# uc-vision/splat-trainer

Hardware: AMD Instinct MI355X
Metric: fwd+bwd Gaussians/s (higher is better)
Workload: dtype f32

## Files before the change

include/gsplat_hip.h:

```cpp
#ifndef GSPLAT_HIP_H
#define GSPLAT_HIP_H

#include <stddef.h>
#include <stdint.h>

#ifdef __cplusplus
extern "C" {
#endif

#define GSR_OK 0
#define GSR_ERR_INVALID_ARGUMENT -1
#define GSR_ERR_WORKSPACE_TOO_SMALL -2
#define GSR_ERR_LAUNCH_FAILED -3
#define GSR_ERR_UNSUPPORTED -4

#define GSR_ROW_FLOATS 16
#define GSR_PARTIAL_FLOATS 12
#define GSR_MAX_FEATURES 16
#define GSR_WIDE_MIN_FEATURES 4

#ifndef GSR_HAVE_RASTER_PARAMS
#define GSR_HAVE_RASTER_PARAMS
typedef struct GsrRasterParamsC {
  float alpha_threshold;
  float clamp_max_alpha;
  float T_eps;
  float q_max;
  float blur;
  int32_t antialias;
  int32_t tile_size;
  float margin_px;
} GsrRasterParamsC;
#endif

typedef struct GsrSegmentsC {
  const uint32_t* tile_seg;
  const uint32_t* seg_desc;
  const uint32_t* seg_total;
  int64_t capacity;
  int64_t heavy_capacity;
  float* seg_P;
  float* seg_TC;
  int32_t* seg_last;
  float* seg_median;
  const uint32_t* tile_order;
} GsrSegmentsC;
#define GSR_SEG_TOTAL_WORDS 272
#define GSR_TILE_ORDER_WORDS(num_tiles) (8 * 32 * ((((num_tiles) + 127) / 128) * 16))

int64_t gsr_struct_bytes(int32_t which);
int gsr_abi_version(void);
const char* gsr_error_string(int code);

size_t gsr_scan_workspace_bytes(int64_t n);
int gsr_exclusive_scan_u32(const uint32_t* in, uint32_t* out, int64_t n, uint32_t* total_dev, void* workspace,
                           size_t workspace_bytes, void* stream);
int gsr_exclusive_scan_u32_checked(const uint32_t* in, uint32_t* out, int64_t n, uint32_t* total_dev,
                                   uint32_t* overflow_dev, void* workspace, size_t workspace_bytes, void* stream);
size_t gsr_sort_workspace_bytes(int64_t n);
int gsr_sort_pairs_u32(uint32_t* keys_a, uint32_t* vals_a, uint32_t* keys_b, uint32_t* vals_b, int64_t n,
                       int vals_are_iota, int begin_bit, int end_bit, void* workspace, size_t workspace_bytes,
                       const uint32_t* n_dev, void* stream);
int gsr_sort_pairs2_u32(uint32_t* keys_a, uint32_t* vals_a, uint32_t* vals2_a, uint32_t* keys_b, uint32_t* vals_b,
                        uint32_t* vals2_b, int64_t n, int vals_are_iota, int begin_bit, int end_bit, void* workspace,
                        size_t workspace_bytes, const uint32_t* n_dev, void* stream);

size_t gsr_cull_workspace_bytes(int64_t N);
int gsr_frustum_cull(const float* position, int64_t N, const float* T_camera_world, const float* projection,
                     int32_t W, int32_t H, float near_plane, float far_plane, float margin_px,
                     int64_t* indexes_out, uint32_t* count_dev, void* workspace, size_t workspace_bytes, void* stream);

int gsr_project_forward(const float* position, const float* log_scaling, const float* rotation_xyzw,
                        const float* alpha_logit, const int64_t* indexes, int64_t M, const float* T_camera_world,
                        const float* projection, const GsrRasterParamsC* params_host, float* gaussians2d_out,
                        float* depth_out, const uint32_t* count_dev, uint32_t* depth_keys_out, uint32_t depth_key_bias,
                        uint32_t depth_key_max, void* stream);
int gsr_project_backward(const float* position, const float* log_scaling, const float* rotation_xyzw,
                         const float* alpha_logit, const int64_t* indexes, int64_t M, const float* T_camera_world,
                         const float* projection, const GsrRasterParamsC* params_host, const float* dL_dgaussians2d,
                         const float* dL_ddepth, float* d_position, float* d_log_scaling, float* d_rotation,
                         float* d_alpha_logit, int32_t accumulate, void* stream);

int64_t gsr_camera_grad_partial_rows(int64_t count);
int gsr_project_backward_camera(const float* position, const float* log_scaling, const float* rotation_xyzw,
                                const float* alpha_logit, const int64_t* indexes, int64_t M, const float* T_camera_world,
                                const float* projection, const GsrRasterParamsC* params_host,
                                const float* dL_dgaussians2d, const float* dL_ddepth, float* d_position,
                                float* d_log_scaling, float* d_rotation, float* d_alpha_logit, int32_t accumulate,
                                float* camera_partials, float* d_camera, void* stream);
int gsr_sh_camera_position_grad(const float* dL_dcolors, const float* jacobian, int64_t M, float* camera_partials,
                                float* d_camera_pos, void* stream);
int gsr_camera_grad_finish(const float* camera_partials, int64_t rows, const float* T_camera_world, float* d_camera,
                           void* stream);

int gsr_sh_forward(const float* sh_features, const float* positions, const int64_t* indexes, int64_t M, int32_t K,
                   const float* camera_pos, float* colors_out, float* jacobian_out, const uint32_t* count_dev,
                   void* stream);
int gsr_sh_backward(const float* dL_dcolors, const float* sh_features, const float* positions, const int64_t* indexes,
                    int64_t M, int32_t K, const float* camera_pos, const float* jacobian ,
                    float* d_sh_features, float* d_positions, int32_t accumulate, void* stream);

int gsr_inverse_map(const int64_t* indexes, int64_t M, int64_t N, int32_t* inverse_out, void* stream);
int gsr_sh_backward_dense(const float* dL_dcolors, const float* sh_features, const float* positions,
                          const int32_t* inverse, int64_t M, int64_t N, int32_t K, const float* camera_pos,
                          const float* jacobian , float* d_sh_features, float* d_positions,
                          void* stream);

int gsr_sh_backward_multi(const float* dL_dcolors_dense, int64_t dense_stride, const float* camera_positions,
                          int64_t camera_stride, int32_t num_cameras, const float* sh_features, const float* positions,
                          int64_t N, int32_t K, float* d_sh_features, float* d_positions, int32_t accumulate,
                          void* stream);

int gsr_project_sh_forward(const float* position, const float* log_scaling, const float* rotation_xyzw,
                           const float* alpha_logit, const float* sh_features, int32_t K, const int64_t* indexes, int64_t M,
                           const float* T_camera_world, const float* projection, const float* camera_pos,
                           const GsrRasterParamsC* params_host, float* rows_out, float* screen_scale_out,
                           float* jacobian_out, const uint32_t* count_dev, uint32_t* depth_keys_out,
                           uint32_t depth_key_bias, uint32_t depth_key_max, void* stream);
int gsr_project_backward_rows(const float* position, const float* log_scaling, const float* rotation_xyzw,
                              const float* alpha_logit, const int64_t* indexes, int64_t M, const int32_t* inverse,
                              int64_t N, const float* T_camera_world, const float* projection,
                              const GsrRasterParamsC* params_host, const float* rows ,
                              const float* grad_rows, const float* dL_dgaussians2d_extra, const float* dL_ddepth,
                              const float* jacobian,
                              float* d_position, float* d_log_scaling, float* d_rotation, float* d_alpha_logit,
                              int32_t mode, float* d_colors_out, float* prune_cost_out, float* split_score_out,
                              float* visibility_out, void* stream);
int gsr_project_backward_rows_camera(const float* position, const float* log_scaling, const float* rotation_xyzw,
                                     const float* alpha_logit, const int64_t* indexes, int64_t M, const int32_t* inverse,
                                     int64_t N, const float* T_camera_world, const float* projection,
                                     const GsrRasterParamsC* params_host, const float* rows, const float* grad_rows,
                                     const float* dL_dgaussians2d_extra, const float* dL_ddepth, const float* jacobian,
                                     float* d_position, float* d_log_scaling, float* d_rotation, float* d_alpha_logit,
                                     int32_t mode, float* d_colors_out, float* prune_cost_out, float* split_score_out,
                                     float* visibility_out, float* camera_partials, float* d_camera, void* stream);

int gsr_depth_key_range(float near_plane, float far_plane, uint32_t* bias_out, uint32_t* max_key_out);
int gsr_depth_keys(const float* depth, int64_t M, uint32_t bias, uint32_t max_key, uint32_t* keys_out, void* stream);
int gsr_pack_rows(const float* gaussians2d, const float* depth, const float* features, int64_t M, int32_t C,
                  const GsrRasterParamsC* params_host, float* rows_out, float* screen_scale_out, void* stream);
int gsr_pack_rows_wide(const float* gaussians2d, const float* depth, const float* features, int64_t M, int32_t C,
                       const GsrRasterParamsC* params_host, float* rows_out, float* feat_rows_out, float* screen_scale_out,
                       void* stream);
int gsr_tile_count(const float* rows, const uint32_t* order, int64_t M, int32_t W, int32_t H,
                   const GsrRasterParamsC* params_host, uint32_t* count_out, uint32_t* tile_hits_out,
                   const uint32_t* M_dev , void* stream);
#define GSR_TILE_COUNT_OFFSETS_MAX 4194304
size_t gsr_tile_count_offsets_workspace_bytes(int64_t M);
int gsr_tile_count_offsets(const float* rows, const uint32_t* order, int64_t M, int32_t W, int32_t H,
                           const GsrRasterParamsC* params_host, uint32_t* count_out, uint32_t* tile_hits_out,
                           const uint32_t* M_dev, uint32_t* offsets_out, uint32_t* total_dev, uint32_t* overflow_flag,
                           void* workspace, size_t workspace_bytes, void* stream);
int gsr_tile_emit(const float* rows, const uint32_t* order, const uint32_t* offsets, const uint32_t* tile_hits, int64_t M,
                  int32_t W, int32_t H, const GsrRasterParamsC* params_host, uint32_t* keys_out, uint32_t* inst2splat_out,
                  int64_t capacity, const uint32_t* M_dev , void* stream);
int gsr_tile_ranges(const uint32_t* sorted_keys, int64_t O, int32_t num_tiles, uint32_t* tile_range,
                    const uint32_t* O_dev , void* stream);

int gsr_segment_thresholds(int32_t seg_pairs_cfg, int32_t heavy_min_cfg, int64_t O, int32_t num_tiles, int32_t needs_grad,
                           int32_t* seg_pairs_out, int32_t* heavy_min_out);
int64_t gsr_segment_capacity(int64_t O, int32_t O_is_bound, int32_t seg_pairs_cfg, int32_t heavy_min_cfg, int32_t num_tiles,
                             int32_t needs_grad);
int64_t gsr_segment_heavy_capacity(int64_t O, int32_t O_is_bound, int32_t seg_pairs_cfg, int32_t heavy_min_cfg,
                                   int32_t num_tiles, int32_t needs_grad);
int gsr_segment_plan(const uint32_t* tile_range, int32_t num_tiles, int32_t seg_pairs_cfg, int32_t heavy_min_cfg,
                     int32_t needs_grad, int64_t O, const uint32_t* O_dev, int64_t capacity, int64_t heavy_capacity,
                     uint32_t* tile_seg_out, uint32_t* seg_desc_out, uint32_t* seg_total_out, uint32_t* tile_order_out,
                     void* stream);

int gsr_composite_forward(const float* rows , const uint32_t* sorted_splat, const uint32_t* sorted_inst,
                          const uint32_t* tile_range, int32_t W, int32_t H, int32_t C,
                          const GsrRasterParamsC* params_host, float* image_out, float* final_T_out,
                          int32_t* last_out, float* median_depth_out, float* vis_partial_out, float* pair_vis_out,
                          const GsrSegmentsC* segments_host ,
                          int32_t prefetch_rows ,
                          void* stream);
int gsr_composite_forward_wide(const float* rows , const float* feat_rows ,
                               const uint32_t* sorted_splat, const uint32_t* sorted_inst, const uint32_t* tile_range,
                               int32_t W, int32_t H, int32_t C, const GsrRasterParamsC* params_host, float* image_out,
                               float* final_T_out, int32_t* last_out, float* median_depth_out, float* vis_partial_out,
                               float* pair_vis_out, void* stream);
#ifndef GSR_PREFETCH_MIN_ROWS
#define GSR_PREFETCH_MIN_ROWS 1000000
#endif

int gsr_composite_backward(const float* rows , const uint32_t* sorted_splat, const uint32_t* sorted_inst,
                           const float* pair_vis, const uint32_t* tile_range, int32_t W, int32_t H, int32_t C,
                           const GsrRasterParamsC* params_host, const float* final_T, const int32_t* last,
                           const float* dL_dimage, const float* image ,
                           float* partial_out, const GsrSegmentsC* segments_host ,
                           void* stream);
int gsr_composite_backward_wide(const float* rows , const float* feat_rows ,
                                const uint32_t* sorted_splat, const uint32_t* sorted_inst, const float* pair_vis,
                                const uint32_t* tile_range, int32_t W, int32_t H, int32_t C,
                                const GsrRasterParamsC* params_host, const float* final_T, const int32_t* last,
                                const float* dL_dimage, float* partial_out, void* stream);

int gsr_reduce_visibility(const float* vis_partial, const uint32_t* offsets, const uint32_t* count,
                          const uint32_t* order, int64_t M, float* visibility_out, int64_t capacity,
                          const uint32_t* M_dev , void* stream);
int gsr_reduce_gradients(const float* partial, const float* vis_partial, const uint32_t* offsets,
                         const uint32_t* count, const uint32_t* order, int64_t M, float* grad_rows_out, void* stream);
int gsr_reduce_gradients_wide(const float* partial, const float* vis_partial, const uint32_t* offsets,
                              const uint32_t* count, const uint32_t* order, int64_t M, int32_t C, float* grad_rows_out,
                              float* d_features_out, void* stream);
int gsr_unpack_grad_rows(const float* rows , const float* grad_rows, int64_t M, int32_t C,
                         float* d_gaussians2d, float* d_features, float* prune_cost_out, float* split_score_out,
                         float* visibility_out, void* stream);

typedef struct GsrFrameC {
  const float* position;
  const float* log_scaling;
  const float* rotation_xyzw;
  const float* alpha_logit;
  const float* sh_features;
  int64_t N;
  int32_t K;
  int32_t W, H;
  const float* T_camera_world;
  const float* projection;
  const float* camera_pos;
  float near_plane, far_plane;
  GsrRasterParamsC params;
  int32_t want_jacobian;
  int32_t want_median;
  int32_t compute_visibility;
  int32_t needs_grad;
  int32_t seg_pairs, seg_min_pairs;
  int64_t pair_capacity;
  const float* gaussians2d;
  const float* depth;
  const float* features;
  int32_t C;
  const uint32_t* depth_order;
  int32_t feature_table;
} GsrFrameC;
typedef struct GsrFramePlanC {
  int64_t out_bytes, work_bytes;
  int64_t zero_begin, zero_bytes;
  int64_t prune_cost, split_score, counts, tile_range, vis_partial, indexes, rows, screen_scale, jacobian, visibility,
      image, final_T, last, median, count, offsets, vals_a, vals_b, tvals_a, tvals_b, trank_a, trank_b, pair_vis,
      seg_tables, seg_pix, seg_last;
  int64_t seg_capacity, seg_heavy_capacity;
  int64_t cull_ws, sort_ws, scan_ws, tsort_ws, keys_a, keys_b, tile_hits, tkeys_a, tkeys_b;
  int64_t cull_ws_bytes, sort_ws_bytes, scan_ws_bytes, tsort_ws_bytes;
  int64_t feat_rows;
} GsrFramePlanC;
typedef struct GsrFrameResultC {
  int64_t order;
  int64_t sorted_inst;
  int64_t sorted_splat;
  GsrSegmentsC segments;
  int32_t has_segments;
} GsrFrameResultC;
int gsr_frame_plan(const GsrFrameC* frame_host, GsrFramePlanC* plan_out_host);
int gsr_frame_forward(const GsrFrameC* frame_host, const GsrFramePlanC* plan_host, void* out_arena, void* work_arena,
                      GsrFrameResultC* result_out_host, uint32_t* counts_host, void* event_counts, void* event_k6_begin,
                      void* event_k6_end, void* stream);

typedef struct GsrFrameBackwardC {
  const float* position; const float* log_scaling; const float* rotation_xyzw; const float* alpha_logit;
  const float* sh_features;
  int64_t N; int32_t K; int32_t W, H, C;
  const float* T_camera_world; const float* projection; const float* camera_pos;
  GsrRasterParamsC params;
  int64_t M, O;
  const int64_t* indexes; const float* rows; const uint32_t* order; const uint32_t* count; const uint32_t* offsets;
  const uint32_t* sorted_splat; const uint32_t* sorted_inst; const float* pair_vis; const float* vis_partial;
  const uint32_t* tile_range; const float* final_T; const int32_t* last; const float* image;
  const float* jacobian;
  const GsrSegmentsC* segments;
  const float* d_image; const float* d_gaussians2d; const float* d_depth;
  float* partial;
  float* grad_rows;
  int32_t* inverse;
  float* d_colors;
  float* d_position; float* d_log_scaling; float* d_rotation; float* d_alpha_logit; int32_t mode;
  float* d_sh; int32_t sh_mode;
  float* prune_cost; float* split_score; float* visibility;
  float* camera_partials; float* d_camera;
} GsrFrameBackwardC;
int gsr_frame_backward(const GsrFrameBackwardC* backward_host, void* event_k7_begin, void* event_k7_end, void* stream);
int gsr_frame_backward_stages(const GsrFrameBackwardC* backward_host, int32_t stages, void* event_k7_begin,
                              void* event_k7_end, void* stream);

size_t gsr_ssim_workspace_bytes(int32_t B, int32_t C, int32_t H, int32_t W);
int gsr_ssim_forward(const float* img1, const float* img2, const int64_t* strides1_host, const int64_t* strides2_host,
                     int32_t B, int32_t C, int32_t H, int32_t W, int32_t crop, float* mean_out, float* dm_dmu1,
                     float* dm_dm11, float* dm_dm12, void* workspace, size_t workspace_bytes, void* stream);
int gsr_ssim_backward(const float* img1, const float* img2, const int64_t* strides1_host, const int64_t* strides2_host,
                      const int64_t* strides_out_host, int32_t B, int32_t C, int32_t H, int32_t W, const float* dm_dmu1,
                      const float* dm_dm11, const float* dm_dm12, const float* grad_scale_dev, float* d_img1,
                      void* stream);

size_t gsr_pixel_loss_workspace_bytes(int64_t n);
int gsr_pixel_loss_forward(const float* image, const float* target, int64_t n, int32_t kind, float lo, float hi,
                           float* loss_out, void* workspace, size_t workspace_bytes, void* stream);
int gsr_pixel_loss_backward(const float* image, const float* target, int64_t n, int32_t kind, float lo, float hi,
                            const float* grad_scale_dev, float* d_image, void* stream);

int gsr_opt_point_weights(const int64_t* indexes, const float* visibility, int64_t M, float* step, float* vis_avg,
                          float beta1, float beta2, float vis_beta, float vis_smooth, int32_t bias_correction,
                          float* row_scale_out, void* stream);
int gsr_opt_step(float* param, const float* grad, float* exp_avg, float* exp_avg_sq, const int64_t* indexes,
                 const float* row_scale, const float* basis, int64_t M, int32_t D, int32_t type, int32_t algo, float lr,
                 float beta1, float beta2, float eps, float grad_clip, void* stream);
int gsr_point_basis(const float* log_scaling, const float* rotation_xyzw, const int64_t* indexes, int64_t M, float eps,
                    float* basis_out, void* stream);

size_t gsr_select_workspace_bytes(int64_t N);
int gsr_select_n(const float* values, int64_t N, int64_t n, int32_t descending, uint8_t* mask_out, void* workspace,
                 size_t workspace_bytes, void* stream);

#define GSR_MAX_COLUMNS 32
typedef struct GsrColumnC {
  const void* src;
  void* dst;
  const void* tail;
  int32_t width_dwords;
} GsrColumnC;
size_t gsr_compact_workspace_bytes(int64_t N);
int gsr_compact_offsets(const uint8_t* keep_mask, int64_t N, uint32_t* block_offsets_out, uint32_t* kept_total_dev,
                        void* workspace, size_t workspace_bytes, void* stream);
int gsr_compact_columns(const uint8_t* keep_mask, int64_t N, const uint32_t* block_offsets, int64_t kept_total,
                        int64_t n_tail, const GsrColumnC* columns_host, int32_t n_columns, void* stream);

int gsr_point_state_add(const int64_t* idx, const float* screen_scale, int32_t scale_cols, const float* visibility,
                        const float* split_score, const float* prune_cost, int64_t M, float split_alpha,
                        float prune_alpha, float* state_prune_cost, float* state_split_score, float* state_max_scale_px,
                        int16_t* state_points_in_view, float* state_visibility, float* visible_sum, void* stream);

size_t gsr_msloss_workspace_bytes(int32_t H, int32_t W, int32_t C, int32_t levels);
int gsr_msloss_forward(const float* image, const float* target, int32_t H, int32_t W, int32_t C, int32_t levels,
                       float w_l1, float w_mse, float w_ssim, float lo, float hi, float* metrics_out, void* workspace,
                       size_t workspace_bytes, void* stream);
int gsr_msloss_backward(const float* image, const float* target, int32_t H, int32_t W, int32_t C, int32_t levels,
                        float w_l1, float w_mse, float w_ssim, float lo, float hi, const float* grad_scale_dev,
                        void* workspace, size_t workspace_bytes, float* d_image, void* stream);

#define GSR_BILAGRID_MAX_SIDE 32768
size_t gsr_bilagrid_workspace_bytes(int32_t L, int32_t GH, int32_t GW);
int gsr_bilagrid_slice_forward(const float* grids, int64_t N, int32_t L, int32_t GH, int32_t GW, int64_t k,
                               const float* rgb, int32_t H, int32_t W, float* out, void* stream);
int gsr_bilagrid_slice_backward(const float* grids, int64_t N, int32_t L, int32_t GH, int32_t GW, int64_t k,
                                const float* rgb, int32_t H, int32_t W, const float* d_out, float* d_rgb, float* d_grids,
                                void* workspace, size_t workspace_bytes, void* stream);
int gsr_bilagrid_tv(const float* grids, int64_t N, int32_t L, int32_t GH, int32_t GW, float weight, float* tv_out,
                    float* d_grids, int32_t accumulate, void* workspace, size_t workspace_bytes, void* stream);

#define GSR_KNN_MAX_K 16
#define GSR_NEIGHBOURS_MAX_N 0x7FFFFFFF
size_t gsr_knn_workspace_bytes(int64_t N, int32_t k);
int gsr_knn(const float* points, int64_t N, int32_t k, float* dist2_out, int64_t* idx_out, float* scale_out,
            void* workspace, size_t workspace_bytes, void* stream);
int gsr_assign_clusters(const float* x, int64_t N, const float* centroids, int64_t K, int64_t* labels_out, void* stream);
size_t gsr_kmeans_workspace_bytes(int64_t N, int64_t K);
int gsr_kmeans_iter(const float* x, int64_t N, float* centroids, int64_t K, int32_t iters, int64_t* labels_out,
                    void* workspace, size_t workspace_bytes, void* stream);

typedef struct GsrColorModel {
  int32_t P, G, H, L, S, color_channels;
  const float* weight[7];
  const float* bias[7];
} GsrColorModel;
typedef struct GsrColorGrads {
  float* d_weight[7];
  float* d_bias[7];
  float* d_glo;
  float* d_cam_pos;
} GsrColorGrads;
int64_t gsr_color_struct_bytes(int32_t which);
int gsr_color_supported(const GsrColorModel* model);
size_t gsr_color_forward_workspace_bytes(const GsrColorModel* model);
size_t gsr_color_backward_workspace_bytes(const GsrColorModel* model, int64_t M);
int gsr_color_forward(const GsrColorModel* model, const float* point_features, const float* positions,
                      const float* cam_pos, const float* glo_feature, int64_t M, float* diffuse_out, float* specular_out,
                      void* workspace, size_t workspace_bytes, void* stream);
int gsr_color_backward(const GsrColorModel* model, const float* point_features, const float* positions,
                       const float* cam_pos, const float* glo_feature, int64_t M, const float* d_diffuse,
                       const float* d_specular, float* d_point_features, const GsrColorGrads* grads, void* workspace,
                       size_t workspace_bytes, void* stream);

#define GSR_DP_BLOCK_FLOATS(N) (6 * (int64_t)(N) + 3)
int gsr_dp_pack(const int64_t* idx, const float* dL_dcolors, const float* split_score, const float* prune_cost,
                const float* screen_scale, int32_t scale_cols, const float* camera_pos, int64_t M, int64_t N,
                float* block_out, const float* visibility, float* visibility_sum, float* views_sum, void* stream);
int gsr_dp_replay(const float* blocks, int64_t stride, const int32_t* slots, int32_t num_cameras, int64_t N,
                  float split_alpha, float prune_alpha, float* state_split_score, float* state_prune_cost,
                  float* state_max_scale_px, const float* visibility_sum, const float* views_sum,
                  float* state_visibility, int16_t* state_points_in_view, void* stream);

int gsr_dp_pack_sharded(const int64_t* idx, const float* dL_dcolors, const float* split_score, const float* prune_cost,
                        const float* screen_scale, int32_t scale_cols, const float* camera_pos, int64_t M, int64_t N,
                        int32_t num_ranks, int32_t slots_per_rank, int32_t slot, float* factors_out, float* scores_out,
                        float* scale_max, const float* visibility, float* visibility_sum, float* views_sum, void* stream);
int gsr_dp_pack_factors_rows(const int64_t* idx, const float* grad_rows, const float* camera_pos, int64_t M, int64_t N,
                             float* factors_out, void* stream);
int gsr_dp_replay_slice(const float* recv, int32_t num_ranks, int32_t slots_per_rank, int64_t N, int32_t rank,
                        int32_t num_cameras, float split_alpha, float prune_alpha, const float* state_split_score,
                        const float* state_prune_cost, float* slice_out, void* stream);
int gsr_dp_finish(const float* gathered, int32_t num_ranks, int64_t N, float* state_split_score, float* state_prune_cost,
                  const float* scale_max, float* state_max_scale_px, const float* visibility_sum, const float* views_sum,
                  float* state_visibility, int16_t* state_points_in_view, void* stream);

#ifdef __cplusplus
}
#endif
#endif
```

splat-trainer_amd/_lib.py:

```python
from __future__ import annotations

import ctypes as C
import os
import threading

import torch

PKG_DIR = os.path.dirname(os.path.abspath(__file__))
LIB_PATH = os.path.join(PKG_DIR, "libgsplat_hip.so")

ABI_VERSION = 36
PREFETCH_MIN_ROWS = 1_000_000
MAX_FEATURES = 16
WIDE_MIN_FEATURES = 4
BILAGRID_MAX_SIDE = 32768
KNN_MAX_K = 16
NEIGHBOURS_MAX_N = 0x7FFFFFFF


class GsrRasterParamsC(C.Structure):
  _fields_ = [("alpha_threshold", C.c_float), ("clamp_max_alpha", C.c_float), ("T_eps", C.c_float),
              ("q_max", C.c_float), ("blur", C.c_float), ("antialias", C.c_int32), ("tile_size", C.c_int32),
              ("margin_px", C.c_float)]


class GsrSegmentsC(C.Structure):
  _fields_ = [("tile_seg", C.c_void_p), ("seg_desc", C.c_void_p), ("seg_total", C.c_void_p), ("capacity", C.c_int64),
              ("heavy_capacity", C.c_int64), ("seg_P", C.c_void_p), ("seg_TC", C.c_void_p), ("seg_last", C.c_void_p),
              ("seg_median", C.c_void_p), ("tile_order", C.c_void_p)]


class GsrFrameC(C.Structure):
  _fields_ = [("position", C.c_void_p), ("log_scaling", C.c_void_p), ("rotation_xyzw", C.c_void_p),
              ("alpha_logit", C.c_void_p), ("sh_features", C.c_void_p), ("N", C.c_int64), ("K", C.c_int32),
              ("W", C.c_int32), ("H", C.c_int32), ("T_camera_world", C.c_void_p), ("projection", C.c_void_p),
              ("camera_pos", C.c_void_p), ("near_plane", C.c_float), ("far_plane", C.c_float),
              ("params", GsrRasterParamsC), ("want_jacobian", C.c_int32), ("want_median", C.c_int32),
              ("compute_visibility", C.c_int32), ("needs_grad", C.c_int32), ("seg_pairs", C.c_int32),
              ("seg_min_pairs", C.c_int32), ("pair_capacity", C.c_int64), ("gaussians2d", C.c_void_p),
              ("depth", C.c_void_p), ("features", C.c_void_p), ("C", C.c_int32), ("depth_order", C.c_void_p),
              ("feature_table", C.c_int32)]


FRAME_PLAN_FIELDS = ("out_bytes", "work_bytes", "zero_begin", "zero_bytes", "prune_cost", "split_score", "counts",
                     "tile_range", "vis_partial", "indexes", "rows", "screen_scale", "jacobian", "visibility", "image",
                     "final_T", "last", "median", "count", "offsets", "vals_a", "vals_b", "tvals_a", "tvals_b", "trank_a",
                     "trank_b", "pair_vis", "seg_tables", "seg_pix", "seg_last", "seg_capacity", "seg_heavy_capacity",
                     "cull_ws", "sort_ws", "scan_ws", "tsort_ws", "keys_a", "keys_b", "tile_hits", "tkeys_a", "tkeys_b",
                     "cull_ws_bytes", "sort_ws_bytes", "scan_ws_bytes", "tsort_ws_bytes", "feat_rows")


class GsrFramePlanC(C.Structure):
  _fields_ = [(name, C.c_int64) for name in FRAME_PLAN_FIELDS]


class GsrFrameBackwardC(C.Structure):
  _fields_ = [("position", C.c_void_p), ("log_scaling", C.c_void_p), ("rotation_xyzw", C.c_void_p),
              ("alpha_logit", C.c_void_p), ("sh_features", C.c_void_p), ("N", C.c_int64), ("K", C.c_int32),
              ("W", C.c_int32), ("H", C.c_int32), ("C", C.c_int32), ("T_camera_world", C.c_void_p),
              ("projection", C.c_void_p), ("camera_pos", C.c_void_p), ("params", GsrRasterParamsC), ("M", C.c_int64),
              ("O", C.c_int64), ("indexes", C.c_void_p), ("rows", C.c_void_p), ("order", C.c_void_p),
              ("count", C.c_void_p), ("offsets", C.c_void_p), ("sorted_splat", C.c_void_p), ("sorted_inst", C.c_void_p),
              ("pair_vis", C.c_void_p), ("vis_partial", C.c_void_p), ("tile_range", C.c_void_p), ("final_T", C.c_void_p),
              ("last", C.c_void_p), ("image", C.c_void_p), ("jacobian", C.c_void_p), ("segments", C.c_void_p),
              ("d_image", C.c_void_p), ("d_gaussians2d", C.c_void_p), ("d_depth", C.c_void_p), ("partial", C.c_void_p),
              ("grad_rows", C.c_void_p), ("inverse", C.c_void_p), ("d_colors", C.c_void_p), ("d_position", C.c_void_p),
              ("d_log_scaling", C.c_void_p), ("d_rotation", C.c_void_p), ("d_alpha_logit", C.c_void_p),
              ("mode", C.c_int32), ("d_sh", C.c_void_p), ("sh_mode", C.c_int32), ("prune_cost", C.c_void_p),
              ("split_score", C.c_void_p), ("visibility", C.c_void_p), ("camera_partials", C.c_void_p),
              ("d_camera", C.c_void_p)]


class GsrFrameResultC(C.Structure):
  _fields_ = [("order", C.c_int64), ("sorted_inst", C.c_int64), ("sorted_splat", C.c_int64), ("segments", GsrSegmentsC),
              ("has_segments", C.c_int32)]


class GsrColumnC(C.Structure):
  _fields_ = [("src", C.c_void_p), ("dst", C.c_void_p), ("tail", C.c_void_p), ("width_dwords", C.c_int32)]


MAX_COLUMNS = 32


class GsrColorModelC(C.Structure):
  _fields_ = [("P", C.c_int32), ("G", C.c_int32), ("H", C.c_int32), ("L", C.c_int32), ("S", C.c_int32),
              ("color_channels", C.c_int32), ("weight", C.c_void_p * 7), ("bias", C.c_void_p * 7)]


class GsrColorGradsC(C.Structure):
  _fields_ = [("d_weight", C.c_void_p * 7), ("d_bias", C.c_void_p * 7), ("d_glo", C.c_void_p),
              ("d_cam_pos", C.c_void_p)]


def raster_params(config) -> GsrRasterParamsC:
  blur = float(config.blur_cov) + (float(config.aa_blur) if config.antialias else 0.0)
  return GsrRasterParamsC(float(config.alpha_threshold), float(config.clamp_max_alpha),
                          float(config.transmittance_eps), float(config.gaussian_scale) ** 2, blur,
                          1 if config.antialias else 0, int(config.tile_size),
                          float(config.margin_tiles * config.tile_size))


_p = C.c_void_p
_i64, _i32, _u32, _f, _sz = C.c_int64, C.c_int32, C.c_uint32, C.c_float, C.c_size_t
_pp = C.POINTER(GsrRasterParamsC)
_ps = C.POINTER(GsrSegmentsC)

PROTOTYPES = {
    "gsr_abi_version": (C.c_int, []),
    "gsr_error_string": (C.c_char_p, [C.c_int]),
    "gsr_scan_workspace_bytes": (_sz, [_i64]),
    "gsr_exclusive_scan_u32": (C.c_int, [_p, _p, _i64, _p, _p, _sz, _p]),
    "gsr_exclusive_scan_u32_checked": (C.c_int, [_p, _p, _i64, _p, _p, _p, _sz, _p]),
    "gsr_sort_workspace_bytes": (_sz, [_i64]),
    "gsr_sort_pairs_u32": (C.c_int, [_p, _p, _p, _p, _i64, C.c_int, C.c_int, C.c_int, _p, _sz, _p, _p]),
    "gsr_sort_pairs2_u32": (C.c_int, [_p, _p, _p, _p, _p, _p, _i64, C.c_int, C.c_int, C.c_int, _p, _sz, _p, _p]),
    "gsr_cull_workspace_bytes": (_sz, [_i64]),
    "gsr_frustum_cull": (C.c_int, [_p, _i64, _p, _p, _i32, _i32, _f, _f, _f, _p, _p, _p, _sz, _p]),
    "gsr_project_forward": (C.c_int, [_p, _p, _p, _p, _p, _i64, _p, _p, _pp, _p, _p, _p, _p, _u32, _u32, _p]),
    "gsr_project_backward": (C.c_int, [_p, _p, _p, _p, _p, _i64, _p, _p, _pp, _p, _p, _p, _p, _p, _p, _i32, _p]),
    "gsr_camera_grad_partial_rows": (_i64, [_i64]),
    "gsr_project_backward_camera": (C.c_int, [_p, _p, _p, _p, _p, _i64, _p, _p, _pp, _p, _p, _p, _p, _p, _p, _i32, _p, _p,
                                              _p]),
    "gsr_sh_camera_position_grad": (C.c_int, [_p, _p, _i64, _p, _p, _p]),
    "gsr_camera_grad_finish": (C.c_int, [_p, _i64, _p, _p, _p]),
    "gsr_sh_forward": (C.c_int, [_p, _p, _p, _i64, _i32, _p, _p, _p, _p, _p]),
    "gsr_sh_backward": (C.c_int, [_p, _p, _p, _p, _i64, _i32, _p, _p, _p, _p, _i32, _p]),
    "gsr_sh_backward_multi": (C.c_int, [_p, _i64, _p, _i64, _i32, _p, _p, _i64, _i32, _p, _p, _i32, _p]),
    "gsr_inverse_map": (C.c_int, [_p, _i64, _i64, _p, _p]),
    "gsr_sh_backward_dense": (C.c_int, [_p, _p, _p, _p, _i64, _i64, _i32, _p, _p, _p, _p, _p]),
    "gsr_depth_key_range": (C.c_int, [_f, _f, _p, _p]),
    "gsr_depth_keys": (C.c_int, [_p, _i64, _u32, _u32, _p, _p]),
    "gsr_project_sh_forward": (C.c_int, [_p, _p, _p, _p, _p, _i32, _p, _i64, _p, _p, _p, _pp, _p, _p, _p, _p, _p, _u32,
                                         _u32, _p]),
    "gsr_project_backward_rows": (C.c_int, [_p, _p, _p, _p, _p, _i64, _p, _i64, _p, _p, _pp, _p, _p, _p, _p, _p, _p, _p,
                                            _p, _p, _i32, _p, _p, _p, _p, _p]),
    "gsr_project_backward_rows_camera": (C.c_int, [_p, _p, _p, _p, _p, _i64, _p, _i64, _p, _p, _pp, _p, _p, _p, _p, _p,
                                                   _p, _p, _p, _p, _i32, _p, _p, _p, _p, _p, _p, _p]),
    "gsr_pack_rows": (C.c_int, [_p, _p, _p, _i64, _i32, _pp, _p, _p, _p]),
    "gsr_pack_rows_wide": (C.c_int, [_p, _p, _p, _i64, _i32, _pp, _p, _p, _p, _p]),
    "gsr_tile_count": (C.c_int, [_p, _p, _i64, _i32, _i32, _pp, _p, _p, _p, _p]),
    "gsr_tile_count_offsets_workspace_bytes": (_sz, [_i64]),
    "gsr_tile_count_offsets": (C.c_int, [_p, _p, _i64, _i32, _i32, _pp, _p, _p, _p, _p, _p, _p, _p, _sz, _p]),
    "gsr_tile_emit": (C.c_int, [_p, _p, _p, _p, _i64, _i32, _i32, _pp, _p, _p, _i64, _p, _p]),
    "gsr_tile_ranges": (C.c_int, [_p, _i64, _i32, _p, _p, _p]),
    "gsr_segment_thresholds": (C.c_int, [_i32, _i32, _i64, _i32, _i32, _p, _p]),
    "gsr_segment_capacity": (_i64, [_i64, _i32, _i32, _i32, _i32, _i32]),
    "gsr_segment_heavy_capacity": (_i64, [_i64, _i32, _i32, _i32, _i32, _i32]),
    "gsr_segment_plan": (C.c_int, [_p, _i32, _i32, _i32, _i32, _i64, _p, _i64, _i64, _p, _p, _p, _p, _p]),
    "gsr_composite_forward": (C.c_int, [_p, _p, _p, _p, _i32, _i32, _i32, _pp, _p, _p, _p, _p, _p, _p, _ps, _i32, _p]),
    "gsr_composite_backward": (C.c_int, [_p, _p, _p, _p, _p, _i32, _i32, _i32, _pp, _p, _p, _p, _p, _p, _ps, _p]),
    "gsr_composite_forward_wide": (C.c_int, [_p, _p, _p, _p, _p, _i32, _i32, _i32, _pp, _p, _p, _p, _p, _p, _p, _p]),
    "gsr_composite_backward_wide": (C.c_int, [_p, _p, _p, _p, _p, _p, _i32, _i32, _i32, _pp, _p, _p, _p, _p, _p]),
    "gsr_opt_point_weights": (C.c_int, [_p, _p, _i64, _p, _p, _f, _f, _f, _f, _i32, _p, _p]),
    "gsr_opt_step": (C.c_int, [_p, _p, _p, _p, _p, _p, _p, _i64, _i32, _i32, _i32, _f, _f, _f, _f, _f, _p]),
    "gsr_pixel_loss_workspace_bytes": (_sz, [_i64]),
    "gsr_pixel_loss_forward": (C.c_int, [_p, _p, _i64, _i32, _f, _f, _p, _p, _sz, _p]),
    "gsr_pixel_loss_backward": (C.c_int, [_p, _p, _i64, _i32, _f, _f, _p, _p, _p]),
    "gsr_ssim_workspace_bytes": (_sz, [_i32, _i32, _i32, _i32]),
    "gsr_ssim_forward": (C.c_int, [_p, _p, _p, _p, _i32, _i32, _i32, _i32, _i32, _p, _p, _p, _p, _p, _sz, _p]),
    "gsr_ssim_backward": (C.c_int, [_p, _p, _p, _p, _p, _i32, _i32, _i32, _i32, _p, _p, _p, _p, _p, _p]),
    "gsr_msloss_workspace_bytes": (_sz, [_i32, _i32, _i32, _i32]),
    "gsr_msloss_forward": (C.c_int, [_p, _p, _i32, _i32, _i32, _i32, _f, _f, _f, _f, _f, _p, _p, _sz, _p]),
    "gsr_msloss_backward": (C.c_int, [_p, _p, _i32, _i32, _i32, _i32, _f, _f, _f, _f, _f, _p, _p, _sz, _p, _p]),
    "gsr_select_workspace_bytes": (_sz, [_i64]),
    "gsr_select_n": (C.c_int, [_p, _i64, _i64, _i32, _p, _p, _sz, _p]),
    "gsr_compact_workspace_bytes": (_sz, [_i64]),
    "gsr_compact_offsets": (C.c_int, [_p, _i64, _p, _p, _p, _sz, _p]),
    "gsr_compact_columns": (C.c_int, [_p, _i64, _p, _i64, _i64, C.POINTER(GsrColumnC), _i32, _p]),
    "gsr_point_basis": (C.c_int, [_p, _p, _p, _i64, _f, _p, _p]),
    "gsr_dp_pack": (C.c_int, [_p, _p, _p, _p, _p, _i32, _p, _i64, _i64, _p, _p, _p, _p, _p]),
    "gsr_dp_replay": (C.c_int, [_p, _i64, _p, _i32, _i64, _f, _f, _p, _p, _p, _p, _p, _p, _p, _p]),
    "gsr_dp_pack_sharded": (C.c_int, [_p, _p, _p, _p, _p, _i32, _p, _i64, _i64, _i32, _i32, _i32, _p, _p, _p, _p, _p, _p, _p]),
    "gsr_dp_replay_slice": (C.c_int, [_p, _i32, _i32, _i64, _i32, _i32, _f, _f, _p, _p, _p, _p]),
    "gsr_dp_finish": (C.c_int, [_p, _i32, _i64, _p, _p, _p, _p, _p, _p, _p, _p, _p]),
    "gsr_point_state_add": (C.c_int, [_p, _p, _i32, _p, _p, _p, _i64, _f, _f, _p, _p, _p, _p, _p, _p, _p]),
    "gsr_frame_plan": (C.c_int, [C.POINTER(GsrFrameC), C.POINTER(GsrFramePlanC)]),
    "gsr_struct_bytes": (_i64, [_i32]),
    "gsr_frame_backward": (C.c_int, [C.POINTER(GsrFrameBackwardC), _p, _p, _p]),
    "gsr_frame_backward_stages": (C.c_int, [C.POINTER(GsrFrameBackwardC), _i32, _p, _p, _p]),
    "gsr_dp_pack_factors_rows": (C.c_int, [_p, _p, _p, _i64, _i64, _p, _p]),
    "gsr_frame_forward": (C.c_int, [C.POINTER(GsrFrameC), C.POINTER(GsrFramePlanC), _p, _p, C.POINTER(GsrFrameResultC), _p,
                                    _p, _p, _p, _p]),
    "gsr_reduce_visibility": (C.c_int, [_p, _p, _p, _p, _i64, _p, _i64, _p, _p]),
    "gsr_reduce_gradients": (C.c_int, [_p, _p, _p, _p, _p, _i64, _p, _p]),
    "gsr_reduce_gradients_wide": (C.c_int, [_p, _p, _p, _p, _p, _i64, _i32, _p, _p, _p]),
    "gsr_unpack_grad_rows": (C.c_int, [_p, _p, _i64, _i32, _p, _p, _p, _p, _p, _p]),
    "gsr_bilagrid_workspace_bytes": (_sz, [_i32, _i32, _i32]),
    "gsr_bilagrid_slice_forward": (C.c_int, [_p, _i64, _i32, _i32, _i32, _i64, _p, _i32, _i32, _p, _p]),
    "gsr_bilagrid_slice_backward": (C.c_int, [_p, _i64, _i32, _i32, _i32, _i64, _p, _i32, _i32, _p, _p, _p, _p, _sz, _p]),
    "gsr_bilagrid_tv": (C.c_int, [_p, _i64, _i32, _i32, _i32, _f, _p, _p, _i32, _p, _sz, _p]),
    "gsr_knn_workspace_bytes": (_sz, [_i64, _i32]),
    "gsr_knn": (C.c_int, [_p, _i64, _i32, _p, _p, _p, _p, _sz, _p]),
    "gsr_assign_clusters": (C.c_int, [_p, _i64, _p, _i64, _p, _p]),
    "gsr_kmeans_workspace_bytes": (_sz, [_i64, _i64]),
    "gsr_kmeans_iter": (C.c_int, [_p, _i64, _p, _i64, _i32, _p, _p, _sz, _p]),
    "gsr_color_struct_bytes": (_i64, [_i32]),
    "gsr_color_supported": (C.c_int, [C.POINTER(GsrColorModelC)]),
    "gsr_color_forward_workspace_bytes": (_sz, [C.POINTER(GsrColorModelC)]),
    "gsr_color_backward_workspace_bytes": (_sz, [C.POINTER(GsrColorModelC), _i64]),
    "gsr_color_forward": (C.c_int, [C.POINTER(GsrColorModelC), _p, _p, _p, _p, _i64, _p, _p, _p, _sz, _p]),
    "gsr_color_backward": (C.c_int, [C.POINTER(GsrColorModelC), _p, _p, _p, _p, _i64, _p, _p, _p,
                                     C.POINTER(GsrColorGradsC), _p, _sz, _p]),
}

_lib = None
_lock = threading.Lock()


def current_stream_ptr() -> int:
  return torch._C._cuda_getCurrentRawStream(torch._C._cuda_getDevice())


def current_stream() -> "torch.cuda.Stream":
  return torch.cuda.current_stream(torch._C._cuda_getDevice())


class GsplatHipError(RuntimeError):
  pass


def load() -> C.CDLL:
  global _lib
  if _lib is not None:
    return _lib
  with _lock:
    if _lib is not None:
      return _lib
    if not os.path.exists(LIB_PATH):
      raise GsplatHipError(
          f"{LIB_PATH} not found: build it with `python splat-trainer_amd/build.py` "
          "(hipcc --offload-arch=gfx950). There is no CPU fallback for the rasterizer path.")
    try:
      lib = C.CDLL(LIB_PATH)
    except OSError as e:
      raise GsplatHipError(f"failed to load {LIB_PATH}: {e}") from e
    for name, (restype, argtypes) in PROTOTYPES.items():
      fn = getattr(lib, name)
      fn.restype = restype
      fn.argtypes = argtypes
    if lib.gsr_abi_version() != ABI_VERSION:
      raise GsplatHipError(f"ABI mismatch: library {lib.gsr_abi_version()} != binding {ABI_VERSION}; rebuild")
    for which, mirror in enumerate((GsrRasterParamsC, GsrSegmentsC, GsrFrameC, GsrFramePlanC, GsrFrameResultC,
                                    GsrFrameBackwardC)):
      if lib.gsr_struct_bytes(which) != C.sizeof(mirror):
        raise GsplatHipError(f"struct layout mismatch: {mirror.__name__} is {C.sizeof(mirror)} bytes in the binding, "
                             f"{lib.gsr_struct_bytes(which)} in the library; rebuild")
    for which, mirror in enumerate((GsrColorModelC, GsrColorGradsC)):
      if lib.gsr_color_struct_bytes(which) != C.sizeof(mirror):
        raise GsplatHipError(f"struct layout mismatch: {mirror.__name__} is {C.sizeof(mirror)} bytes in the binding, "
                             f"{lib.gsr_color_struct_bytes(which)} in the library; rebuild")
    _lib = lib
  return _lib


def check(code: int, what: str) -> int:
  if code < 0:
    msg = load().gsr_error_string(code).decode()
    raise GsplatHipError(f"{what} failed: {msg} ({code})")
  return code
```

splat-trainer_amd/csrc/binning.hip:

```cpp
#include "gsr_device.h"
#include "../../include/gsplat_hip.h"

namespace {

inline GsrRasterParams to_params(const GsrRasterParamsC* c) {
  GsrRasterParams rp;
  __builtin_memcpy(&rp, c, sizeof(rp));
  return rp;
}
inline unsigned grid_for(int64_t n, int block) { return (unsigned)((n + block - 1) / block); }

__global__ __launch_bounds__(256) void depth_keys_kernel(const float* __restrict__ depth, int64_t M,
                                                         uint32_t* __restrict__ keys, uint32_t bias, uint32_t max_key) {
  const int64_t m = (int64_t)blockIdx.x * blockDim.x + threadIdx.x;
  if (m >= M) return;
  keys[m] = gsr_depth_key(depth[m], bias, max_key);
}

struct TileHits {
  uint32_t origin;
  uint32_t shape;
  uint32_t lo, hi;
};

__device__ __forceinline__ uint32_t hits_of_large_extent(float u, float v, float A, float B, float C, float qmax, int x0,
                                                         int x1, int y0, int y1, uint32_t* keys, uint32_t* ranks,
                                                         uint32_t o, uint32_t capacity, uint32_t k, int tiles_x,
                                                         int lane) {
  const int nx = x1 - x0, total = nx * (y1 - y0);
  uint32_t n = 0;
  for (int t0 = 0; t0 < total; t0 += 64) {
    const int t = t0 + lane;
    uint32_t hm = 0u;
    int tx = 0, ty = 0;
    if (t < total) {
      ty = y0 + t / nx;
      tx = x0 + t % nx;
      if (gsr_tile_hit(u, v, A, B, C, qmax, tx, ty)) hm = gsr_tile_half_mask(u, v, A, B, C, qmax, tx, ty);
    }
    const uint64_t hit = __ballot(hm != 0u);
    if (keys && hm) {
      const uint32_t at = o + n + (uint32_t)gsr_mbcnt(hit);
      if (at < capacity) {
        keys[at] = (uint32_t)(ty * tiles_x + tx);
        ranks[at] = k | (hm << 30);
      }
    }
    n += (uint32_t)__builtin_popcountll(hit);
  }
  return n;
}

__device__ __forceinline__ float gsr_bcast(float x, int l) {
  return __int_as_float(__builtin_amdgcn_readlane(__float_as_int(x), l));
}

__device__ __forceinline__ uint32_t wave_large_extents(bool large, float u, float v, float A, float B, float C,
                                                       const GsrExtent& e, uint32_t* keys, uint32_t* ranks, uint32_t o,
                                                       uint32_t capacity, uint32_t sid, int tiles_x, int lane) {
  uint32_t mine = 0u;
  uint64_t todo = __ballot(large);
  while (todo) {
    const int l = __builtin_ctzll(todo);
    todo &= todo - 1ull;
    const uint32_t n = hits_of_large_extent(
        gsr_bcast(u, l), gsr_bcast(v, l), gsr_bcast(A, l), gsr_bcast(B, l), gsr_bcast(C, l), gsr_bcast(e.qmax, l),
        __builtin_amdgcn_readlane(e.x0, l), __builtin_amdgcn_readlane(e.x1, l), __builtin_amdgcn_readlane(e.y0, l),
        __builtin_amdgcn_readlane(e.y1, l), keys, ranks, (uint32_t)__builtin_amdgcn_readlane((int)o, l), capacity,
        (uint32_t)__builtin_amdgcn_readlane((int)sid, l), tiles_x, lane);
    if (lane == l) mine = n;
  }
  return mine;
}

__device__ __forceinline__ uint32_t tile_count_one(const float* __restrict__ rows, const uint32_t* __restrict__ order,
                                                   int64_t k, bool live, int tiles_x, int tiles_y,
                                                   const GsrRasterParams& rp, TileHits* __restrict__ hits) {
  float2 uv = make_float2(0.f, 0.f), ab = uv, co = uv;
  GsrExtent e;
  e.x0 = e.x1 = e.y0 = e.y1 = 0; e.qmax = 0.f;
  TileHits h;
  h.origin = 0u; h.shape = 0u; h.lo = 0u; h.hi = 0u;
  uint32_t n = 0;
  bool large = false;
  if (live) {
    const int64_t s = order[k];
    const float4* r = reinterpret_cast<const float4*>(rows + GSR_ROW_FLOATS * s);
    const float4 r0 = r[0];
    const float4 r1 = r[1];
    uv = make_float2(r0.x, r0.y); ab = make_float2(r0.z, r0.w); co = make_float2(r1.x, r1.y);
    e = gsr_splat_extent(uv.x, uv.y, ab.x, ab.y, co.x, co.y, rp, tiles_x, tiles_y);
    const int nx = e.x1 - e.x0, ny = e.y1 - e.y0;
    h.origin = (uint32_t)e.x0 | ((uint32_t)e.y0 << 16);
    if (nx > 0 && ny > 0) {
      if (nx * ny <= 32) {
        h.shape = (uint32_t)nx | ((uint32_t)ny << 8);
        uint64_t map = 0ull;
        int t = 0;
        for (int ty = e.y0; ty < e.y1; ++ty)
          for (int tx = e.x0; tx < e.x1; ++tx, ++t) {
            const uint64_t hm = gsr_tile_half_mask(uv.x, uv.y, ab.x, ab.y, co.x, e.qmax, tx, ty);
            map |= hm << (2 * t);
            n += hm ? 1u : 0u;
          }
        h.lo = (uint32_t)map; h.hi = (uint32_t)(map >> 32);
      } else {
        h.shape = 1u << 16;
        large = true;
      }
    }
  }
  const uint32_t nl = wave_large_extents(large, uv.x, uv.y, ab.x, ab.y, co.x, e, nullptr, nullptr, 0u, 0u, 0u, tiles_x,
                                         gsr_lane());
  if (large) n = nl;
  if (live) *reinterpret_cast<uint4*>(hits + k) = make_uint4(h.origin, h.shape, h.lo, h.hi);
  return n;
}

__global__ __launch_bounds__(256) void tile_count_kernel(const float* __restrict__ rows,
                                                         const uint32_t* __restrict__ order, int64_t M, int tiles_x,
                                                         int tiles_y, GsrRasterParams rp, uint32_t* __restrict__ count,
                                                         TileHits* __restrict__ hits,
                                                         const uint32_t* __restrict__ M_dev,
                                                         uint32_t* __restrict__ block_sums) {
  const int64_t k = (int64_t)blockIdx.x * blockDim.x + threadIdx.x;
  const bool live = k < M && !(M_dev && k >= (int64_t)*M_dev);
  uint32_t n = tile_count_one(rows, order, k, live, tiles_x, tiles_y, rp, hits);
  if (k < M) count[k] = n;
  if (block_sums) {
    __shared__ uint32_t s_wave[4];
    n = gsr_wave_sum_u32(n);
    if (gsr_lane() == 0) s_wave[threadIdx.x >> 6] = n;
    __syncthreads();
    if (threadIdx.x == 0) block_sums[blockIdx.x] = (s_wave[0] + s_wave[1]) + (s_wave[2] + s_wave[3]);
  }
}

__global__ __launch_bounds__(256) void offsets_from_sums_kernel(const uint32_t* __restrict__ count, uint32_t n,
                                                                const uint32_t* __restrict__ sums256,
                                                                uint32_t* __restrict__ offsets,
                                                                uint32_t* __restrict__ total_out,
                                                                uint32_t* __restrict__ overflow) {
  __shared__ uint32_t s_wave[4], s_before[4];
  __shared__ float s_f[4];
  const int lane = gsr_lane(), w = (int)(threadIdx.x >> 6);
  const uint32_t base = blockIdx.x * 4096u + threadIdx.x * 16u;
  uint32_t v[16], sum = 0u;
#pragma unroll
  for (int i = 0; i < 16; ++i) {
    v[i] = (base + i < n) ? count[base + i] : 0u;
    sum += v[i];
  }
  uint32_t before = 0u;
  float fbefore = 0.f;
  for (uint32_t j = threadIdx.x; j < blockIdx.x * 16u; j += 256u) {
    const uint32_t b = sums256[j];
    before += b;
    fbefore += (float)b;
  }
  const uint32_t incl = gsr_wave_scan_incl_u32(sum);
  before = gsr_wave_sum_u32(before);
  fbefore = gsr_wave_sum(fbefore + (float)sum);
  if (lane == 63) s_wave[w] = incl;
  if (lane == 0) { s_before[w] = before; s_f[w] = fbefore; }
  __syncthreads();
  uint32_t prefix = (s_before[0] + s_before[1]) + (s_before[2] + s_before[3]), total = 0u;
  uint32_t in_block = 0u;
#pragma unroll
  for (int j = 0; j < 4; ++j) {
    if (j < w) in_block += s_wave[j];
    total += s_wave[j];
  }
  if (threadIdx.x == 0 && (s_f[0] + s_f[1]) + (s_f[2] + s_f[3]) >= 2147000000.f) *overflow = 1u;
  uint32_t run = prefix + in_block + incl - sum;
#pragma unroll
  for (int i = 0; i < 16; ++i) {
    if (base + i < n) offsets[base + i] = run;
    run += v[i];
  }
  if (total_out && blockIdx.x == gridDim.x - 1 && threadIdx.x == 0) *total_out = prefix + total;
}


__global__ __launch_bounds__(256) void tile_emit_kernel(const float* __restrict__ rows,
                                                        const uint32_t* __restrict__ order,
                                                        const uint32_t* __restrict__ offsets,
                                                        const TileHits* __restrict__ hits, int64_t M, int tiles_x,
                                                        int tiles_y, GsrRasterParams rp, uint32_t* __restrict__ keys,
                                                        uint32_t* __restrict__ inst2splat, uint32_t capacity,
                                                        const uint32_t* __restrict__ M_dev) {
  const int64_t k = (int64_t)blockIdx.x * blockDim.x + threadIdx.x;
  const bool live = k < M && !(M_dev && k >= (int64_t)*M_dev);
  uint4 hw = make_uint4(0u, 0u, 0u, 0u);
  uint32_t o = 0u, sid = 0u;
  if (live) {
    hw = *reinterpret_cast<const uint4*>(hits + k);
    o = offsets[k];
    sid = order[k];
  }
  const bool large = (hw.y >> 16) != 0u;
  float4 r0 = make_float4(0.f, 0.f, 0.f, 0.f), r1 = r0;
  GsrExtent e;
  e.x0 = e.x1 = e.y0 = e.y1 = 0; e.qmax = 0.f;
  if (large) {
    const float4* r = reinterpret_cast<const float4*>(rows + GSR_ROW_FLOATS * (int64_t)sid);
    r0 = r[0];
    r1 = r[1];
    e = gsr_splat_extent(r0.x, r0.y, r0.z, r0.w, r1.x, r1.y, rp, tiles_x, tiles_y);
  }
  wave_large_extents(large, r0.x, r0.y, r0.z, r0.w, r1.x, e, keys, inst2splat, o, capacity, sid, tiles_x, gsr_lane());
  if (!live || large) return;
  const int nx = (int)(hw.y & 0xFFu), ny = (int)((hw.y >> 8) & 0xFFu);
  const int x0 = (int)(hw.x & 0xFFFFu), y0 = (int)(hw.x >> 16);
  uint64_t map = (uint64_t)hw.z | ((uint64_t)hw.w << 32);
  for (int j = 0; j < ny; ++j)
    for (int i = 0; i < nx; ++i, map >>= 2) {
      const uint32_t hm = (uint32_t)(map & 3ull);
      if (!hm) continue;
      if (o >= capacity) return;
      keys[o] = (uint32_t)((y0 + j) * tiles_x + x0 + i);
      inst2splat[o] = sid | (hm << 30);
      ++o;
    }
}

__global__ __launch_bounds__(256) void tile_ranges_kernel(const uint32_t* __restrict__ keys, int64_t O,
                                                          uint32_t* __restrict__ range,
                                                          const uint32_t* __restrict__ O_dev) {
  if (O_dev) O = min(O, (int64_t)*O_dev);
  const int64_t i = (int64_t)blockIdx.x * blockDim.x + threadIdx.x;
  if (i >= O) return;
  const uint32_t t = keys[i];
  if (i == 0 || keys[i - 1] != t) range[2 * t] = (uint32_t)i;
  if (i == O - 1 || keys[i + 1] != t) range[2 * t + 1] = (uint32_t)(i + 1);
}

#define GSR_REDUCE_SERIAL 64u

__global__ __launch_bounds__(256) void reduce_vis_kernel(const float* __restrict__ vis_partial,
                                                         const uint32_t* __restrict__ offsets,
                                                         const uint32_t* __restrict__ count,
                                                         const uint32_t* __restrict__ order, int64_t M,
                                                         float* __restrict__ vis, uint32_t limit,
                                                         const uint32_t* __restrict__ M_dev) {
  const int64_t k = (int64_t)blockIdx.x * blockDim.x + threadIdx.x;
  const bool live = k < M && !(M_dev && k >= (int64_t)*M_dev);
  const uint32_t b = live ? offsets[k] : 0u, n = live ? count[k] : 0u;
  const int lane = gsr_lane();
  float acc = 0.f;
  if (n <= GSR_REDUCE_SERIAL)
    for (uint32_t j = 0; j < n && b + j < limit; ++j) acc += vis_partial[b + j];
  uint64_t todo = __ballot(n > GSR_REDUCE_SERIAL);
  while (todo) {
    const int l = __builtin_ctzll(todo);
    todo &= todo - 1ull;
    const uint32_t bl = (uint32_t)__builtin_amdgcn_readlane((int)b, l), nl = (uint32_t)__builtin_amdgcn_readlane((int)n, l);
    float total = 0.f;
    for (uint32_t g = 0; g < nl; g += 64u) {
      const uint32_t j = g + (uint32_t)lane;
      const float v = (j < nl && bl + j < limit) ? vis_partial[bl + j] : 0.f;
      total += gsr_wave_sum_to_lane63(v);
    }
    const float t = __int_as_float(__builtin_amdgcn_readlane(__float_as_int(total), 63));
    if (lane == l) acc = t;
  }
  if (live) vis[order ? order[k] : (uint32_t)k] = acc;
}

__global__ __launch_bounds__(256) void reduce_grad_kernel(const float* __restrict__ partial,
                                                          const float* __restrict__ vis_partial,
                                                          const uint32_t* __restrict__ offsets,
                                                          const uint32_t* __restrict__ count,
                                                          const uint32_t* __restrict__ order, int64_t M,
                                                          float* __restrict__ grows) {
  constexpr int CH = 256;
  __shared__ float4 s_part[CH * 3];
  __shared__ float s_vis[CH];
  __shared__ uint32_t s_lo, s_hi;
  const int64_t k0 = (int64_t)blockIdx.x * 256;
  const int64_t k = k0 + threadIdx.x;
  const bool have = k < M;
  const uint32_t b = have ? offsets[k] : 0u, n = have ? count[k] : 0u;
  const bool serial = n <= GSR_REDUCE_SERIAL;
  if (threadIdx.x == 0) s_lo = b;
  const int64_t klast = (k0 + 255 < M ? k0 + 255 : M - 1);
  if (k == klast) s_hi = b + n;
  __syncthreads();
  const uint32_t lo = s_lo, hi = s_hi;
  float4 a0 = make_float4(0.f, 0.f, 0.f, 0.f), a1 = a0, a2 = a0;
  float vsum = 0.f;
  const float4* src = reinterpret_cast<const float4*>(partial);
  for (uint32_t c = lo; c < hi; c += CH) {
    const uint32_t m = min((uint32_t)CH, hi - c);
    const bool mine = threadIdx.x < m;
    const float v = mine ? vis_partial[c + threadIdx.x] : 0.f;
    s_vis[threadIdx.x] = v;
    __syncthreads();
#pragma unroll
    for (int t = 0; t < 3; ++t) {
      const uint32_t f = threadIdx.x + t * CH;
      if (f < 3 * m && s_vis[f / 3] > 0.f) s_part[f] = src[(size_t)3 * c + f];
    }
    __syncthreads();
    const uint32_t j0 = max(b, c), j1 = serial ? min(b + n, c + m) : 0u;
    for (uint32_t j = j0; j < j1; ++j) {
      const uint32_t l = j - c;
      const float pv = s_vis[l];
      vsum += pv;
      if (pv > 0.f) {
        const float4 p0 = s_part[3 * l], p1 = s_part[3 * l + 1], p2 = s_part[3 * l + 2];
        a0.x += p0.x; a0.y += p0.y; a0.z += p0.z; a0.w += p0.w;
        a1.x += p1.x; a1.y += p1.y; a1.z += p1.z; a1.w += p1.w;
        a2.x += p2.x; a2.y += p2.y; a2.z += p2.z;
      }
    }
    __syncthreads();
  }
  const int lane = gsr_lane();
  uint64_t todo = __ballot(!serial);
  while (todo) {
    const int l = __builtin_ctzll(todo);
    todo &= todo - 1ull;
    const uint32_t bl = (uint32_t)__builtin_amdgcn_readlane((int)b, l), nl = (uint32_t)__builtin_amdgcn_readlane((int)n, l);
    float t[12];
#pragma unroll
    for (int i = 0; i < 12; ++i) t[i] = 0.f;
    for (uint32_t g = 0; g < nl; g += 64u) {
      const uint32_t j = g + (uint32_t)lane;
      const float pv = j < nl ? vis_partial[bl + j] : 0.f;
      float4 p0 = make_float4(0.f, 0.f, 0.f, 0.f), p1 = p0, p2 = p0;
      if (pv > 0.f) {
        const float4* q = src + (size_t)3 * (bl + j);
        p0 = q[0]; p1 = q[1]; p2 = q[2];
      }
      t[0] += gsr_wave_sum_to_lane63(p0.x); t[1] += gsr_wave_sum_to_lane63(p0.y);
      t[2] += gsr_wave_sum_to_lane63(p0.z); t[3] += gsr_wave_sum_to_lane63(p0.w);
      t[4] += gsr_wave_sum_to_lane63(p1.x); t[5] += gsr_wave_sum_to_lane63(p1.y);
      t[6] += gsr_wave_sum_to_lane63(p1.z); t[7] += gsr_wave_sum_to_lane63(p1.w);
      t[8] += gsr_wave_sum_to_lane63(p2.x); t[9] += gsr_wave_sum_to_lane63(p2.y);
      t[10] += gsr_wave_sum_to_lane63(p2.z); t[11] += gsr_wave_sum_to_lane63(pv);
    }
#pragma unroll
    for (int i = 0; i < 12; ++i) t[i] = __int_as_float(__builtin_amdgcn_readlane(__float_as_int(t[i]), 63));
    if (lane == l) {
      a0 = make_float4(t[0], t[1], t[2], t[3]);
      a1 = make_float4(t[4], t[5], t[6], t[7]);
      a2 = make_float4(t[8], t[9], t[10], 0.f);
      vsum = t[11];
    }
  }
  if (!have) return;
  const int64_t s = order ? (int64_t)order[k] : k;
  float4* g = reinterpret_cast<float4*>(grows + GSR_ROW_FLOATS * s);
  g[0] = a0;
  g[1] = a1;
  g[2] = make_float4(a2.x, a2.y, a2.z, vsum);
  g[3] = make_float4(0.f, 0.f, 0.f, 0.f);
}

template <int CW>
__global__ __launch_bounds__(256) void reduce_grad_wide_kernel(const float* __restrict__ partial,
                                                               const float* __restrict__ vis_partial,
                                                               const uint32_t* __restrict__ offsets,
                                                               const uint32_t* __restrict__ count,
                                                               const uint32_t* __restrict__ order, int64_t M, int C,
                                                               float* __restrict__ grows, float* __restrict__ dfeat) {
  constexpr int NV = 8 + CW;
  const int64_t k = (int64_t)blockIdx.x * blockDim.x + threadIdx.x;
  const bool have = k < M;
  const uint32_t b = have ? offsets[k] : 0u, n = have ? count[k] : 0u;
  const bool serial = n <= GSR_REDUCE_SERIAL;
  float a[NV];
#pragma unroll
  for (int v = 0; v < NV; ++v) a[v] = 0.f;
  float vsum = 0.f;
  if (serial) {
    for (uint32_t j = b; j < b + n; ++j) {
      const float pv = vis_partial[j];
      vsum += pv;
      if (pv > 0.f) {
        const float* p = partial + (size_t)NV * j;
#pragma unroll
        for (int v = 0; v < NV; ++v) a[v] += p[v];
      }
    }
  }
  const int lane = gsr_lane();
  uint64_t todo = __ballot(!serial);
  while (todo) {
    const int l = __builtin_ctzll(todo);
    todo &= todo - 1ull;
    const uint32_t bl = (uint32_t)__builtin_amdgcn_readlane((int)b, l), nl = (uint32_t)__builtin_amdgcn_readlane((int)n, l);
    float t[NV + 1];
#pragma unroll
    for (int v = 0; v <= NV; ++v) t[v] = 0.f;
    for (uint32_t g = 0; g < nl; g += 64u) {
      const uint32_t j = g + (uint32_t)lane;
      const float pv = j < nl ? vis_partial[bl + j] : 0.f;
      float pr[NV];
#pragma unroll
      for (int v = 0; v < NV; ++v) pr[v] = 0.f;
      if (pv > 0.f) {
        const float* p = partial + (size_t)NV * (bl + j);
#pragma unroll
        for (int v = 0; v < NV; ++v) pr[v] = p[v];
      }
#pragma unroll
      for (int v = 0; v < NV; ++v) t[v] += gsr_wave_sum_to_lane63(pr[v]);
      t[NV] += gsr_wave_sum_to_lane63(pv);
    }
#pragma unroll
    for (int v = 0; v <= NV; ++v) t[v] = __int_as_float(__builtin_amdgcn_readlane(__float_as_int(t[v]), 63));
    if (lane == l) {
#pragma unroll
      for (int v = 0; v < NV; ++v) a[v] = t[v];
      vsum = t[NV];
    }
  }
  if (!have) return;
  const int64_t s = order ? (int64_t)order[k] : k;
  float4* g = reinterpret_cast<float4*>(grows + GSR_ROW_FLOATS * s);
  g[0] = make_float4(a[0], a[1], a[2], a[3]);
  g[1] = make_float4(a[4], a[5], a[6], a[7]);
  g[2] = make_float4(0.f, 0.f, 0.f, vsum);
  g[3] = make_float4(0.f, 0.f, 0.f, 0.f);
#pragma unroll
  for (int c = 0; c < CW; ++c)
    if (c < C) dfeat[(int64_t)C * s + c] = a[8 + c];
}

template <int C>
__global__ __launch_bounds__(256) void unpack_rows_kernel(const float* __restrict__ rows,
                                                          const float* __restrict__ grows, int64_t M,
                                                          float* __restrict__ dg2d, float* __restrict__ dfeat,
                                                          float* __restrict__ prune, float* __restrict__ split,
                                                          float* __restrict__ vis) {
  const int64_t m = (int64_t)blockIdx.x * blockDim.x + threadIdx.x;
  if (m >= M) return;
  const float4* gr = reinterpret_cast<const float4*>(grows + GSR_ROW_FLOATS * m);
  const float4 g0 = gr[0], g1 = gr[1], g2 = gr[2];
  const float4* fr = reinterpret_cast<const float4*>(rows + GSR_ROW_FLOATS * m);
  const float4 f0 = fr[0];
  const float cA = f0.z, cB = f0.w, cC = fr[1].x;
  float* g = dg2d + 6 * m;
  *reinterpret_cast<float2*>(g) = make_float2(cA * g0.x + cB * g0.y, cB * g0.x + cC * g0.y);
  *reinterpret_cast<float2*>(g + 2) = make_float2(-0.5f * g0.z, -g0.w);
  const float op = fr[1].y;
  *reinterpret_cast<float2*>(g + 4) = make_float2(-0.5f * g1.x, op > 0.f ? g1.y / op : 0.f);
  if (prune) prune[m] = g1.z;
  if (split) split[m] = g1.w;
  if (vis) vis[m] = g2.w;
  if (C == 0) return;
  dfeat[C * m] = g2.x;
  if (C > 1) dfeat[C * m + 1] = g2.y;
  if (C > 2) dfeat[C * m + 2] = g2.z;
}

}

extern "C" {

int gsr_depth_key_range(float near_plane, float far_plane, uint32_t* bias_out, uint32_t* max_key_out) {
  if (!bias_out || !max_key_out) return GSR_ERR_INVALID_ARGUMENT;
  *bias_out = 0u;
  *max_key_out = 0xFFFFFFFFu;
  if (near_plane > 0.f && far_plane > near_plane && far_plane < 3.0e38f) {
    uint32_t lo, hi;
    __builtin_memcpy(&lo, &near_plane, 4);
    __builtin_memcpy(&hi, &far_plane, 4);
    *bias_out = lo | 0x80000000u;
    *max_key_out = hi - lo;
  }
  return GSR_OK;
}

int gsr_depth_keys(const float* depth, int64_t M, uint32_t bias, uint32_t max_key, uint32_t* keys_out, void* stream_) {
  hipStream_t stream = reinterpret_cast<hipStream_t>(stream_);
  if (M < 0) return GSR_ERR_INVALID_ARGUMENT;
  if (M == 0) return GSR_OK;
  if (!depth || !keys_out) return GSR_ERR_INVALID_ARGUMENT;
  depth_keys_kernel<<<grid_for(M, 256), 256, 0, stream>>>(depth, M, keys_out, bias, max_key);
  GSR_CHECK_LAUNCH();
  return GSR_OK;
}

int gsr_tile_count(const float* rows, const uint32_t* order, int64_t M, int32_t W, int32_t H,
                   const GsrRasterParamsC* params_host, uint32_t* count_out, uint32_t* tile_hits_out,
                   const uint32_t* M_dev, void* stream_) {
  hipStream_t stream = reinterpret_cast<hipStream_t>(stream_);
  if (M < 0 || M >= (1ll << 30) || !params_host || W <= 0 || H <= 0) return GSR_ERR_INVALID_ARGUMENT;
  if (params_host->tile_size != 16) return GSR_ERR_UNSUPPORTED;
  if (M == 0) return GSR_OK;
  if (!rows || !order || !count_out || !tile_hits_out) return GSR_ERR_INVALID_ARGUMENT;
  const int tx = (W + 15) / 16, ty = (H + 15) / 16;
  if (tx > 0xFFFF || ty > 0xFFFF) return GSR_ERR_UNSUPPORTED;
  tile_count_kernel<<<grid_for(M, 256), 256, 0, stream>>>(rows, order, M, tx, ty, to_params(params_host), count_out,
                                                         reinterpret_cast<TileHits*>(tile_hits_out), M_dev, nullptr);
  GSR_CHECK_LAUNCH();
  return GSR_OK;
}

size_t gsr_tile_count_offsets_workspace_bytes(int64_t M) {
  return M > 0 ? (size_t)((M + 255) / 256) * sizeof(uint32_t) + 256 : 256;
}

int gsr_tile_count_offsets(const float* rows, const uint32_t* order, int64_t M, int32_t W, int32_t H,
                           const GsrRasterParamsC* params_host, uint32_t* count_out, uint32_t* tile_hits_out,
                           const uint32_t* M_dev, uint32_t* offsets_out, uint32_t* total_dev, uint32_t* overflow_flag,
                           void* workspace, size_t workspace_bytes, void* stream_) {
  hipStream_t stream = reinterpret_cast<hipStream_t>(stream_);
  if (M < 0 || M > GSR_TILE_COUNT_OFFSETS_MAX || !params_host || W <= 0 || H <= 0) return GSR_ERR_INVALID_ARGUMENT;
  if (params_host->tile_size != 16) return GSR_ERR_UNSUPPORTED;
  if (!total_dev || !overflow_flag) return GSR_ERR_INVALID_ARGUMENT;
  if (M == 0) { hipMemsetAsync(total_dev, 0, sizeof(uint32_t), stream); return GSR_OK; }
  if (!rows || !order || !count_out || !tile_hits_out || !offsets_out) return GSR_ERR_INVALID_ARGUMENT;
  if (!workspace || workspace_bytes < gsr_tile_count_offsets_workspace_bytes(M)) return GSR_ERR_WORKSPACE_TOO_SMALL;
  const int tx = (W + 15) / 16, ty = (H + 15) / 16;
  if (tx > 0xFFFF || ty > 0xFFFF) return GSR_ERR_UNSUPPORTED;
  uint32_t* sums = reinterpret_cast<uint32_t*>(workspace);
  tile_count_kernel<<<grid_for(M, 256), 256, 0, stream>>>(rows, order, M, tx, ty, to_params(params_host), count_out,
                                                         reinterpret_cast<TileHits*>(tile_hits_out), M_dev, sums);
  GSR_CHECK_LAUNCH();
  offsets_from_sums_kernel<<<grid_for(M, 4096), 256, 0, stream>>>(count_out, (uint32_t)M, sums, offsets_out, total_dev,
                                                                 overflow_flag);
  GSR_CHECK_LAUNCH();
  return GSR_OK;
}

int gsr_tile_emit(const float* rows, const uint32_t* order, const uint32_t* offsets, const uint32_t* tile_hits, int64_t M,
                  int32_t W, int32_t H, const GsrRasterParamsC* params_host, uint32_t* keys_out, uint32_t* inst2splat_out,
                  int64_t capacity, const uint32_t* M_dev, void* stream_) {
  hipStream_t stream = reinterpret_cast<hipStream_t>(stream_);
  if (M < 0 || M >= (1ll << 30) || !params_host || W <= 0 || H <= 0) return GSR_ERR_INVALID_ARGUMENT;
  if (capacity < 0 || capacity > 0x7FFFFFFFll) return GSR_ERR_INVALID_ARGUMENT;
  if (params_host->tile_size != 16) return GSR_ERR_UNSUPPORTED;
  if (M == 0) return GSR_OK;
  if (!rows || !order || !offsets || !tile_hits || !keys_out || !inst2splat_out) return GSR_ERR_INVALID_ARGUMENT;
  const int tx = (W + 15) / 16, ty = (H + 15) / 16;
  tile_emit_kernel<<<grid_for(M, 256), 256, 0, stream>>>(rows, order, offsets, reinterpret_cast<const TileHits*>(tile_hits),
                                                        M, tx, ty, to_params(params_host), keys_out, inst2splat_out,
                                                        (uint32_t)capacity, M_dev);
  GSR_CHECK_LAUNCH();
  return GSR_OK;
}

int gsr_tile_ranges(const uint32_t* sorted_keys, int64_t O, int32_t num_tiles, uint32_t* tile_range,
                    const uint32_t* O_dev, void* stream_) {
  hipStream_t stream = reinterpret_cast<hipStream_t>(stream_);
  if (O < 0 || num_tiles <= 0) return GSR_ERR_INVALID_ARGUMENT;
  if (O == 0) return GSR_OK;
  if (!sorted_keys || !tile_range) return GSR_ERR_INVALID_ARGUMENT;
  tile_ranges_kernel<<<grid_for(O, 256), 256, 0, stream>>>(sorted_keys, O, tile_range, O_dev);
  GSR_CHECK_LAUNCH();
  return GSR_OK;
}

int gsr_reduce_visibility(const float* vis_partial, const uint32_t* offsets, const uint32_t* count,
                          const uint32_t* order, int64_t M, float* visibility_out, int64_t capacity,
                          const uint32_t* M_dev, void* stream_) {
  hipStream_t stream = reinterpret_cast<hipStream_t>(stream_);
  if (M < 0 || capacity < 0 || capacity > 0x7FFFFFFFll) return GSR_ERR_INVALID_ARGUMENT;
  if (M == 0) return GSR_OK;
  if (!offsets || !count || !visibility_out) return GSR_ERR_INVALID_ARGUMENT;
  reduce_vis_kernel<<<grid_for(M, 256), 256, 0, stream>>>(vis_partial, offsets, count, order, M, visibility_out,
                                                         (uint32_t)capacity, M_dev);
  GSR_CHECK_LAUNCH();
  return GSR_OK;
}

int gsr_reduce_gradients(const float* partial, const float* vis_partial, const uint32_t* offsets,
                         const uint32_t* count, const uint32_t* order, int64_t M, float* grad_rows_out, void* stream_) {
  hipStream_t stream = reinterpret_cast<hipStream_t>(stream_);
  if (M < 0) return GSR_ERR_INVALID_ARGUMENT;
  if (M == 0) return GSR_OK;
  if (!offsets || !count || !grad_rows_out) return GSR_ERR_INVALID_ARGUMENT;
  reduce_grad_kernel<<<grid_for(M, 256), 256, 0, stream>>>(partial, vis_partial, offsets, count, order, M, grad_rows_out);
  GSR_CHECK_LAUNCH();
  return GSR_OK;
}

int gsr_reduce_gradients_wide(const float* partial, const float* vis_partial, const uint32_t* offsets,
                              const uint32_t* count, const uint32_t* order, int64_t M, int32_t C, float* grad_rows_out,
                              float* d_features_out, void* stream_) {
  hipStream_t stream = reinterpret_cast<hipStream_t>(stream_);
  if (M < 0) return GSR_ERR_INVALID_ARGUMENT;
  if (C < GSR_WIDE_MIN_FEATURES || C > GSR_MAX_FEATURES) return GSR_ERR_UNSUPPORTED;
  if (M == 0) return GSR_OK;
  if (!offsets || !count || !grad_rows_out || !d_features_out || !vis_partial) return GSR_ERR_INVALID_ARGUMENT;
  const unsigned g = grid_for(M, 256);
  if (C <= 4) reduce_grad_wide_kernel<4><<<g, 256, 0, stream>>>(partial, vis_partial, offsets, count, order, M, C, grad_rows_out, d_features_out);
  else if (C <= 8) reduce_grad_wide_kernel<8><<<g, 256, 0, stream>>>(partial, vis_partial, offsets, count, order, M, C, grad_rows_out, d_features_out);
  else reduce_grad_wide_kernel<16><<<g, 256, 0, stream>>>(partial, vis_partial, offsets, count, order, M, C, grad_rows_out, d_features_out);
  GSR_CHECK_LAUNCH();
  return GSR_OK;
}

int gsr_unpack_grad_rows(const float* rows, const float* grad_rows, int64_t M, int32_t C, float* d_gaussians2d,
                         float* d_features, float* prune_cost_out, float* split_score_out, float* visibility_out,
                         void* stream_) {
  hipStream_t stream = reinterpret_cast<hipStream_t>(stream_);
  if (M < 0) return GSR_ERR_INVALID_ARGUMENT;
  if (C < 1 || C > (d_features ? 3 : GSR_MAX_FEATURES)) return GSR_ERR_UNSUPPORTED;
  if (M == 0) return GSR_OK;
  if (!rows || !grad_rows || !d_gaussians2d) return GSR_ERR_INVALID_ARGUMENT;
  const unsigned g = grid_for(M, 256);
  if (!d_features) unpack_rows_kernel<0><<<g, 256, 0, stream>>>(rows, grad_rows, M, d_gaussians2d, nullptr, prune_cost_out, split_score_out, visibility_out);
  else if (C == 1) unpack_rows_kernel<1><<<g, 256, 0, stream>>>(rows, grad_rows, M, d_gaussians2d, d_features, prune_cost_out, split_score_out, visibility_out);
  else if (C == 2) unpack_rows_kernel<2><<<g, 256, 0, stream>>>(rows, grad_rows, M, d_gaussians2d, d_features, prune_cost_out, split_score_out, visibility_out);
  else unpack_rows_kernel<3><<<g, 256, 0, stream>>>(rows, grad_rows, M, d_gaussians2d, d_features, prune_cost_out, split_score_out, visibility_out);
  GSR_CHECK_LAUNCH();
  return GSR_OK;
}

}
```

splat-trainer_amd/csrc/frame.hip:

```cpp
#include <hip/hip_runtime.h>
#include <stdint.h>
#include <string.h>

#include "../../include/gsplat_hip.h"

namespace {

inline int64_t align_up(int64_t x, int64_t a = 256) { return (x + a - 1) / a * a; }

struct Cursor {
  int64_t at = 0;
  int64_t take(int64_t bytes) {
    const int64_t o = at;
    at = align_up(at + (bytes > 0 ? bytes : 1));
    return o;
  }
};

inline int tile_bits_of(int num_tiles) {
  int b = 1;
  while ((1 << b) < num_tiles) ++b;
  return b;
}

inline int bit_length(uint32_t v) {
  int b = 0;
  while (v) { ++b; v >>= 1; }
  return b < 1 ? 1 : b;
}

template <class T>
inline T* at(void* base, int64_t off) {
  return off < 0 ? nullptr : reinterpret_cast<T*>(reinterpret_cast<uint8_t*>(base) + off);
}

}

extern "C" {

int gsr_frame_plan(const GsrFrameC* f, GsrFramePlanC* p) {
  if (!f || !p) return GSR_ERR_INVALID_ARGUMENT;
  if (f->N < 0 || f->N >= (1ll << 30) || f->W <= 0 || f->H <= 0 || f->pair_capacity < 0 || f->pair_capacity > 0x7FFFFFFFll)
    return GSR_ERR_INVALID_ARGUMENT;
  const bool projected = f->position == nullptr;
  if (!projected && f->K != 1 && f->K != 4 && f->K != 9 && f->K != 16) return GSR_ERR_UNSUPPORTED;
  if (f->C < 1 || f->C > GSR_MAX_FEATURES || (!projected && f->C != 3)) return GSR_ERR_UNSUPPORTED;
  const bool wide = f->C >= GSR_WIDE_MIN_FEATURES;
  if (wide && !f->feature_table) return GSR_ERR_UNSUPPORTED;
  if (f->params.tile_size != 16) return GSR_ERR_UNSUPPORTED;
  memset(p, 0, sizeof(*p));
  const int64_t N = f->N, cap = f->pair_capacity;
  const int64_t tx = (f->W + 15) / 16, ty = (f->H + 15) / 16, T = tx * ty, P = (int64_t)f->W * f->H;
  const bool vis_partial = f->compute_visibility || f->needs_grad;

  Cursor out;
  p->zero_begin = 0;
  p->prune_cost = out.take(4 * N);
  p->split_score = out.take(4 * N);
  p->counts = out.take(4 * (3 + GSR_SEG_TOTAL_WORDS));
  p->tile_range = out.take(4 * 2 * T);
  p->vis_partial = vis_partial ? out.take(4 * cap) : -1;
  p->zero_bytes = out.at;
  p->indexes = projected ? -1 : out.take(8 * N);
  p->rows = out.take(4 * GSR_ROW_FLOATS * N);
  p->screen_scale = out.take(4 * 2 * N);
  p->jacobian = (!projected && f->want_jacobian && f->K > 1) ? out.take(4 * 9 * N) : -1;
  p->visibility = out.take(4 * N);
  p->image = out.take(4 * f->C * P);
  p->final_T = out.take(4 * P);
  p->last = out.take(4 * P);
  p->median = f->want_median ? out.take(4 * P) : -1;
  p->count = out.take(4 * N);
  p->offsets = out.take(4 * N);
  p->vals_a = out.take(4 * N);
  p->vals_b = out.take(4 * N);
  p->tvals_a = out.take(4 * cap);
  p->tvals_b = out.take(4 * cap);
  p->trank_a = out.take(4 * cap + 16);
  p->trank_b = out.take(4 * cap + 16);
  p->pair_vis = vis_partial ? out.take(4 * cap) : -1;
  p->feat_rows = wide ? out.take(4 * (f->C <= 4 ? 4 : f->C <= 8 ? 8 : 16) * N) : -1;
  p->seg_capacity = 0;
  p->seg_heavy_capacity = 0;
  p->seg_tables = p->seg_pix = p->seg_last = -1;
  if (f->seg_pairs != 0 && cap > 0 && !wide) {
    const int64_t sc = gsr_segment_capacity(cap, 1, f->seg_pairs, f->seg_min_pairs, (int32_t)T, f->needs_grad ? 1 : 0);
    if (sc > 0) {
      int64_t hc = gsr_segment_heavy_capacity(cap, 1, f->seg_pairs, f->seg_min_pairs, (int32_t)T, f->needs_grad ? 1 : 0);
      if (hc > sc) hc = sc;
      p->seg_capacity = sc;
      p->seg_heavy_capacity = hc;
      p->seg_tables = out.take(4 * (2 * T + hc + 4 * sc + GSR_TILE_ORDER_WORDS(T)));
      const int64_t planes = 5 + (f->want_median ? 1 : 0);
      p->seg_pix = out.take(4 * planes * sc * 256);
      p->seg_last = out.take(4 * sc * 256);
    }
  }
  p->out_bytes = out.at;

  Cursor work;
  p->cull_ws_bytes = projected ? 0 : (int64_t)gsr_cull_workspace_bytes(N);
  p->sort_ws_bytes = (int64_t)gsr_sort_workspace_bytes(N);
  p->scan_ws_bytes = (int64_t)gsr_scan_workspace_bytes(N);
  if (N <= GSR_TILE_COUNT_OFFSETS_MAX && (int64_t)gsr_tile_count_offsets_workspace_bytes(N) > p->scan_ws_bytes)
    p->scan_ws_bytes = (int64_t)gsr_tile_count_offsets_workspace_bytes(N);
  p->tsort_ws_bytes = (int64_t)gsr_sort_workspace_bytes(cap);
  p->cull_ws = projected ? -1 : work.take(p->cull_ws_bytes);
  p->sort_ws = work.take(p->sort_ws_bytes);
  p->scan_ws = work.take(p->scan_ws_bytes);
  p->tsort_ws = work.take(p->tsort_ws_bytes);
  p->keys_a = work.take(4 * N);
  p->keys_b = work.take(4 * N);
  p->tile_hits = work.take(16 * N);
  p->tkeys_a = work.take(4 * cap);
  p->tkeys_b = work.take(4 * cap);
  p->work_bytes = work.at;
  return GSR_OK;
}

int gsr_frame_forward(const GsrFrameC* f, const GsrFramePlanC* p, void* out, void* work, GsrFrameResultC* res,
                      uint32_t* counts_host, void* event_counts, void* event_k6_begin, void* event_k6_end,
                      void* stream_) {
  hipStream_t stream = reinterpret_cast<hipStream_t>(stream_);
  if (!f || !p || !out || !work || !res) return GSR_ERR_INVALID_ARGUMENT;
  if (f->N <= 0) return GSR_ERR_INVALID_ARGUMENT;
  const bool projected = f->position == nullptr;
  if (projected) {
    if (!f->gaussians2d || !f->depth || !f->features) return GSR_ERR_INVALID_ARGUMENT;
  } else if (!f->log_scaling || !f->rotation_xyzw || !f->alpha_logit || !f->sh_features || !f->T_camera_world ||
             !f->projection || !f->camera_pos) {
    return GSR_ERR_INVALID_ARGUMENT;
  }
  memset(res, 0, sizeof(*res));
  const int64_t N = f->N, cap = f->pair_capacity;
  const int tx = (f->W + 15) / 16, ty = (f->H + 15) / 16, T = tx * ty;
  uint32_t* counts = at<uint32_t>(out, p->counts);
  uint32_t* M_dev = projected ? nullptr : counts;
  uint32_t* O_dev = counts + 1;
  int rc;
#define GSR_TRY(call)          \
  do {                         \
    rc = (call);               \
    if (rc < 0) return rc;     \
  } while (0)

  if (hipMemsetAsync(at<uint8_t>(out, p->zero_begin), 0, (size_t)p->zero_bytes, stream) != hipSuccess)
    return GSR_ERR_LAUNCH_FAILED;
  float* rows = at<float>(out, p->rows);
  uint32_t key_bias = 0, key_max = 0;
  GSR_TRY(gsr_depth_key_range(f->near_plane, f->far_plane, &key_bias, &key_max));
  uint32_t* keys_a = at<uint32_t>(work, p->keys_a);
  if (projected) {
    if (p->feat_rows >= 0)
      GSR_TRY(gsr_pack_rows_wide(f->gaussians2d, f->depth, f->features, N, f->C, &f->params, rows,
                                 at<float>(out, p->feat_rows), at<float>(out, p->screen_scale), stream_));
    else
      GSR_TRY(gsr_pack_rows(f->gaussians2d, f->depth, f->features, N, f->C, &f->params, rows,
                            at<float>(out, p->screen_scale), stream_));
    if (!f->depth_order) GSR_TRY(gsr_depth_keys(f->depth, N, key_bias, key_max, keys_a, stream_));
  } else {
    int64_t* indexes = at<int64_t>(out, p->indexes);
    GSR_TRY(gsr_frustum_cull(f->position, N, f->T_camera_world, f->projection, f->W, f->H, f->near_plane, f->far_plane,
                             f->params.margin_px, indexes, M_dev, at<uint8_t>(work, p->cull_ws),
                             (size_t)p->cull_ws_bytes, stream_));
    GSR_TRY(gsr_project_sh_forward(f->position, f->log_scaling, f->rotation_xyzw, f->alpha_logit, f->sh_features, f->K,
                                   indexes, N, f->T_camera_world, f->projection, f->camera_pos, &f->params, rows,
                                   at<float>(out, p->screen_scale), at<float>(out, p->jacobian), M_dev,
                                   keys_a, key_bias, key_max, stream_));
  }
  uint32_t* vals_a = at<uint32_t>(out, p->vals_a);
  uint32_t* vals_b = at<uint32_t>(out, p->vals_b);
  const uint32_t* order = f->depth_order;
  res->order = -1;
  if (!order) {
    GSR_TRY(gsr_sort_pairs_u32(keys_a, vals_a, at<uint32_t>(work, p->keys_b), vals_b, N, 1, 0, bit_length(key_max),
                               at<uint8_t>(work, p->sort_ws), (size_t)p->sort_ws_bytes, M_dev, stream_));
    res->order = rc == 1 ? p->vals_b : p->vals_a;
    order = rc == 1 ? vals_b : vals_a;
  }
  uint32_t* count = at<uint32_t>(out, p->count);
  uint32_t* offsets = at<uint32_t>(out, p->offsets);
  uint32_t* hits = at<uint32_t>(work, p->tile_hits);
  if (N <= GSR_TILE_COUNT_OFFSETS_MAX) {
    GSR_TRY(gsr_tile_count_offsets(rows, order, N, f->W, f->H, &f->params, count, hits, M_dev, offsets, O_dev, counts + 2,
                                   at<uint8_t>(work, p->scan_ws), (size_t)p->scan_ws_bytes, stream_));
  } else {
    GSR_TRY(gsr_tile_count(rows, order, N, f->W, f->H, &f->params, count, hits, M_dev, stream_));
    GSR_TRY(gsr_exclusive_scan_u32_checked(count, offsets, N, O_dev, counts + 2, at<uint8_t>(work, p->scan_ws),
                                           (size_t)p->scan_ws_bytes, stream_));
  }
  if (counts_host) {
    if (hipMemcpyAsync(counts_host, counts, 3 * sizeof(uint32_t), hipMemcpyDeviceToHost, stream) != hipSuccess)
      return GSR_ERR_LAUNCH_FAILED;
    if (event_counts && hipEventRecord(reinterpret_cast<hipEvent_t>(event_counts), stream) != hipSuccess)
      return GSR_ERR_LAUNCH_FAILED;
  }
  res->sorted_inst = res->sorted_splat = -1;
  float* image = at<float>(out, p->image);
  if (cap > 0) {
    uint32_t* tkeys_a = at<uint32_t>(work, p->tkeys_a);
    uint32_t* tkeys_b = at<uint32_t>(work, p->tkeys_b);
    uint32_t* tvals_a = at<uint32_t>(out, p->tvals_a);
    uint32_t* tvals_b = at<uint32_t>(out, p->tvals_b);
    uint32_t* trank_a = at<uint32_t>(out, p->trank_a);
    uint32_t* trank_b = at<uint32_t>(out, p->trank_b);
    GSR_TRY(gsr_tile_emit(rows, order, offsets, hits, N, f->W, f->H, &f->params, tkeys_a, trank_a, cap, M_dev, stream_));
    GSR_TRY(gsr_sort_pairs2_u32(tkeys_a, tvals_a, trank_a, tkeys_b, tvals_b, trank_b, cap, 1, 0, tile_bits_of(T),
                                at<uint8_t>(work, p->tsort_ws), (size_t)p->tsort_ws_bytes, O_dev, stream_));
    const bool in_b = rc == 1;
    res->sorted_inst = in_b ? p->tvals_b : p->tvals_a;
    res->sorted_splat = in_b ? p->trank_b : p->trank_a;
    const uint32_t* sorted_keys = in_b ? tkeys_b : tkeys_a;
    const uint32_t* sorted_inst = in_b ? tvals_b : tvals_a;
    const uint32_t* sorted_splat = in_b ? trank_b : trank_a;
    uint32_t* tile_range = at<uint32_t>(out, p->tile_range);
    GSR_TRY(gsr_tile_ranges(sorted_keys, cap, T, tile_range, O_dev, stream_));
    const GsrSegmentsC* seg = nullptr;
    if (p->seg_capacity > 0) {
      uint32_t* tables = at<uint32_t>(out, p->seg_tables);
      uint32_t* tile_seg = tables;
      uint32_t* seg_desc = tables + 2 * (int64_t)T + p->seg_heavy_capacity;
      uint32_t* seg_total = counts + 3;
      uint32_t* tile_order = seg_desc + 4 * p->seg_capacity;
      GSR_TRY(gsr_segment_plan(tile_range, T, f->seg_pairs, f->seg_min_pairs, f->needs_grad ? 1 : 0, cap, O_dev,
                               p->seg_capacity, p->seg_heavy_capacity, tile_seg, seg_desc, seg_total, tile_order, stream_));
      float* pix = at<float>(out, p->seg_pix);
      res->segments.tile_seg = tile_seg;
      res->segments.seg_desc = seg_desc;
      res->segments.seg_total = seg_total;
      res->segments.tile_order = tile_order;
      res->segments.capacity = p->seg_capacity;
      res->segments.heavy_capacity = p->seg_heavy_capacity;
      res->segments.seg_TC = pix;
      res->segments.seg_P = pix + 4 * p->seg_capacity * 256;
      res->segments.seg_median = f->want_median ? pix + 5 * p->seg_capacity * 256 : nullptr;
      res->segments.seg_last = at<int32_t>(out, p->seg_last);
      res->has_segments = 1;
      seg = &res->segments;
    }
    if (event_k6_begin && hipEventRecord(reinterpret_cast<hipEvent_t>(event_k6_begin), stream) != hipSuccess)
      return GSR_ERR_LAUNCH_FAILED;
    if (p->feat_rows >= 0)
      GSR_TRY(gsr_composite_forward_wide(rows, at<float>(out, p->feat_rows), sorted_splat, sorted_inst, tile_range, f->W,
                                         f->H, f->C, &f->params, image, at<float>(out, p->final_T),
                                         at<int32_t>(out, p->last), at<float>(out, p->median),
                                         at<float>(out, p->vis_partial), at<float>(out, p->pair_vis), stream_));
    else
      GSR_TRY(gsr_composite_forward(rows, sorted_splat, sorted_inst, tile_range, f->W, f->H, f->C, &f->params, image,
                                    at<float>(out, p->final_T), at<int32_t>(out, p->last), at<float>(out, p->median),
                                    at<float>(out, p->vis_partial), at<float>(out, p->pair_vis), seg,
                                    N >= GSR_PREFETCH_MIN_ROWS ? 1 : 0, stream_));
    if (event_k6_end && hipEventRecord(reinterpret_cast<hipEvent_t>(event_k6_end), stream) != hipSuccess)
      return GSR_ERR_LAUNCH_FAILED;
    if (f->compute_visibility && !f->needs_grad)
      GSR_TRY(gsr_reduce_visibility(at<float>(out, p->vis_partial), offsets, count, order, N,
                                    at<float>(out, p->visibility), cap, M_dev, stream_));
  }
#undef GSR_TRY
  return GSR_OK;
}

int64_t gsr_struct_bytes(int32_t which) {
  switch (which) {
    case 0: return (int64_t)sizeof(GsrRasterParamsC);
    case 1: return (int64_t)sizeof(GsrSegmentsC);
    case 2: return (int64_t)sizeof(GsrFrameC);
    case 3: return (int64_t)sizeof(GsrFramePlanC);
    case 4: return (int64_t)sizeof(GsrFrameResultC);
    case 5: return (int64_t)sizeof(GsrFrameBackwardC);
    default: return -1;
  }
}

int gsr_frame_backward(const GsrFrameBackwardC* b, void* event_k7_begin, void* event_k7_end, void* stream_) {
  return gsr_frame_backward_stages(b, 3, event_k7_begin, event_k7_end, stream_);
}

int gsr_frame_backward_stages(const GsrFrameBackwardC* b, int32_t stages, void* event_k7_begin, void* event_k7_end,
                              void* stream_) {
  hipStream_t stream = reinterpret_cast<hipStream_t>(stream_);
  if (stages < 1 || stages > 3) return GSR_ERR_INVALID_ARGUMENT;
  if (!b || b->N < 0 || b->M < 0 || b->M > b->N || b->O < 0 || b->mode < 0 || b->mode > 2 || b->sh_mode < 0 ||
      b->sh_mode > 2)
    return GSR_ERR_INVALID_ARGUMENT;
  const int64_t M = b->M, N = b->N;
  if (M > 0 && (!b->grad_rows || !b->rows || !b->indexes)) return GSR_ERR_INVALID_ARGUMENT;
  if (b->sh_mode && (!b->d_sh || !b->sh_features || !b->camera_pos || (M > 0 && !b->d_colors))) return GSR_ERR_INVALID_ARGUMENT;
  const bool needs_inverse = M < N && (b->mode == 2 || b->sh_mode == 1);
  if (needs_inverse && !b->inverse) return GSR_ERR_INVALID_ARGUMENT;
#define GSR_TRY(call)                 \
  do {                                \
    const int rc_ = (call);           \
    if (rc_ < 0) return rc_;          \
  } while (0)
  const bool live = M > 0 && b->O > 0 && b->d_image != nullptr;
  if (!(stages & 1)) {
  } else if (live) {
    if (!b->partial || !b->vis_partial) return GSR_ERR_INVALID_ARGUMENT;
    if (event_k7_begin && hipEventRecord(reinterpret_cast<hipEvent_t>(event_k7_begin), stream) != hipSuccess)
      return GSR_ERR_LAUNCH_FAILED;
    GSR_TRY(gsr_composite_backward(b->rows, b->sorted_splat, b->sorted_inst, b->pair_vis, b->tile_range, b->W, b->H, b->C,
                                   &b->params, b->final_T, b->last, b->d_image, b->image, b->partial, b->segments, stream_));
    if (event_k7_end && hipEventRecord(reinterpret_cast<hipEvent_t>(event_k7_end), stream) != hipSuccess)
      return GSR_ERR_LAUNCH_FAILED;
    GSR_TRY(gsr_reduce_gradients(b->partial, b->vis_partial, b->offsets, b->count, b->order, M, b->grad_rows, stream_));
  } else if (M > 0) {
    if (hipMemsetAsync(b->grad_rows, 0, (size_t)M * GSR_ROW_FLOATS * sizeof(float), stream) != hipSuccess)
      return GSR_ERR_LAUNCH_FAILED;
  }
  if (!(stages & 2)) return GSR_OK;
  if (needs_inverse) GSR_TRY(gsr_inverse_map(b->indexes, M, N, b->inverse, stream_));
  if (b->d_camera)
    GSR_TRY(gsr_project_backward_rows_camera(
        b->position, b->log_scaling, b->rotation_xyzw, b->alpha_logit, b->indexes, M, b->mode == 2 ? b->inverse : nullptr,
        N, b->T_camera_world, b->projection, &b->params, b->rows, b->grad_rows, b->d_gaussians2d, b->d_depth, b->jacobian,
        b->d_position, b->d_log_scaling, b->d_rotation, b->d_alpha_logit, b->mode, b->d_colors,
        live ? b->prune_cost : nullptr, live ? b->split_score : nullptr, live ? b->visibility : nullptr,
        b->camera_partials, b->d_camera, stream_));
  else if (M > 0 || b->mode == 2)
    GSR_TRY(gsr_project_backward_rows(b->position, b->log_scaling, b->rotation_xyzw, b->alpha_logit, b->indexes, M,
                                      b->mode == 2 ? b->inverse : nullptr, N, b->T_camera_world, b->projection, &b->params,
                                      b->rows, b->grad_rows, b->d_gaussians2d, b->d_depth, b->jacobian, b->d_position,
                                      b->d_log_scaling, b->d_rotation, b->d_alpha_logit, b->mode, b->d_colors,
                                      live ? b->prune_cost : nullptr, live ? b->split_score : nullptr,
                                      live ? b->visibility : nullptr, stream_));
  if (b->sh_mode == 1) {
    GSR_TRY(gsr_sh_backward_dense(b->d_colors, b->sh_features, b->position, b->inverse, M, N, b->K, b->camera_pos, nullptr,
                                  b->d_sh, nullptr, stream_));
  } else if (b->sh_mode == 2 && M > 0) {
    GSR_TRY(gsr_sh_backward(b->d_colors, b->sh_features, b->position, b->indexes, M, b->K, b->camera_pos, nullptr, b->d_sh,
                            nullptr, 1, stream_));
  }
#undef GSR_TRY
  return GSR_OK;
}

}
```

splat-trainer_amd/csrc/geometry.hip:

```cpp
#include "gsr_device.h"
#include "gsr_dpp_reduce.h"
#include "../../include/gsplat_hip.h"

static_assert(sizeof(GsrRasterParams) == sizeof(GsrRasterParamsC), "raster params layout");

namespace {

constexpr int CULL_ITEMS = 16;
constexpr int CULL_WAVE_SPAN = 64 * CULL_ITEMS;
constexpr int64_t CULL_SELF_PREFIX_MAX_WAVES = 4096;

__global__ __launch_bounds__(256) void cull_count_kernel(const float* __restrict__ pos, int64_t N,
                                                         const float* __restrict__ Tcw, const float* __restrict__ proj,
                                                         int W, int H, float near_p, float far_p, float margin,
                                                         uint32_t* __restrict__ wave_counts, int64_t num_waves) {
  const int64_t wave = (int64_t)blockIdx.x * 4 + (threadIdx.x >> 6);
  if (wave >= num_waves) return;
  const int lane = gsr_lane();
  const GsrCam cam = gsr_load_cam(Tcw, proj);
  const int64_t base = wave * CULL_WAVE_SPAN;
  uint32_t cnt = 0;
#pragma unroll 4
  for (int it = 0; it < CULL_ITEMS; ++it) {
    int64_t i = base + it * 64 + lane;
// ... 490 lines not shown
  GsrProjectGrad o = gsr_project_one_bwd(cam, rp, p, s, q, logit[i], g, gd);
  if (jac) {
    const float g3[3] = {g2.x, g2.y, g2.z};
    float pj[3];
    gsr_jac_apply(g3, jac + 9 * m, pj);
    o.dp[0] += pj[0]; o.dp[1] += pj[1]; o.dp[2] += pj[2];
  }
  constexpr bool ACC = MODE == 1;
  float4 r = make_float4(o.dq[0], o.dq[1], o.dq[2], o.dq[3]);
  if (ACC) {
    const float4 old = *reinterpret_cast<const float4*>(drot + 4 * i);
    r.x += old.x; r.y += old.y; r.z += old.z; r.w += old.w;
  }
#pragma unroll
  for (int k = 0; k < 3; ++k) {
    dpos[3 * i + k] = ACC ? dpos[3 * i + k] + o.dp[k] : o.dp[k];
    dls[3 * i + k] = ACC ? dls[3 * i + k] + o.dls[k] : o.dls[k];
  }
  *reinterpret_cast<float4*>(drot + 4 * i) = r;
  dlogit[i] = ACC ? dlogit[i] + o.dlogit : o.dlogit;
}

__global__ __launch_bounds__(256) void project_bwd_rows_camera_kernel(
    const float* __restrict__ pos, const float* __restrict__ ls, const float* __restrict__ rot,
    const float* __restrict__ logit, const int64_t* __restrict__ idx, int64_t M, const float* __restrict__ Tcw,
    const float* __restrict__ proj, GsrRasterParams rp, const float* __restrict__ grows,
    const float* __restrict__ dg2d_extra, const float* __restrict__ ddepth, const float* __restrict__ jac,
    float* __restrict__ cam_partials) {
  const int64_t m = (int64_t)blockIdx.x * blockDim.x + threadIdx.x;
  float acc[CAM_PARTIAL_FLOATS];
#pragma unroll
  for (int j = 0; j < CAM_PARTIAL_FLOATS; ++j) acc[j] = 0.f;
  if (m < M) {
    const int64_t i = idx[m];
    const float4* gr = reinterpret_cast<const float4*>(grows + (int64_t)GSR_ROW_FLOATS * m);
    const float4 g0 = gr[0], g1 = gr[1], g2 = gr[2];
    const GsrCam cam = gsr_load_cam(Tcw, proj);
    float p[3] = {pos[3 * i], pos[3 * i + 1], pos[3 * i + 2]};
    float s[3] = {ls[3 * i], ls[3 * i + 1], ls[3 * i + 2]};
    const float4 qv = *reinterpret_cast<const float4*>(rot + 4 * i);
    float q[4] = {qv.x, qv.y, qv.z, qv.w};
    const GsrProjected fo = gsr_project_one(cam, rp, p, s, q, logit[i]);
    const float cA = fo.A, cB = fo.B, cC = fo.C;
    float g[6] = {cA * g0.x + cB * g0.y, cB * g0.x + cC * g0.y, -0.5f * g0.z, -g0.w, -0.5f * g1.x,
                  fo.opacity > 0.f ? g1.y / fo.opacity : 0.f};
    if (dg2d_extra) {
#pragma unroll
      for (int k = 0; k < 6; ++k) g[k] += dg2d_extra[6 * m + k];
    }
    const float gd = ddepth ? ddepth[m] : 0.f;
    (void)gsr_project_one_bwd<true>(cam, rp, p, s, q, logit[i], g, gd, acc);
    if (jac) {
      const float g3[3] = {g2.x, g2.y, g2.z};
      float pj[3];
      gsr_jac_apply(g3, jac + 9 * m, pj);
      acc[CAM_POS_AT] = -pj[0]; acc[CAM_POS_AT + 1] = -pj[1]; acc[CAM_POS_AT + 2] = -pj[2];
    }
  }
  gsr_block_cam_sum(acc, cam_partials + (int64_t)blockIdx.x * CAM_PARTIAL_FLOATS);
}

template <int K, bool ACC>
__global__ __launch_bounds__(256) void sh_bwd_kernel(const float* __restrict__ dcol, const float* __restrict__ sh,
                                                     const float* __restrict__ pos, const int64_t* __restrict__ idx,
                                                     int64_t M, const float* __restrict__ cam_pos,
                                                     float* __restrict__ dsh, float* __restrict__ dpos,
                                                     const float* __restrict__ jac) {
  const int64_t m = (int64_t)blockIdx.x * blockDim.x + threadIdx.x;
  if (m >= M) return;
  const int64_t i = idx[m];
  float vx = pos[3 * i] - cam_pos[0], vy = pos[3 * i + 1] - cam_pos[1], vz = pos[3 * i + 2] - cam_pos[2];
  float inv = 1.f / sqrtf(vx * vx + vy * vy + vz * vz);
  const float x = vx * inv, y = vy * inv, z = vz * inv;
  float Y[K];
  gsr_sh_basis<K>(x, y, z, Y);
  float* row = dsh + (int64_t)3 * K * i;
  const float g3[3] = {dcol[3 * m], dcol[3 * m + 1], dcol[3 * m + 2]};
#pragma unroll
  for (int ch = 0; ch < 3; ++ch) {
    const float g = g3[ch];
    if (K % 4 == 0) {
#pragma unroll
      for (int k = 0; k < K; k += 4) {
        float4 v = make_float4(g * Y[k], g * Y[k + 1], g * Y[k + 2], g * Y[k + 3]);
        if (ACC) {
          const float4 old = *reinterpret_cast<const float4*>(row + ch * K + k);
          v.x += old.x; v.y += old.y; v.z += old.z; v.w += old.w;
        }
        *reinterpret_cast<float4*>(row + ch * K + k) = v;
      }
    } else {
#pragma unroll
      for (int k = 0; k < K; ++k) row[ch * K + k] = ACC ? row[ch * K + k] + g * Y[k] : g * Y[k];
    }
  }
  if (dpos != nullptr && jac != nullptr) {
    float pj[3];
    gsr_jac_apply(g3, jac + 9 * m, pj);
    dpos[3 * i] = ACC ? dpos[3 * i] + pj[0] : pj[0];
    dpos[3 * i + 1] = ACC ? dpos[3 * i + 1] + pj[1] : pj[1];
    dpos[3 * i + 2] = ACC ? dpos[3 * i + 2] + pj[2] : pj[2];
  } else if (dpos != nullptr && K > 1) {
    float dYx[K], dYy[K], dYz[K];
    gsr_sh_basis_grad<K>(x, y, z, dYx, dYy, dYz);
    const float* c = sh + (int64_t)3 * K * i;
    float gx = 0.f, gy = 0.f, gz = 0.f;
#pragma unroll
    for (int ch = 0; ch < 3; ++ch) {
#pragma unroll
      for (int k = 1; k < K; ++k) {
        const float w = g3[ch] * c[ch * K + k];
        gx += w * dYx[k]; gy += w * dYy[k]; gz += w * dYz[k];
      }
    }
    const float dot = gx * x + gy * y + gz * z;
    const float px_ = (gx - x * dot) * inv, py_ = (gy - y * dot) * inv, pz_ = (gz - z * dot) * inv;
    dpos[3 * i] = ACC ? dpos[3 * i] + px_ : px_;
    dpos[3 * i + 1] = ACC ? dpos[3 * i + 1] + py_ : py_;
    dpos[3 * i + 2] = ACC ? dpos[3 * i + 2] + pz_ : pz_;
  }
}

__global__ __launch_bounds__(256) void inverse_map_kernel(const int64_t* __restrict__ idx, int64_t M, int64_t N,
                                                          int32_t* __restrict__ inv) {
  const int64_t m = (int64_t)blockIdx.x * blockDim.x + threadIdx.x;
  if (m > M) return;
  const int64_t lo = m > 0 ? idx[m - 1] + 1 : 0;
  const int64_t hi = m < M ? idx[m] : N;
  for (int64_t r = lo; r < hi; ++r) inv[r] = -1;
  if (m < M) inv[hi] = (int32_t)m;
}

template <int K>
__global__ __launch_bounds__(256) void sh_bwd_dense_kernel(const float* __restrict__ dcol, const float* __restrict__ sh,
                                                           const float* __restrict__ pos,
                                                           const int32_t* __restrict__ inv, int64_t N,
                                                           const float* __restrict__ cam_pos,
                                                           float* __restrict__ dsh, float* __restrict__ dpos,
                                                           const float* __restrict__ jac) {
  constexpr int ROW = 3 * K, PITCH = ROW + 1;
  __shared__ float s_rows[256 * PITCH];
  const int64_t row0 = (int64_t)blockIdx.x * 256;
  const int64_t i = row0 + threadIdx.x;
  float* mine = s_rows + threadIdx.x * PITCH;
  const int64_t m = (i < N) ? (inv ? (int64_t)inv[i] : i) : -1;
  if (m >= 0) {
    const float vx = pos[3 * i] - cam_pos[0], vy = pos[3 * i + 1] - cam_pos[1], vz = pos[3 * i + 2] - cam_pos[2];
    const float rinv = 1.f / sqrtf(vx * vx + vy * vy + vz * vz);
    const float x = vx * rinv, y = vy * rinv, z = vz * rinv;
    float Y[K];
    gsr_sh_basis<K>(x, y, z, Y);
    const float g3[3] = {dcol[3 * m], dcol[3 * m + 1], dcol[3 * m + 2]};
#pragma unroll
    for (int ch = 0; ch < 3; ++ch)
#pragma unroll
      for (int k = 0; k < K; ++k) mine[ch * K + k] = g3[ch] * Y[k];
    if (dpos != nullptr && jac != nullptr) {
      float pj[3];
      gsr_jac_apply(g3, jac + 9 * m, pj);
      dpos[3 * i] += pj[0];
      dpos[3 * i + 1] += pj[1];
      dpos[3 * i + 2] += pj[2];
    } else if (dpos != nullptr && K > 1) {
      float dYx[K], dYy[K], dYz[K];
      gsr_sh_basis_grad<K>(x, y, z, dYx, dYy, dYz);
      const float* c = sh + (int64_t)ROW * i;
      float gx = 0.f, gy = 0.f, gz = 0.f;
#pragma unroll
      for (int ch = 0; ch < 3; ++ch) {
#pragma unroll
        for (int k = 1; k < K; ++k) {
          const float w = g3[ch] * c[ch * K + k];
          gx += w * dYx[k]; gy += w * dYy[k]; gz += w * dYz[k];
        }
      }
      const float dot = gx * x + gy * y + gz * z;
      dpos[3 * i] += (gx - x * dot) * rinv;
      dpos[3 * i + 1] += (gy - y * dot) * rinv;
      dpos[3 * i + 2] += (gz - z * dot) * rinv;
    }
  } else {
#pragma unroll
    for (int e = 0; e < ROW; ++e) mine[e] = 0.f;
  }
  __syncthreads();
  const int64_t rows_here = (N - row0) < 256 ? (N - row0) : 256;
  const int total = (int)rows_here * ROW;
  float* out = dsh + row0 * ROW;
  for (int e = threadIdx.x; e < total; e += 256) out[e] = s_rows[(e / ROW) * PITCH + (e % ROW)];
}

template <int K>
__global__ __launch_bounds__(256) void sh_bwd_multi_kernel(const float* __restrict__ G, int64_t g_stride,
                                                           const float* __restrict__ cams, int64_t cam_stride,
                                                           int ncam, const float* __restrict__ sh,
                                                           const float* __restrict__ pos, int64_t N,
                                                           float* __restrict__ dsh, float* __restrict__ dpos,
                                                           int accumulate) {
  const int64_t i = (int64_t)blockIdx.x * blockDim.x + threadIdx.x;
  if (i >= N) return;
  const float px = pos[3 * i], py = pos[3 * i + 1], pz = pos[3 * i + 2];
  const float* coef = sh + (int64_t)3 * K * i;
  float acc[3][K];
#pragma unroll
  for (int ch = 0; ch < 3; ++ch)
#pragma unroll
    for (int k = 0; k < K; ++k) acc[ch][k] = 0.f;
  float gpx = 0.f, gpy = 0.f, gpz = 0.f;
  bool any = false;
  for (int c = 0; c < ncam; ++c) {
    const float* g = G + (int64_t)c * g_stride + i * 3;
    const float g0 = g[0], g1 = g[1], g2 = g[2];
    if (g0 == 0.f && g1 == 0.f && g2 == 0.f) continue;
    any = true;
    const float* cp = cams + (int64_t)c * cam_stride;
    const float vx = px - cp[0], vy = py - cp[1], vz = pz - cp[2];
    const float inv = 1.f / sqrtf(vx * vx + vy * vy + vz * vz);
    const float x = vx * inv, y = vy * inv, z = vz * inv;
    float Y[K];
    gsr_sh_basis<K>(x, y, z, Y);
#pragma unroll
    for (int k = 0; k < K; ++k) {
      acc[0][k] += g0 * Y[k]; acc[1][k] += g1 * Y[k]; acc[2][k] += g2 * Y[k];
    }
    if (dpos != nullptr && K > 1) {
      float dYx[K], dYy[K], dYz[K];
      gsr_sh_basis_grad<K>(x, y, z, dYx, dYy, dYz);
      float gx = 0.f, gy = 0.f, gz = 0.f;
#pragma unroll
      for (int k = 1; k < K; ++k) {
        const float w = g0 * coef[k] + g1 * coef[K + k] + g2 * coef[2 * K + k];
        gx += w * dYx[k]; gy += w * dYy[k]; gz += w * dYz[k];
      }
      const float dot = gx * x + gy * y + gz * z;
      gpx += (gx - x * dot) * inv; gpy += (gy - y * dot) * inv; gpz += (gz - z * dot) * inv;
    }
  }
  if (!any && accumulate) return;
  float* row = dsh + (int64_t)3 * K * i;
#pragma unroll
  for (int ch = 0; ch < 3; ++ch)
#pragma unroll
    for (int k = 0; k < K; ++k) row[ch * K + k] = accumulate ? row[ch * K + k] + acc[ch][k] : acc[ch][k];
  if (any && dpos != nullptr && K > 1) {
    dpos[3 * i] += gpx; dpos[3 * i + 1] += gpy; dpos[3 * i + 2] += gpz;
  }
}

template <int K>
__global__ __launch_bounds__(256) void sh_bwd_multi_stream_kernel(const float* __restrict__ G, int64_t g_stride,
                                                                  const float* __restrict__ cams, int64_t cam_stride,
                                                                  int ncam, const float* __restrict__ pos, int64_t N,
                                                                  float* __restrict__ dsh) {
  constexpr int ROW = 3 * K, PITCH = ROW + 1;
  __shared__ float s_rows[256 * PITCH];
  const int64_t row0 = (int64_t)blockIdx.x * 256;
  const int64_t i = row0 + threadIdx.x;
  float acc[3][K];
#pragma unroll
  for (int ch = 0; ch < 3; ++ch)
#pragma unroll
    for (int k = 0; k < K; ++k) acc[ch][k] = 0.f;
  if (i < N) {
    const float px = pos[3 * i], py = pos[3 * i + 1], pz = pos[3 * i + 2];
    for (int c = 0; c < ncam; ++c) {
      const float* g = G + (int64_t)c * g_stride + i * 3;
      const float g0 = g[0], g1 = g[1], g2 = g[2];
      if (g0 == 0.f && g1 == 0.f && g2 == 0.f) continue;
      const float* cp = cams + (int64_t)c * cam_stride;
      const float vx = px - cp[0], vy = py - cp[1], vz = pz - cp[2];
      const float inv = 1.f / sqrtf(vx * vx + vy * vy + vz * vz);
      float Y[K];
      gsr_sh_basis<K>(vx * inv, vy * inv, vz * inv, Y);
#pragma unroll
      for (int k = 0; k < K; ++k) {
        acc[0][k] += g0 * Y[k]; acc[1][k] += g1 * Y[k]; acc[2][k] += g2 * Y[k];
      }
    }
  }
  float* mine = s_rows + threadIdx.x * PITCH;
#pragma unroll
  for (int ch = 0; ch < 3; ++ch)
#pragma unroll
    for (int k = 0; k < K; ++k) mine[ch * K + k] = acc[ch][k];
  __syncthreads();
  const int64_t rows_here = (N - row0) < 256 ? (N - row0) : 256;
  const int total = (int)rows_here * ROW;
  float* out = dsh + row0 * ROW;
  for (int e = threadIdx.x; e < total; e += 256) out[e] = s_rows[(e / ROW) * PITCH + (e % ROW)];
}

inline GsrRasterParams to_params(const GsrRasterParamsC* c) {
  GsrRasterParams rp;
  __builtin_memcpy(&rp, c, sizeof(rp));
  return rp;
}

inline unsigned grid_for(int64_t n, int block) { return (unsigned)((n + block - 1) / block); }

}

extern "C" {

int gsr_abi_version(void) { return 36; }

const char* gsr_error_string(int code) {
  switch (code) {
    case GSR_OK: return "ok";
    case GSR_ERR_INVALID_ARGUMENT: return "invalid argument";
    case GSR_ERR_WORKSPACE_TOO_SMALL: return "workspace too small";
    case GSR_ERR_LAUNCH_FAILED: return "kernel launch failed";
    case GSR_ERR_UNSUPPORTED: return "unsupported configuration";
    default: return "unknown error";
  }
}

size_t gsr_cull_workspace_bytes(int64_t N) {
  if (N < 0) N = 0;
  int64_t nw = (N + CULL_WAVE_SPAN - 1) / CULL_WAVE_SPAN;
  size_t counts = (((size_t)nw * sizeof(uint32_t) + 255) / 256) * 256;
  return counts + gsr_scan_workspace_bytes(nw) + 256;
}

int gsr_frustum_cull(const float* position, int64_t N, const float* T_camera_world, const float* projection, int32_t W,
                     int32_t H, float near_plane, float far_plane, float margin_px, int64_t* indexes_out,
                     uint32_t* count_dev, void* workspace, size_t workspace_bytes, void* stream_) {
  hipStream_t stream = reinterpret_cast<hipStream_t>(stream_);
  if (N < 0 || N > 0x7FFFFFFFll || !count_dev || !T_camera_world || !projection) return GSR_ERR_INVALID_ARGUMENT;
  if (N == 0) { hipMemsetAsync(count_dev, 0, sizeof(uint32_t), stream); return GSR_OK; }
  if (!position || !indexes_out) return GSR_ERR_INVALID_ARGUMENT;
  if (!workspace || workspace_bytes < gsr_cull_workspace_bytes(N)) return GSR_ERR_WORKSPACE_TOO_SMALL;
  const int64_t nw = (N + CULL_WAVE_SPAN - 1) / CULL_WAVE_SPAN;
  uint32_t* wave_counts = reinterpret_cast<uint32_t*>(workspace);
  size_t counts_bytes = (((size_t)nw * sizeof(uint32_t) + 255) / 256) * 256;
  uint8_t* scan_ws = reinterpret_cast<uint8_t*>(workspace) + counts_bytes;
  const unsigned blocks = grid_for(nw, 4);
  cull_count_kernel<<<blocks, 256, 0, stream>>>(position, N, T_camera_world, projection, W, H, near_plane, far_plane,
                                               margin_px, wave_counts, nw);
  GSR_CHECK_LAUNCH();
  const bool self_prefix = nw <= CULL_SELF_PREFIX_MAX_WAVES;
  if (!self_prefix) {
    int rc = gsr_exclusive_scan_u32(wave_counts, wave_counts, nw, count_dev, scan_ws, workspace_bytes - counts_bytes, stream_);
    if (rc != GSR_OK) return rc;
  }
  cull_write_kernel<<<blocks, 256, 0, stream>>>(position, N, T_camera_world, projection, W, H, near_plane, far_plane,
                                               margin_px, wave_counts, nw, indexes_out, self_prefix ? count_dev : nullptr);
  GSR_CHECK_LAUNCH();
  return GSR_OK;
}

int gsr_project_forward(const float* position, const float* log_scaling, const float* rotation_xyzw,
                        const float* alpha_logit, const int64_t* indexes, int64_t M, const float* T_camera_world,
                        const float* projection, const GsrRasterParamsC* params_host, float* gaussians2d_out,
                        float* depth_out, const uint32_t* count_dev, uint32_t* depth_keys_out, uint32_t depth_key_bias,
                        uint32_t depth_key_max, void* stream_) {
  hipStream_t stream = reinterpret_cast<hipStream_t>(stream_);
  if (M < 0 || !params_host) return GSR_ERR_INVALID_ARGUMENT;
  if (M == 0) return GSR_OK;
  if (!position || !log_scaling || !rotation_xyzw || !alpha_logit || !indexes || !T_camera_world || !projection ||
      !gaussians2d_out || !depth_out)
    return GSR_ERR_INVALID_ARGUMENT;
  project_fwd_kernel<<<grid_for(M, 256), 256, 0, stream>>>(position, log_scaling, rotation_xyzw, alpha_logit, indexes, M,
                                                          T_camera_world, projection, to_params(params_host),
                                                          gaussians2d_out, depth_out, count_dev, depth_keys_out,
                                                          depth_key_bias, depth_key_max);
  GSR_CHECK_LAUNCH();
  return GSR_OK;
}

int gsr_project_backward(const float* position, const float* log_scaling, const float* rotation_xyzw,
                         const float* alpha_logit, const int64_t* indexes, int64_t M, const float* T_camera_world,
                         const float* projection, const GsrRasterParamsC* params_host, const float* dL_dgaussians2d,
                         const float* dL_ddepth, float* d_position, float* d_log_scaling, float* d_rotation,
                         float* d_alpha_logit, int32_t accumulate, void* stream_) {
  hipStream_t stream = reinterpret_cast<hipStream_t>(stream_);
  if (M < 0 || !params_host) return GSR_ERR_INVALID_ARGUMENT;
  if (M == 0) return GSR_OK;
  if (!position || !log_scaling || !rotation_xyzw || !alpha_logit || !indexes || !T_camera_world || !projection ||
      !dL_dgaussians2d || !d_position || !d_log_scaling || !d_rotation || !d_alpha_logit)
    return GSR_ERR_INVALID_ARGUMENT;
  if (accumulate)
    project_bwd_kernel<true><<<grid_for(M, 256), 256, 0, stream>>>(position, log_scaling, rotation_xyzw, alpha_logit,
                                                                  indexes, M, T_camera_world, projection,
                                                                  to_params(params_host), dL_dgaussians2d, dL_ddepth,
                                                                  d_position, d_log_scaling, d_rotation, d_alpha_logit);
  else
    project_bwd_kernel<false><<<grid_for(M, 256), 256, 0, stream>>>(position, log_scaling, rotation_xyzw, alpha_logit,
                                                                   indexes, M, T_camera_world, projection,
                                                                   to_params(params_host), dL_dgaussians2d, dL_ddepth,
                                                                   d_position, d_log_scaling, d_rotation, d_alpha_logit);
  GSR_CHECK_LAUNCH();
  return GSR_OK;
}

int64_t gsr_camera_grad_partial_rows(int64_t count) { return count > 0 ? (int64_t)grid_for(count, 256) : 0; }

int gsr_camera_grad_finish(const float* partials, int64_t rows, const float* T_camera_world, float* d_camera,
                           void* stream_) {
  hipStream_t stream = reinterpret_cast<hipStream_t>(stream_);
  if (rows < 0 || !d_camera || (rows > 0 && !partials)) return GSR_ERR_INVALID_ARGUMENT;
  cam_grad_finish_kernel<<<1, 256, 0, stream>>>(partials, rows, T_camera_world, d_camera);
  GSR_CHECK_LAUNCH();
  return GSR_OK;
}

int gsr_project_backward_camera(const float* position, const float* log_scaling, const float* rotation_xyzw,
                                const float* alpha_logit, const int64_t* indexes, int64_t M, const float* T_camera_world,
                                const float* projection, const GsrRasterParamsC* params_host,
                                const float* dL_dgaussians2d, const float* dL_ddepth, float* d_position,
                                float* d_log_scaling, float* d_rotation, float* d_alpha_logit, int32_t accumulate,
                                float* camera_partials, float* d_camera, void* stream_) {
  hipStream_t stream = reinterpret_cast<hipStream_t>(stream_);
  if (M < 0 || !params_host || !T_camera_world || !projection || !d_camera) return GSR_ERR_INVALID_ARGUMENT;
  if (M > 0 && (!position || !log_scaling || !rotation_xyzw || !alpha_logit || !indexes || !dL_dgaussians2d ||
                !d_position || !d_log_scaling || !d_rotation || !d_alpha_logit || !camera_partials))
    return GSR_ERR_INVALID_ARGUMENT;
  if (M > 0) {
    const int rc = gsr_project_backward(position, log_scaling, rotation_xyzw, alpha_logit, indexes, M, T_camera_world,
                                        projection, params_host, dL_dgaussians2d, dL_ddepth, d_position, d_log_scaling,
                                        d_rotation, d_alpha_logit, accumulate, stream_);
    if (rc != GSR_OK) return rc;
    project_bwd_camera_kernel<<<grid_for(M, 256), 256, 0, stream>>>(position, log_scaling, rotation_xyzw, alpha_logit,
                                                                    indexes, M, T_camera_world, projection,
                                                                    to_params(params_host), dL_dgaussians2d, dL_ddepth,
                                                                    camera_partials);
    GSR_CHECK_LAUNCH();
  }
  return gsr_camera_grad_finish(camera_partials, gsr_camera_grad_partial_rows(M), T_camera_world, d_camera, stream_);
}

int gsr_sh_camera_position_grad(const float* dL_dcolors, const float* jacobian, int64_t M, float* camera_partials,
                                float* d_camera_pos, void* stream_) {
  hipStream_t stream = reinterpret_cast<hipStream_t>(stream_);
  if (M < 0 || !d_camera_pos) return GSR_ERR_INVALID_ARGUMENT;
  const bool live = M > 0 && jacobian != nullptr;
  if (live && (!dL_dcolors || !camera_partials)) return GSR_ERR_INVALID_ARGUMENT;
  if (live) {
    sh_camera_grad_kernel<<<grid_for(M, 256), 256, 0, stream>>>(dL_dcolors, jacobian, M, camera_partials);
    GSR_CHECK_LAUNCH();
  }
  return gsr_camera_grad_finish(camera_partials, live ? gsr_camera_grad_partial_rows(M) : 0, nullptr, d_camera_pos,
                                stream_);
}

int gsr_project_sh_forward(const float* position, const float* log_scaling, const float* rotation_xyzw,
                           const float* alpha_logit, const float* sh_features, int32_t K, const int64_t* indexes, int64_t M,
                           const float* T_camera_world, const float* projection, const float* camera_pos,
                           const GsrRasterParamsC* params_host, float* rows_out, float* screen_scale_out,
                           float* jacobian_out, const uint32_t* count_dev, uint32_t* depth_keys_out,
                           uint32_t depth_key_bias, uint32_t depth_key_max, void* stream_) {
  hipStream_t stream = reinterpret_cast<hipStream_t>(stream_);
  if (M < 0 || !params_host) return GSR_ERR_INVALID_ARGUMENT;
  if (K != 1 && K != 4 && K != 9 && K != 16) return GSR_ERR_UNSUPPORTED;
  if (M == 0) return GSR_OK;
  if (!position || !log_scaling || !rotation_xyzw || !alpha_logit || !sh_features || !indexes || !T_camera_world ||
      !projection || !camera_pos || !rows_out || !screen_scale_out)
    return GSR_ERR_INVALID_ARGUMENT;
  const unsigned g = grid_for(M, 256);
  const GsrRasterParams rp = to_params(params_host);
#define GSR_LAUNCH_PSF(KK, JJ)                                                                                          \
  project_sh_fwd_kernel<KK, JJ><<<g, 256, 0, stream>>>(position, log_scaling, rotation_xyzw, alpha_logit, sh_features,   \
                                                       indexes, M, T_camera_world, projection, camera_pos, rp, rows_out, \
                                                       screen_scale_out, jacobian_out, count_dev, depth_keys_out,        \
                                                       depth_key_bias, depth_key_max)
  const bool jj = jacobian_out != nullptr;
  switch (K) {
    case 1: if (jj) GSR_LAUNCH_PSF(1, true); else GSR_LAUNCH_PSF(1, false); break;
    case 4: if (jj) GSR_LAUNCH_PSF(4, true); else GSR_LAUNCH_PSF(4, false); break;
    case 9: if (jj) GSR_LAUNCH_PSF(9, true); else GSR_LAUNCH_PSF(9, false); break;
    default: if (jj) GSR_LAUNCH_PSF(16, true); else GSR_LAUNCH_PSF(16, false); break;
  }
#undef GSR_LAUNCH_PSF
  GSR_CHECK_LAUNCH();
  return GSR_OK;
}

int gsr_pack_rows(const float* gaussians2d, const float* depth, const float* features, int64_t M, int32_t C,
                  const GsrRasterParamsC* params_host, float* rows_out, float* screen_scale_out, void* stream_) {
  hipStream_t stream = reinterpret_cast<hipStream_t>(stream_);
  if (M < 0 || !params_host) return GSR_ERR_INVALID_ARGUMENT;
  const GsrRasterParams rp = to_params(params_host);
  if (C < 1 || C > 3) return GSR_ERR_UNSUPPORTED;
  if (M == 0) return GSR_OK;
  if (!gaussians2d || !depth || !features || !rows_out || !screen_scale_out) return GSR_ERR_INVALID_ARGUMENT;
  const unsigned g = grid_for(M, 256);
  if (C == 1) pack_rows_kernel<1><<<g, 256, 0, stream>>>(gaussians2d, depth, features, M, rp, rows_out, screen_scale_out);
  else if (C == 2) pack_rows_kernel<2><<<g, 256, 0, stream>>>(gaussians2d, depth, features, M, rp, rows_out, screen_scale_out);
  else pack_rows_kernel<3><<<g, 256, 0, stream>>>(gaussians2d, depth, features, M, rp, rows_out, screen_scale_out);
  GSR_CHECK_LAUNCH();
  return GSR_OK;
}

int gsr_pack_rows_wide(const float* gaussians2d, const float* depth, const float* features, int64_t M, int32_t C,
                       const GsrRasterParamsC* params_host, float* rows_out, float* feat_rows_out, float* screen_scale_out,
                       void* stream_) {
  hipStream_t stream = reinterpret_cast<hipStream_t>(stream_);
  if (M < 0 || !params_host) return GSR_ERR_INVALID_ARGUMENT;
  const GsrRasterParams rp = to_params(params_host);
  if (C < GSR_WIDE_MIN_FEATURES || C > GSR_MAX_FEATURES) return GSR_ERR_UNSUPPORTED;
  if (M == 0) return GSR_OK;
  if (!gaussians2d || !depth || !features || !rows_out || !feat_rows_out || !screen_scale_out) return GSR_ERR_INVALID_ARGUMENT;
  const unsigned g = grid_for(M, 256);
  if (C <= 4) pack_rows_wide_kernel<4><<<g, 256, 0, stream>>>(gaussians2d, depth, features, M, C, rp, rows_out, feat_rows_out, screen_scale_out);
  else if (C <= 8) pack_rows_wide_kernel<8><<<g, 256, 0, stream>>>(gaussians2d, depth, features, M, C, rp, rows_out, feat_rows_out, screen_scale_out);
  else pack_rows_wide_kernel<16><<<g, 256, 0, stream>>>(gaussians2d, depth, features, M, C, rp, rows_out, feat_rows_out, screen_scale_out);
  GSR_CHECK_LAUNCH();
  return GSR_OK;
}

int gsr_project_backward_rows(const float* position, const float* log_scaling, const float* rotation_xyzw,
                              const float* alpha_logit, const int64_t* indexes, int64_t M, const int32_t* inverse,
                              int64_t N, const float* T_camera_world, const float* projection,
                              const GsrRasterParamsC* params_host, const float* rows, const float* grad_rows,
                              const float* dL_dgaussians2d_extra, const float* dL_ddepth, const float* jacobian,
                              float* d_position, float* d_log_scaling, float* d_rotation, float* d_alpha_logit,
                              int32_t mode, float* d_colors_out, float* prune_cost_out, float* split_score_out,
                              float* visibility_out, void* stream_) {
  hipStream_t stream = reinterpret_cast<hipStream_t>(stream_);
  if (M < 0 || N < 0 || M > N || !params_host || mode < 0 || mode > 2) return GSR_ERR_INVALID_ARGUMENT;
  const bool geom = d_position != nullptr;
  if (geom && (!position || !log_scaling || !rotation_xyzw || !alpha_logit || !T_camera_world || !projection ||
               !d_log_scaling || !d_rotation || !d_alpha_logit || (M > 0 && !indexes)))
    return GSR_ERR_INVALID_ARGUMENT;
  if (mode == 2 && (!geom || (!inverse && M != N))) return GSR_ERR_INVALID_ARGUMENT;
  if (mode != 2 && M == 0) return GSR_OK;
  if (mode == 2 && N == 0) return GSR_OK;
  if (M > 0 && !grad_rows) return GSR_ERR_INVALID_ARGUMENT;
  const GsrRasterParams rp = to_params(params_host);
#define GSR_LAUNCH_PBR(MODE, COUNT)                                                                                      \
  project_bwd_rows_kernel<MODE><<<grid_for(COUNT, 256), 256, 0, stream>>>(                                               \
      position, log_scaling, rotation_xyzw, alpha_logit, indexes, M, inverse, N, T_camera_world, projection, rp, rows,   \
      grad_rows, dL_dgaussians2d_extra, dL_ddepth, jacobian, d_position, d_log_scaling, d_rotation, d_alpha_logit,       \
      d_colors_out, prune_cost_out, split_score_out, visibility_out)
  if (mode == 2) GSR_LAUNCH_PBR(2, N);
  else if (mode == 1) GSR_LAUNCH_PBR(1, M);
  else GSR_LAUNCH_PBR(0, M);
#undef GSR_LAUNCH_PBR
  GSR_CHECK_LAUNCH();
  return GSR_OK;
}

int gsr_project_backward_rows_camera(const float* position, const float* log_scaling, const float* rotation_xyzw,
                                     const float* alpha_logit, const int64_t* indexes, int64_t M, const int32_t* inverse,
                                     int64_t N, const float* T_camera_world, const float* projection,
                                     const GsrRasterParamsC* params_host, const float* rows, const float* grad_rows,
                                     const float* dL_dgaussians2d_extra, const float* dL_ddepth, const float* jacobian,
                                     float* d_position, float* d_log_scaling, float* d_rotation, float* d_alpha_logit,
                                     int32_t mode, float* d_colors_out, float* prune_cost_out, float* split_score_out,
                                     float* visibility_out, float* camera_partials, float* d_camera, void* stream_) {
  hipStream_t stream = reinterpret_cast<hipStream_t>(stream_);
  if (M < 0 || !d_camera || !T_camera_world || !projection || !d_position || (M > 0 && (!indexes || !grad_rows || !camera_partials)))
    return GSR_ERR_INVALID_ARGUMENT;
  const int rc = gsr_project_backward_rows(position, log_scaling, rotation_xyzw, alpha_logit, indexes, M, inverse, N,
                                           T_camera_world, projection, params_host, rows, grad_rows,
                                           dL_dgaussians2d_extra, dL_ddepth, jacobian, d_position, d_log_scaling,
                                           d_rotation, d_alpha_logit, mode, d_colors_out, prune_cost_out,
                                           split_score_out, visibility_out, stream_);
  if (rc != GSR_OK) return rc;
  if (M > 0) {
    project_bwd_rows_camera_kernel<<<grid_for(M, 256), 256, 0, stream>>>(
        position, log_scaling, rotation_xyzw, alpha_logit, indexes, M, T_camera_world, projection, to_params(params_host),
        grad_rows, dL_dgaussians2d_extra, dL_ddepth, jacobian, camera_partials);
    GSR_CHECK_LAUNCH();
  }
  return gsr_camera_grad_finish(camera_partials, gsr_camera_grad_partial_rows(M), T_camera_world, d_camera, stream_);
}

int gsr_sh_forward(const float* sh_features, const float* positions, const int64_t* indexes, int64_t M, int32_t K,
                   const float* camera_pos, float* colors_out, float* jacobian_out, const uint32_t* count_dev,
                   void* stream_) {
  hipStream_t stream = reinterpret_cast<hipStream_t>(stream_);
  if (M < 0) return GSR_ERR_INVALID_ARGUMENT;
  if (K != 1 && K != 4 && K != 9 && K != 16) return GSR_ERR_UNSUPPORTED;
  if (M == 0) return GSR_OK;
  if (!sh_features || !positions || !indexes || !camera_pos || !colors_out) return GSR_ERR_INVALID_ARGUMENT;
  const unsigned g = grid_for(M, 256);
  switch (K) {
    case 1:
      if (jacobian_out) sh_fwd_kernel<1, true><<<g, 256, 0, stream>>>(sh_features, positions, indexes, M, camera_pos, colors_out, jacobian_out, count_dev);
      else sh_fwd_kernel<1, false><<<g, 256, 0, stream>>>(sh_features, positions, indexes, M, camera_pos, colors_out, nullptr, count_dev);
      break;
    case 4:
      if (jacobian_out) sh_fwd_kernel<4, true><<<g, 256, 0, stream>>>(sh_features, positions, indexes, M, camera_pos, colors_out, jacobian_out, count_dev);
      else sh_fwd_kernel<4, false><<<g, 256, 0, stream>>>(sh_features, positions, indexes, M, camera_pos, colors_out, nullptr, count_dev);
      break;
    case 9:
      if (jacobian_out) sh_fwd_kernel<9, true><<<g, 256, 0, stream>>>(sh_features, positions, indexes, M, camera_pos, colors_out, jacobian_out, count_dev);
      else sh_fwd_kernel<9, false><<<g, 256, 0, stream>>>(sh_features, positions, indexes, M, camera_pos, colors_out, nullptr, count_dev);
      break;
    default:
      if (jacobian_out) sh_fwd_kernel<16, true><<<g, 256, 0, stream>>>(sh_features, positions, indexes, M, camera_pos, colors_out, jacobian_out, count_dev);
      else sh_fwd_kernel<16, false><<<g, 256, 0, stream>>>(sh_features, positions, indexes, M, camera_pos, colors_out, nullptr, count_dev);
      break;
  }
  GSR_CHECK_LAUNCH();
  return GSR_OK;
}

int gsr_sh_backward(const float* dL_dcolors, const float* sh_features, const float* positions, const int64_t* indexes,
                    int64_t M, int32_t K, const float* camera_pos, const float* jacobian, float* d_sh_features,
                    float* d_positions, int32_t accumulate, void* stream_) {
  hipStream_t stream = reinterpret_cast<hipStream_t>(stream_);
  if (M < 0) return GSR_ERR_INVALID_ARGUMENT;
  if (K != 1 && K != 4 && K != 9 && K != 16) return GSR_ERR_UNSUPPORTED;
  if (M == 0) return GSR_OK;
  if (!dL_dcolors || !sh_features || !positions || !indexes || !camera_pos || !d_sh_features)
    return GSR_ERR_INVALID_ARGUMENT;
// ... 84 lines not shown
```

splat-trainer_amd/renderer.py:

```python
from __future__ import annotations

import ctypes as C
import math
import os
import threading
from typing import Optional, Tuple

import torch

from . import _lib
from .data_types import CameraParams, Gaussians3D, RasterConfig, RenderedPoints, Rendering
from . import sh as _sh
from .sh import evaluate_sh_at

ROW_FLOATS = 16
PARTIAL_FLOATS = 12
CAMERA_GRAD_FLOATS = 20


class KernelTimer:

  def __init__(self):
    self.events = {}
    self._open = {}
# ... 213 lines not shown
  def feature_uninitialized(self) -> bool:
    return "feature" in self._fresh

  @feature_uninitialized.setter
  def feature_uninitialized(self, value: bool):
    (self._fresh.add if value else self._fresh.discard)("feature")

  def take_geometry_uninitialized(self) -> bool:
    return self.claim_overwrite("caller", self.GEOMETRY)

  def ensure_geometry_initialized(self):
    self.claim_accumulate("caller", self.GEOMETRY)

  def _check(self, name, like):
    t = getattr(self, name)
    if t is None or t.shape != like.shape or t.dtype != torch.float32 or not t.is_contiguous() or t.device != like.device:
      raise ValueError(f"GradOut.{name} must be a contiguous float32 tensor shaped like the parameter")
    return t


class _ProjectFn(torch.autograd.Function):

  @staticmethod
  def forward(ctx, position, log_scaling, rotation, alpha_logit, T, proj, cull_args, params, grad_out, prefetch):
    lib = _lib.load()
    pos, ls, rot, al = _f32c(position), _f32c(log_scaling), _f32c(rotation), _f32c(alpha_logit)
    N, dev = pos.shape[0], pos.device
    W, H, near, far, margin = cull_args
    stream = _stream()
    indexes_full = torch.empty(N, dtype=torch.int64, device=dev)
    count = torch.empty(1, dtype=torch.int32, device=dev)
    ws_bytes = lib.gsr_cull_workspace_bytes(N)
    ws = torch.empty(ws_bytes, dtype=torch.uint8, device=dev)
    g2d_full = torch.empty(N, 6, dtype=torch.float32, device=dev)
    depth_full = torch.empty(N, 1, dtype=torch.float32, device=dev)
    keys_full = _u32(N, dev) if prefetch is not None else None
    key_range = _depth_key_range(near, far)
    _lib.check(lib.gsr_frustum_cull(_ptr(pos), N, _ptr(T), _ptr(proj), W, H, near, far, margin, _ptr(indexes_full),
                                    _ptr(count), _ptr(ws), ws_bytes, stream), "gsr_frustum_cull")
    _lib.check(lib.gsr_project_forward(_ptr(pos), _ptr(ls), _ptr(rot), _ptr(al), _ptr(indexes_full), N, _ptr(T),
                                       _ptr(proj), C.byref(params), _ptr(g2d_full), _ptr(depth_full), _ptr(count),
                                       _ptr(keys_full), key_range[0], key_range[1], stream), "gsr_project_forward")
    wait = _start_readback(count)
    sh_job = prefetch.pop("sh", None) if prefetch is not None else None
    if sh_job is not None and N > 0:
      sh_out = _sh.launch_forward_counted(*sh_job[:3], indexes_full, count, sh_job[3])
    M = int(wait()[0])
    if sh_job is not None and N > 0:
      prefetch["sh_out"] = (sh_out[0][:M], sh_out[1][:M] if sh_out[1] is not None else None)
    indexes, g2d, depth = indexes_full[:M], g2d_full[:M], depth_full[:M]
    if prefetch is not None and M > 0:
      prefetch["order"] = _launch_depth_order(depth.reshape(-1), M, key_range, keys=keys_full[:M])
    ctx.save_for_backward(pos, ls, rot, al, indexes, T, proj)
    ctx.set_materialize_grads(False)
    ctx.params = params
    ctx.grad_out = grad_out
    ctx.in_dtypes = (position.dtype, log_scaling.dtype, rotation.dtype, alpha_logit.dtype)
    ctx.mark_non_differentiable(indexes)
    return g2d, depth, indexes

  @staticmethod
  def backward(ctx, d_g2d, d_depth, _d_indexes):
    lib = _lib.load()
    pos, ls, rot, al, indexes, T, proj = ctx.saved_tensors
    M, N = indexes.shape[0], pos.shape[0]
    go = ctx.grad_out
    if go is not None:
      d_pos, d_ls = go._check("position", pos), go._check("log_scaling", ls)
      d_rot, d_al = go._check("rotation", rot), go._check("alpha_logit", al)
      go.claim_accumulate("project_to_image.backward", go.GEOMETRY)
    else:
      live = M > 0 and (d_g2d is not None or d_depth is not None)
      alloc = torch.empty_like if (M == N and live) else torch.zeros_like
      d_pos, d_ls, d_rot, d_al = alloc(pos), alloc(ls), alloc(rot), alloc(al)
    want_cam = ctx.needs_input_grad[4] or ctx.needs_input_grad[5]
    d_camera = None
    if M > 0 and (d_g2d is not None or d_depth is not None):
      dg = _f32c(d_g2d) if d_g2d is not None else torch.zeros(M, 6, dtype=torch.float32, device=pos.device)
      dd = _f32c(d_depth) if d_depth is not None else None
      if want_cam:
        partials, d_camera = _camera_scratch(M, pos.device)
        _lib.check(lib.gsr_project_backward_camera(_ptr(pos), _ptr(ls), _ptr(rot), _ptr(al), _ptr(indexes), M, _ptr(T),
                                                   _ptr(proj), C.byref(ctx.params), _ptr(dg), _ptr(dd), _ptr(d_pos),
                                                   _ptr(d_ls), _ptr(d_rot), _ptr(d_al), 1 if go is not None else 0,
                                                   _ptr(partials), _ptr(d_camera), _stream()),
                   "gsr_project_backward_camera")
      else:
        _lib.check(lib.gsr_project_backward(_ptr(pos), _ptr(ls), _ptr(rot), _ptr(al), _ptr(indexes), M, _ptr(T),
                                            _ptr(proj), C.byref(ctx.params), _ptr(dg), _ptr(dd), _ptr(d_pos),
                                            _ptr(d_ls), _ptr(d_rot), _ptr(d_al), 1 if go is not None else 0,
                                            _stream()), "gsr_project_backward")
    d_T, d_proj = _camera_grads(d_camera, pos.device) if want_cam else (None, None)
    if go is not None:
      return None, None, None, None, d_T, d_proj, None, None, None, None
    dt = ctx.in_dtypes
    return d_pos.to(dt[0]), d_ls.to(dt[1]), d_rot.to(dt[2]), d_al.to(dt[3]), d_T, d_proj, None, None, None, None


def project_to_image(gaussians: Gaussians3D, camera_params: CameraParams, config: RasterConfig,
                     grad_out: Optional[GradOut] = None, prefetch: Optional[dict] = None
                     ) -> Tuple[torch.Tensor, torch.Tensor, torch.Tensor]:
  _require_device(gaussians.position, gaussians.log_scaling, gaussians.rotation, gaussians.alpha_logit)
  T = _f32c_camera(camera_params.T_camera_world)
  proj = _f32c_camera(camera_params.projection)
  params = _lib.raster_params(config)
  W, H = camera_params.image_size
  cull_args = (int(W), int(H), float(camera_params.near_plane), float(camera_params.far_plane),
               float(config.margin_tiles * config.tile_size))
  g2d, depth, indexes = _ProjectFn.apply(gaussians.position, gaussians.log_scaling, gaussians.rotation,
                                         gaussians.alpha_logit, T, proj, cull_args, params, grad_out, prefetch)
  if prefetch is not None and "order" in prefetch:
    prefetch["depth_order"] = (prefetch.pop("order"), depth, depth._version)
  return g2d, depth, indexes


class _RasterState:
  __slots__ = ("M", "O", "C", "W", "H", "params", "rows", "order", "count", "offsets", "sorted_splat",
               "sorted_inst", "tile_range", "vis_partial", "pair_vis", "final_T", "last", "median", "visibility",
               "prune_cost", "split_score", "screen_scale", "want_median", "compute_visibility", "needs_grad",
               "segments", "segment_buffers", "seg_pairs", "seg_min", "image", "key_range", "vis_ready", "vis_capacity",
               "near_far", "feat_rows")

  def materialize_visibility(self) -> torch.Tensor:
    if not self.vis_ready:
      _lib.check(_lib.load().gsr_reduce_visibility(_ptr(self.vis_partial), _ptr(self.offsets), _ptr(self.count),
                                                   _ptr(self.order), self.M, _ptr(self.visibility), self.vis_capacity,
                                                   None, _stream()), "gsr_reduce_visibility")
      self.vis_ready = True
    return self.visibility


def _u32(n: int, device) -> torch.Tensor:
  return torch.empty(max(n, 1), dtype=torch.int32, device=device)


_KEY_RANGES = {}


def _depth_key_range(near: float, far: float):
  key = (float(near), float(far))
  hit = _KEY_RANGES.get(key)
  if hit is None:
    bias, top = C.c_uint32(0), C.c_uint32(0)
    _lib.check(_lib.load().gsr_depth_key_range(key[0], key[1], C.byref(bias), C.byref(top)), "gsr_depth_key_range")
    hit = _KEY_RANGES[key] = (bias.value, top.value, max(1, int(top.value).bit_length()))
    if len(_KEY_RANGES) > 4096:
      _KEY_RANGES.clear()
  return hit


def _launch_depth_order(depth: Optional[torch.Tensor], M: int, key_range, keys: Optional[torch.Tensor] = None) -> torch.Tensor:
  lib = _lib.load()
  dev = keys.device if keys is not None else depth.device
  stream = _stream()
  bias, max_key, key_bits = key_range
  keys_a = keys if keys is not None else _u32(M, dev)
  keys_b, vals_a, vals_b = _u32(M, dev), _u32(M, dev), _u32(M, dev)
  sort_bytes = lib.gsr_sort_workspace_bytes(M)
  sort_ws = torch.empty(sort_bytes, dtype=torch.uint8, device=dev)
  if keys is None:
    _lib.check(lib.gsr_depth_keys(_ptr(depth), M, bias, max_key, _ptr(keys_a), stream), "gsr_depth_keys")
  where = _lib.check(lib.gsr_sort_pairs_u32(_ptr(keys_a), _ptr(vals_a), _ptr(keys_b), _ptr(vals_b), M, 1, 0, key_bits,
                                            _ptr(sort_ws), sort_bytes, None, stream), "gsr_sort_pairs_u32(depth)")
  return vals_b if where == 1 else vals_a


def _seg_ref(st: "_RasterState"):
  return C.byref(st.segments) if st.segments is not None else None


def _blank_frame(st: _RasterState, dev) -> torch.Tensor:
  M, C_, W, H = st.M, st.C, st.W, st.H
  st.O = 0
  st.rows = torch.empty(0, ROW_FLOATS, dtype=torch.float32, device=dev)
  st.prune_cost, st.split_score = torch.zeros(2, M, dtype=torch.float32, device=dev).unbind(0)
  st.screen_scale = torch.zeros(0, 2, dtype=torch.float32, device=dev)
  st.final_T = torch.ones(H, W, dtype=torch.float32, device=dev)
  st.last = torch.zeros(H, W, dtype=torch.int32, device=dev)
  st.median = torch.zeros(H, W, dtype=torch.float32, device=dev) if st.want_median else None
  st.visibility = torch.zeros(M, dtype=torch.float32, device=dev)
  st.vis_ready = True
  st.segments, st.segment_buffers = None, None
  return torch.zeros(H, W, C_, dtype=torch.float32, device=dev)


def _wide_width(C_: int) -> int:
  return 4 if C_ <= 4 else (8 if C_ <= 8 else 16)


def _composite_backward_wide(st: _RasterState, d_image: torch.Tensor, d_feat: torch.Tensor, dev) -> torch.Tensor:
  lib = _lib.load()
  if st.vis_partial is None:
    raise _lib.GsplatHipError("backward called on a rendering made without gradient state")
  stream = _stream()
  dimg = _f32c(d_image)
  partial = torch.empty(st.O, 8 + _wide_width(st.C), dtype=torch.float32, device=dev)
  timer = KERNEL_TIMER
  if timer is not None:
    timer.begin("composite_backward")
  _lib.check(lib.gsr_composite_backward_wide(_ptr(st.rows), _ptr(st.feat_rows), _ptr(st.sorted_splat),
                                             _ptr(st.sorted_inst), _ptr(st.pair_vis), _ptr(st.tile_range), st.W, st.H,
                                             st.C, C.byref(st.params), _ptr(st.final_T), _ptr(st.last), _ptr(dimg),
                                             _ptr(partial), stream), "gsr_composite_backward_wide")
  if timer is not None:
    timer.end("composite_backward")
  grows = torch.empty(st.M, ROW_FLOATS, dtype=torch.float32, device=dev)
  _lib.check(lib.gsr_reduce_gradients_wide(_ptr(partial), _ptr(st.vis_partial), _ptr(st.offsets), _ptr(st.count),
                                           _ptr(st.order), st.M, st.C, _ptr(grows), _ptr(d_feat), stream),
             "gsr_reduce_gradients_wide")
  return grows


def _composite_backward_rows(st: _RasterState, d_image: Optional[torch.Tensor], dev) -> torch.Tensor:
  lib = _lib.load()
  live = st.M > 0 and st.O > 0 and d_image is not None
  if not live:
    return torch.zeros(st.M, ROW_FLOATS, dtype=torch.float32, device=dev)
  if st.vis_partial is None:
    raise _lib.GsplatHipError("backward called on a rendering made without gradient state")
  stream = _stream()
  dimg = _f32c(d_image)
  partial = torch.empty(st.O, PARTIAL_FLOATS, dtype=torch.float32, device=dev)
  timer = KERNEL_TIMER
  if timer is not None:
    timer.begin("composite_backward")
  _lib.check(lib.gsr_composite_backward(_ptr(st.rows), _ptr(st.sorted_splat), _ptr(st.sorted_inst),
                                        _ptr(st.pair_vis), _ptr(st.tile_range), st.W, st.H, st.C,
                                        C.byref(st.params), _ptr(st.final_T), _ptr(st.last), _ptr(dimg),
                                        _ptr(st.image), _ptr(partial), _seg_ref(st), stream),
             "gsr_composite_backward")
  if timer is not None:
    timer.end("composite_backward")
  grows = torch.empty(st.M, ROW_FLOATS, dtype=torch.float32, device=dev)
  _lib.check(lib.gsr_reduce_gradients(_ptr(partial), _ptr(st.vis_partial), _ptr(st.offsets), _ptr(st.count),
                                      _ptr(st.order), st.M, _ptr(grows), stream), "gsr_reduce_gradients")
  return grows


def _vis_out(st: _RasterState, live: bool):
  if live and st.compute_visibility and not st.vis_ready:
    st.vis_ready = True
    return st.visibility
  return None


class _RasterFn(torch.autograd.Function):

  @staticmethod
  def forward(ctx, g2d, feats, depth, st: _RasterState, order):
    g, f, d = _f32c(g2d), _f32c(feats), _f32c(depth).reshape(-1)
    if st.M == 0:
      image = _blank_frame(st, g.device)
    else:
      st.order = order
      frame = _lib.GsrFrameC(None, None, None, None, None, st.M, 1, st.W, st.H, None, None, None, st.near_far[0],
                             st.near_far[1], st.params, 0, int(st.want_median), int(st.compute_visibility),
                             int(bool(st.needs_grad)), st.seg_pairs, st.seg_min, 0, g.data_ptr(), d.data_ptr(),
                             f.data_ptr(), st.C, order.data_ptr() if order is not None else None)
      frame.feature_table = int(st.C >= _lib.WIDE_MIN_FEATURES)
      _, _, _, image = _run_frame(frame, st, g.device, st.M, projected=True)
    ctx.st = st
    ctx.in_dtypes = (g2d.dtype, feats.dtype)
    return image

  @staticmethod
  def backward(ctx, d_image):
    lib = _lib.load()
    st: _RasterState = ctx.st
    dev = d_image.device
    live = st.M > 0 and st.O > 0
    alloc = torch.empty if live else torch.zeros
    d_g2d = alloc(st.M, 6, dtype=torch.float32, device=dev)
    d_feat = alloc(st.M, st.C, dtype=torch.float32, device=dev)
    if live:
      wide = st.C >= _lib.WIDE_MIN_FEATURES
      grows = _composite_backward_wide(st, d_image, d_feat, dev) if wide else _composite_backward_rows(st, d_image, dev)
      _lib.check(lib.gsr_unpack_grad_rows(_ptr(st.rows), _ptr(grows), st.M, st.C, _ptr(d_g2d),
                                          None if wide else _ptr(d_feat), _ptr(st.prune_cost), _ptr(st.split_score),
                                          _ptr(_vis_out(st, live)), _stream()), "gsr_unpack_grad_rows")
    return d_g2d.to(ctx.in_dtypes[0]), d_feat.to(ctx.in_dtypes[1]), None, None, None


def _arena_view(arena: torch.Tensor, offset: int, shape, dtype=torch.float32) -> torch.Tensor:
  typed = arena.view(dtype)
  size = typed.element_size()
  if len(shape) == 1:
    strides = (1,)
  elif len(shape) == 2:
    strides = (int(shape[1]), 1)
  else:
    strides = (int(shape[1]) * int(shape[2]), int(shape[2]), 1)
  return torch.as_strided(typed, shape, strides, offset // size)


def _pair_capacity(dev_index, N: int):
  guesses = _TLS.__dict__.setdefault("overlap_guess", {})
  raw = guesses.get(dev_index, 0)
  if raw <= 0:
    raw = max(4 * N, 1 << 16)
  step = 1 << max(raw.bit_length() - 5, 0)
  return guesses, raw, min((raw + step - 1) // step * step, 0x7fffffff)


def _run_frame(frame: "_lib.GsrFrameC", st: _RasterState, dev, rows_bound: int, projected: bool):
  lib = _lib.load()
  guesses, raw_guess, capacity = _pair_capacity(dev.index, rows_bound)
  plan, res = _lib.GsrFramePlanC(), _lib.GsrFrameResultC()
  timer = KERNEL_TIMER
  N, W, H, C_ = rows_bound, st.W, st.H, st.C
  while True:
    frame.pair_capacity = capacity
    _lib.check(lib.gsr_frame_plan(C.byref(frame), C.byref(plan)), "gsr_frame_plan")
    out = torch.empty(plan.out_bytes, dtype=torch.uint8, device=dev)
    work = torch.empty(plan.work_bytes, dtype=torch.uint8, device=dev)
    ev = timer.pair("composite_forward") if timer is not None else (None, None)
    host, ready, host_words = _readback_slot(dev)
    _lib.check(lib.gsr_frame_forward(C.byref(frame), C.byref(plan), C.c_void_p(out.data_ptr()),
                                     C.c_void_p(work.data_ptr()), C.byref(res), C.c_void_p(host.data_ptr()),
                                     C.c_void_p(ready.cuda_event), ev[0], ev[1], _stream()), "gsr_frame_forward")
    del work
    ready.synchronize()
    M, O, overflow = host_words[0], host_words[1], host_words[2]
    if overflow or O < 0:
      raise _lib.GsplatHipError("tile overlap count reached 2^31: the (tile, splat) lists are addressed with 32 bits")
    if O <= capacity:
      break
    if timer is not None:
      timer.events["composite_forward"].pop()
    capacity = O
  guesses[dev.index] = min(max(O + O // 4 + 4096, raw_guess - raw_guess // 64), 0x7fffffff)
  if projected:
    M = N
  base = out.data_ptr()
  out_f = out.view(torch.float32)
  V = lambda off, shape, strides: torch.as_strided(out_f, shape, strides, off >> 2)
  st.M, st.O = M, O
  st.rows = V(plan.rows, (M, ROW_FLOATS), (ROW_FLOATS, 1))
  st.screen_scale = V(plan.screen_scale, (M, 2), (2, 1))
  if res.order >= 0:
    st.order = base + res.order
  st.count, st.offsets = base + plan.count, base + plan.offsets
  st.sorted_splat, st.sorted_inst = base + res.sorted_splat, base + res.sorted_inst
  st.tile_range = base + plan.tile_range
  keep = st.compute_visibility or st.needs_grad
  st.vis_partial = base + plan.vis_partial if keep else None
  st.pair_vis = base + plan.pair_vis if keep else None
  st.final_T, st.last = V(plan.final_T, (H, W), (W, 1)), base + plan.last
  st.median = V(plan.median, (H, W), (W, 1)) if st.want_median else None
  st.visibility = V(plan.visibility, (M,), (1,))
  st.prune_cost, st.split_score = V(plan.prune_cost, (M,), (1,)), V(plan.split_score, (M,), (1,))
  st.vis_capacity = capacity
  st.feat_rows = base + plan.feat_rows if plan.feat_rows >= 0 else None
  if not st.compute_visibility:
    st.visibility.zero_()
  st.vis_ready = not (st.compute_visibility and st.needs_grad)
  st.segments = _lib.GsrSegmentsC.from_buffer_copy(res.segments) if res.has_segments else None
  st.segment_buffers = (out,)
  image = V(plan.image, (H, W, C_), (W * C_, C_, 1))
  st.image = base + plan.image if st.needs_grad else None
  return out, plan, M, image


class _FrameFn(torch.autograd.Function):

  @staticmethod
  def forward(ctx, position, log_scaling, rotation, alpha_logit, feature, T, proj, cam_pos, cull_args, st: _RasterState,
              grad_out, sh_out, want_jac):
    lib = _lib.load()
    pos, ls, rot, al = _f32c(position), _f32c(log_scaling), _f32c(rotation), _f32c(alpha_logit)
    sh, cam = _f32c(feature), _f32c(cam_pos)
    N, K, dev = pos.shape[0], sh.shape[2], pos.device
    W, H, near, far, margin = cull_args
    num_tiles = ((W + 15) // 16) * ((H + 15) // 16)
    if N == 0:
      indexes = torch.empty(0, dtype=torch.int64, device=dev)
      st.M = 0
      image = _blank_frame(st, dev)
      rows = st.rows
      ctx.save_for_backward(pos, ls, rot, al, sh, indexes, T, proj, cam)
      ctx.set_materialize_grads(False)
      ctx.st, ctx.jac, ctx.grad_out, ctx.sh_out = st, None, grad_out, sh_out
      ctx.in_dtypes = (position.dtype, log_scaling.dtype, rotation.dtype, alpha_logit.dtype, feature.dtype)
      ctx.mark_non_differentiable(indexes)
      return image, rows[:, 0:6], rows[:, 10:11], indexes
    frame = _lib.GsrFrameC(pos.data_ptr(), ls.data_ptr(), rot.data_ptr(), al.data_ptr(), sh.data_ptr(), N, K, W, H,
                           T.data_ptr(), proj.data_ptr(), cam.data_ptr(), near, far, st.params,
                           int(bool(want_jac and K > 1)), int(st.want_median), int(st.compute_visibility),
                           int(bool(st.needs_grad)), st.seg_pairs, st.seg_min, 0, None, None, None, 3, None)
    out, plan, M, image = _run_frame(frame, st, dev, N, projected=False)
    indexes = _arena_view(out, plan.indexes, (M,), torch.int64)
    rows = st.rows
    ctx.save_for_backward(pos, ls, rot, al, sh, indexes, T, proj, cam)
    ctx.set_materialize_grads(False)
    ctx.st, ctx.jac = st, (_arena_view(out, plan.jacobian, (M, 9)) if plan.jacobian >= 0 else None)
    ctx.grad_out, ctx.sh_out = grad_out, sh_out
    ctx.in_dtypes = (position.dtype, log_scaling.dtype, rotation.dtype, alpha_logit.dtype, feature.dtype)
    ctx.mark_non_differentiable(indexes)
    return image, rows[:, 0:6], rows[:, 10:11], indexes

  @staticmethod
  def backward(ctx, d_image, d_g2d, d_depth, _d_indexes):
    lib = _lib.load()
    pos, ls, rot, al, sh, indexes, T, proj, cam = ctx.saved_tensors
    st: _RasterState = ctx.st
    M, N, K, dev = indexes.shape[0], pos.shape[0], sh.shape[2], pos.device
    go, sh_out = ctx.grad_out, ctx.sh_out
    collector = sh_out if isinstance(sh_out, _sh.ShFactorCollector) else None
    nothing = (None,) * 13
    want_cam = ctx.needs_input_grad[5] or ctx.needs_input_grad[6]
    partials = d_camera = None
    dense = N > 0 and (M == N or 8 * M >= N)
    if go is not None:
      d_pos, d_ls = go._check("position", pos), go._check("log_scaling", ls)
      d_rot, d_al = go._check("rotation", rot), go._check("alpha_logit", al)
      mode = 1
      if dense and go.claim_overwrite("render_gaussians.backward", go.GEOMETRY):
        mode = 2
      elif not dense:
        go.claim_accumulate("render_gaussians.backward", go.GEOMETRY)
    else:
      alloc = torch.empty_like if dense else torch.zeros_like
      d_pos, d_ls, d_rot, d_al = alloc(pos), alloc(ls), alloc(rot), alloc(al)
      mode = 2 if dense else 0
    want_sh = collector is not None or sh_out is not None or ctx.needs_input_grad[4]
    d_sh, owner, sh_mode = None, None, 0
    if collector is None and want_sh:
      owner = sh_out[2] if (sh_out is not None and len(sh_out) > 2) else None
      d_sh = sh_out[0] if sh_out is not None else torch.empty(N, 3, K, dtype=torch.float32, device=dev)
      if sh_out is None:
        overwrite = True
        if not dense:
          d_sh.zero_()
      elif owner is None:
        overwrite = False
      elif dense:
        overwrite = owner.claim_overwrite("render_gaussians.backward", ("feature",))
      else:
        owner.claim_accumulate("render_gaussians.backward", ("feature",))
        overwrite = False
      sh_mode = 1 if (overwrite and dense) else 2
    if N > 0:
      live = M > 0 and st.O > 0 and d_image is not None
      if live and st.vis_partial is None:
        raise _lib.GsplatHipError("backward called on a rendering made without gradient state")
      inv = torch.empty(N, dtype=torch.int32, device=dev) if (M < N and dense) else None
      partial = torch.empty(st.O, PARTIAL_FLOATS, dtype=torch.float32, device=dev) if live else None
      grows = torch.empty(M, ROW_FLOATS, dtype=torch.float32, device=dev) if M > 0 else None
      dcol = torch.empty(M, 3, dtype=torch.float32, device=dev) if want_sh else None
      dimg = _f32c(d_image) if live else None
      dg = _f32c(d_g2d) if d_g2d is not None else None
      dd = _f32c(d_depth).reshape(-1) if d_depth is not None else None
      timer = KERNEL_TIMER
      ev = timer.pair("composite_backward") if (timer is not None and live) else (None, None)
      seg = C.addressof(st.segments) if st.segments is not None else None
      if want_cam:
        partials, d_camera = _camera_scratch(M, dev)
      args = _lib.GsrFrameBackwardC(
          _ptr(pos), _ptr(ls), _ptr(rot), _ptr(al), _ptr(sh), N, K, st.W, st.H, st.C, _ptr(T), _ptr(proj), _ptr(cam),
          st.params, M, st.O, _ptr(indexes), _ptr(st.rows), _ptr(st.order), _ptr(st.count), _ptr(st.offsets),
          _ptr(st.sorted_splat), _ptr(st.sorted_inst), _ptr(st.pair_vis), _ptr(st.vis_partial), _ptr(st.tile_range),
          _ptr(st.final_T), _ptr(st.last), _ptr(st.image), _ptr(ctx.jac), seg, _ptr(dimg), _ptr(dg), _ptr(dd),
          _ptr(partial), _ptr(grows), _ptr(inv), _ptr(dcol), _ptr(d_pos), _ptr(d_ls), _ptr(d_rot), _ptr(d_al), mode,
          _ptr(d_sh), sh_mode, _ptr(st.prune_cost), _ptr(st.split_score), _ptr(_vis_out(st, live)), _ptr(partials),
          _ptr(d_camera))
      early = getattr(collector, "on_rows", None) if collector is not None else None
      if early is not None and M > 0:
        _lib.check(lib.gsr_frame_backward_stages(C.byref(args), 1, ev[0], ev[1], _stream()), "gsr_frame_backward_stages(1)")
        early(indexes, grows, cam)
        _lib.check(lib.gsr_frame_backward_stages(C.byref(args), 2, None, None, _stream()), "gsr_frame_backward_stages(2)")
      else:
        _lib.check(lib.gsr_frame_backward(C.byref(args), ev[0], ev[1], _stream()), "gsr_frame_backward")
    else:
      dcol = torch.zeros(0, 3, dtype=torch.float32, device=dev) if want_sh else None
    if collector is not None:
      collector.items.append((indexes, dcol, cam, K == 1 or ctx.jac is not None))
    cam = _camera_grads(d_camera, dev) if want_cam else (None, None)
    if go is not None:
      return (None, None, None, None, d_sh.to(ctx.in_dtypes[4]) if (d_sh is not None and sh_out is None) else None) + \
          cam + nothing[7:]
    dt = ctx.in_dtypes
    return (d_pos.to(dt[0]), d_ls.to(dt[1]), d_rot.to(dt[2]), d_al.to(dt[3]),
            d_sh.to(dt[4]) if (d_sh is not None and sh_out is None) else None) + cam + nothing[7:]


def render_projected(indexes: torch.Tensor, gaussians2d: torch.Tensor, features: torch.Tensor,
                     depth: torch.Tensor, camera_params: CameraParams, config: RasterConfig,
                     render_median_depth: bool = False, _depth_order=None, **_unused) -> Rendering:
  _require_device(gaussians2d, features, depth)
  if features.dim() != 2 or not (1 <= features.shape[1] <= _lib.MAX_FEATURES):
    raise ValueError(f"features must be (M, C) with C in 1..{_lib.MAX_FEATURES}, got {tuple(features.shape)}")
  if config.tile_size != 16:
    raise ValueError("the HIP kernels are specialised for tile_size=16")
  W, H = camera_params.image_size
  st = _RasterState()
  st.M, st.C, st.W, st.H = int(gaussians2d.shape[0]), int(features.shape[1]), int(W), int(H)
  _init_state(st, camera_params, config, render_median_depth)
  st.needs_grad = torch.is_grad_enabled() and (gaussians2d.requires_grad or features.requires_grad)
  order = None
  if _depth_order is not None and _depth_order[1] is depth and _depth_order[2] == depth._version:
    order = _depth_order[0]
  image = _RasterFn.apply(gaussians2d, features, depth, st, order)
  return _rendering_of(st, image, indexes, gaussians2d, depth, camera_params)


def _init_state(st: _RasterState, camera_params: CameraParams, config: RasterConfig, render_median_depth: bool):
  st.params = _lib.raster_params(config)
  st.want_median = bool(render_median_depth)
  st.compute_visibility = bool(config.compute_visibility or config.compute_point_heuristic)
  st.vis_partial = st.pair_vis = st.segments = st.segment_buffers = st.rows = st.image = st.feat_rows = None
  st.vis_ready, st.vis_capacity = True, 0
  st.seg_pairs, st.seg_min = int(config.segment_pairs), int(config.segment_min_pairs)
  st.near_far = (float(camera_params.near_plane), float(camera_params.far_plane))
  st.key_range = _depth_key_range(*st.near_far)


def _rendering_of(st: _RasterState, image, indexes, gaussians2d, depth, camera_params) -> Rendering:
  points = RenderedPoints(idx=indexes, depths=depth, opacity=gaussians2d[:, 5], screen_scale=st.screen_scale,
                          visibility=st.visibility if st.vis_ready else st.materialize_visibility,
                          prune_cost=st.prune_cost, split_score=st.split_score)
  return Rendering(image=image, camera=camera_params, points=points, median_depth_image=st.median,
                   final_transmittance=st.final_T, num_overlaps=st.O)


def render_gaussians(gaussians: Gaussians3D, camera_params: CameraParams, config: Optional[RasterConfig] = None,
                     use_sh: bool = False, render_median_depth: bool = False, grad_out: Optional[GradOut] = None,
                     sh_collector=None, **options) -> Rendering:
  config = config or RasterConfig()
  feature = gaussians.feature
  if use_sh and feature.is_cuda and feature.dim() == 3 and feature.shape[1] == 3 and feature.shape[2] in (1, 4, 9, 16):
    return _render_frame(gaussians, camera_params, config, render_median_depth, grad_out, sh_collector)
  prefetch = {}
  if use_sh:
    sh_out = None
    if sh_collector is not None:
      sh_out = sh_collector
    elif grad_out is not None:
      sh_out = (grad_out._check("feature", feature), grad_out._check("position", gaussians.position), grad_out)
    g2d, depth, indexes = project_to_image(gaussians, camera_params, config, grad_out=grad_out, prefetch=prefetch)
    feats = evaluate_sh_at(feature, gaussians.position, indexes, camera_params.camera_position, grad_out=sh_out)
  else:
    if grad_out is not None:
      raise ValueError("grad_out with use_sh=False: gather the features yourself or use plain autograd")
    g2d, depth, indexes = project_to_image(gaussians, camera_params, config, grad_out=grad_out, prefetch=prefetch)
    feats = feature[indexes]
  return render_projected(indexes, g2d, feats, depth, camera_params, config,
                          render_median_depth=render_median_depth, _depth_order=prefetch.get("depth_order"), **options)


def _render_frame(gaussians: Gaussians3D, camera_params: CameraParams, config: RasterConfig, render_median_depth: bool,
                  grad_out: Optional[GradOut], sh_collector) -> Rendering:
  position, feature = gaussians.position, gaussians.feature
  _require_device(position, gaussians.log_scaling, gaussians.rotation, gaussians.alpha_logit, feature)
  if config.tile_size != 16:
    raise ValueError("the HIP kernels are specialised for tile_size=16")
  cam_grad = _wants_camera_grad(camera_params)
  if cam_grad and sh_collector is not None:
    raise ValueError("camera gradients are not supported in data-parallel mode (sh_collector): detach T_camera_world "
                     "and projection, or render on one device")
  sh_out = None
  if sh_collector is not None:
    sh_out = sh_collector
  elif grad_out is not None:
    sh_out = (grad_out._check("feature", feature), grad_out._check("position", position), grad_out)
  W, H = camera_params.image_size
  st = _RasterState()
  st.M, st.C, st.W, st.H, st.O = 0, 3, int(W), int(H), 0
  _init_state(st, camera_params, config, render_median_depth)
  st.needs_grad = torch.is_grad_enabled() and (grad_out is not None or sh_collector is not None or cam_grad or any(
      t.requires_grad for t in (position, gaussians.log_scaling, gaussians.rotation, gaussians.alpha_logit, feature)))
  cull_args = (int(W), int(H), float(camera_params.near_plane), float(camera_params.far_plane),
               float(config.margin_tiles * config.tile_size))
  want_pos_grad = _sh.wants_position_grad(position, sh_out) or (
      sh_collector is not None and sh_collector.position_term_local and torch.is_grad_enabled() and
      (position.requires_grad or grad_out is not None))
  if camera_params.T_camera_world.requires_grad:
    T_ = camera_params.T_camera_world.detach()
    cam_pos = -(T_[:3, :3].t() @ T_[:3, 3])
  else:
    cam_pos = camera_params.camera_position
  image, g2d, depth, indexes = _FrameFn.apply(position, gaussians.log_scaling, gaussians.rotation, gaussians.alpha_logit,
                                              feature, _f32c_camera(camera_params.T_camera_world),
                                              _f32c_camera(camera_params.projection), cam_pos, cull_args, st,
                                              grad_out, sh_out, want_pos_grad or cam_grad)
  return _rendering_of(st, image, indexes, g2d, depth, camera_params)
```

Baseline: 543.5 million.

## Replace global depth sort with per-tile bitonic depth sort after tile binning

Skips the global radix sort of all splats by depth. Tiles are binned in unsorted splat order, and each tile's list is then sorted by depth with in-register bitonic sorts. Lists longer than the cap are handled with chunk sorts followed by a galloping merge. A device flag records whether any tile list exceeds the cap, and the host polls it every few frames to pick between per-tile and global sort. This trades the N-sized global sort for per-tile work, but falls back whenever the flag reports long lists, and the flag decision lags by several frames.

```diff
diff --git a/include/gsplat_hip.h b/include/gsplat_hip.h
--- a/include/gsplat_hip.h
+++ b/include/gsplat_hip.h
@@ -156,6 +156,14 @@
                   int64_t capacity, const uint32_t* M_dev , void* stream);
 int gsr_tile_ranges(const uint32_t* sorted_keys, int64_t O, int32_t num_tiles, uint32_t* tile_range,
                     const uint32_t* O_dev , void* stream);
+int gsr_tile_ranges_flag_long(const uint32_t* sorted_keys, int64_t O, int32_t num_tiles, uint32_t* tile_range,
+                              const uint32_t* O_dev, uint32_t long_bound, uint32_t* long_flag, void* stream);
+
+#define GSR_TILE_SORT_CAP 1024u
+size_t gsr_tile_depth_sort_workspace_bytes(int64_t capacity);
+int gsr_tile_depth_sort(const uint32_t* tile_range, int32_t num_tiles, const uint32_t* tile_keys, const uint32_t* depth_keys,
+                        const uint32_t* inst_in, const uint32_t* splat_in, uint32_t* inst_out, uint32_t* splat_out,
+                        int64_t capacity, const uint32_t* O_dev, void* workspace, size_t workspace_bytes, void* stream);
 
 int gsr_segment_thresholds(int32_t seg_pairs_cfg, int32_t heavy_min_cfg, int64_t O, int32_t num_tiles, int32_t needs_grad,
                            int32_t* seg_pairs_out, int32_t* heavy_min_out);
@@ -234,7 +242,12 @@
   int32_t C;
   const uint32_t* depth_order;
   int32_t feature_table;
+  int32_t per_tile_sort;
 } GsrFrameC;
+#define GSR_TILE_SORT_MEAN_MAX 384
+#define GSR_COUNTS_LONG_LIST (3 + GSR_SEG_TOTAL_WORDS)
+#define GSR_ORDER_CALLER (-1)
+#define GSR_ORDER_IDENTITY (-2)
 typedef struct GsrFramePlanC {
   int64_t out_bytes, work_bytes;
   int64_t zero_begin, zero_bytes;
diff --git a/splat-trainer_amd/_lib.py b/splat-trainer_amd/_lib.py
--- a/splat-trainer_amd/_lib.py
+++ b/splat-trainer_amd/_lib.py
@@ -9,13 +9,16 @@
 PKG_DIR = os.path.dirname(os.path.abspath(__file__))
 LIB_PATH = os.path.join(PKG_DIR, "libgsplat_hip.so")
 
-ABI_VERSION = 36
+ABI_VERSION = 37
 PREFETCH_MIN_ROWS = 1_000_000
 MAX_FEATURES = 16
 WIDE_MIN_FEATURES = 4
 BILAGRID_MAX_SIDE = 32768
 KNN_MAX_K = 16
 NEIGHBOURS_MAX_N = 0x7FFFFFFF
+ORDER_IDENTITY = -2
+TILE_SORT_CAP = 1024
+COUNTS_LONG_LIST = 3 + 272
 
 
 class GsrRasterParamsC(C.Structure):
@@ -39,7 +42,7 @@
               ("compute_visibility", C.c_int32), ("needs_grad", C.c_int32), ("seg_pairs", C.c_int32),
               ("seg_min_pairs", C.c_int32), ("pair_capacity", C.c_int64), ("gaussians2d", C.c_void_p),
               ("depth", C.c_void_p), ("features", C.c_void_p), ("C", C.c_int32), ("depth_order", C.c_void_p),
-              ("feature_table", C.c_int32)]
+              ("feature_table", C.c_int32), ("per_tile_sort", C.c_int32)]
 
 
 FRAME_PLAN_FIELDS = ("out_bytes", "work_bytes", "zero_begin", "zero_bytes", "prune_cost", "split_score", "counts",
@@ -144,6 +147,9 @@
     "gsr_tile_count_offsets": (C.c_int, [_p, _p, _i64, _i32, _i32, _pp, _p, _p, _p, _p, _p, _p, _p, _sz, _p]),
     "gsr_tile_emit": (C.c_int, [_p, _p, _p, _p, _i64, _i32, _i32, _pp, _p, _p, _i64, _p, _p]),
     "gsr_tile_ranges": (C.c_int, [_p, _i64, _i32, _p, _p, _p]),
+    "gsr_tile_ranges_flag_long": (C.c_int, [_p, _i64, _i32, _p, _p, _u32, _p, _p]),
+    "gsr_tile_depth_sort_workspace_bytes": (_sz, [_i64]),
+    "gsr_tile_depth_sort": (C.c_int, [_p, _i32, _p, _p, _p, _p, _p, _p, _i64, _p, _p, _sz, _p]),
     "gsr_segment_thresholds": (C.c_int, [_i32, _i32, _i64, _i32, _i32, _p, _p]),
     "gsr_segment_capacity": (_i64, [_i64, _i32, _i32, _i32, _i32, _i32]),
     "gsr_segment_heavy_capacity": (_i64, [_i64, _i32, _i32, _i32, _i32, _i32]),
diff --git a/splat-trainer_amd/csrc/binning.hip b/splat-trainer_amd/csrc/binning.hip
--- a/splat-trainer_amd/csrc/binning.hip
+++ b/splat-trainer_amd/csrc/binning.hip
@@ -84,7 +84,7 @@
   uint32_t n = 0;
   bool large = false;
   if (live) {
-    const int64_t s = order[k];
+    const int64_t s = order ? (int64_t)order[k] : k;
     const float4* r = reinterpret_cast<const float4*>(rows + GSR_ROW_FLOATS * s);
     const float4 r0 = r[0];
     const float4 r1 = r[1];
@@ -196,7 +196,7 @@
   if (live) {
     hw = *reinterpret_cast<const uint4*>(hits + k);
     o = offsets[k];
-    sid = order[k];
+    sid = order ? order[k] : (uint32_t)k;
   }
   const bool large = (hw.y >> 16) != 0u;
   float4 r0 = make_float4(0.f, 0.f, 0.f, 0.f), r1 = r0;
@@ -226,13 +226,215 @@
 
 __global__ __launch_bounds__(256) void tile_ranges_kernel(const uint32_t* __restrict__ keys, int64_t O,
                                                           uint32_t* __restrict__ range,
-                                                          const uint32_t* __restrict__ O_dev) {
+                                                          const uint32_t* __restrict__ O_dev, uint32_t long_bound,
+                                                          uint32_t* __restrict__ long_flag) {
   if (O_dev) O = min(O, (int64_t)*O_dev);
   const int64_t i = (int64_t)blockIdx.x * blockDim.x + threadIdx.x;
   if (i >= O) return;
   const uint32_t t = keys[i];
   if (i == 0 || keys[i - 1] != t) range[2 * t] = (uint32_t)i;
-  if (i == O - 1 || keys[i + 1] != t) range[2 * t + 1] = (uint32_t)(i + 1);
+  if (i == O - 1 || keys[i + 1] != t) {
+    range[2 * t + 1] = (uint32_t)(i + 1);
+    if (long_flag && i >= (int64_t)long_bound && keys[i - long_bound] == t) *long_flag = 1u;
+  }
+}
+
+
+__device__ __forceinline__ uint64_t shfl_xor_u64(uint64_t x, int mask) {
+  const uint32_t lo = (uint32_t)__shfl_xor((int)(uint32_t)x, mask), hi = (uint32_t)__shfl_xor((int)(uint32_t)(x >> 32), mask);
+  return ((uint64_t)hi << 32) | lo;
+}
+
+template <int THREADS, int E>
+__device__ __forceinline__ void bitonic_sort_regs(uint64_t (&v)[E], uint32_t tid, uint64_t* xch) {
+  constexpr uint32_t P = (uint32_t)THREADS * E;
+  for (uint32_t k = 2; k <= P; k <<= 1) {
+    for (uint32_t j = k >> 1; j >= (uint32_t)E; j >>= 1) {
+      const uint32_t d = j / E;
+      const bool lower = (tid & d) == 0u;
+      const bool across_waves = THREADS > GSR_WAVE && d >= (uint32_t)GSR_WAVE;
+      if (across_waves) {
+        __syncthreads();
+#pragma unroll
+        for (int r = 0; r < E; ++r) xch[tid * E + r] = v[r];
+        __syncthreads();
+      }
+#pragma unroll
+      for (int r = 0; r < E; ++r) {
+        const uint64_t a = v[r], b = across_waves ? xch[(tid ^ d) * E + r] : shfl_xor_u64(a, (int)d);
+        const bool keep_min = lower == (((tid * E + r) & k) == 0u);
+        v[r] = keep_min ? (a < b ? a : b) : (a < b ? b : a);
+      }
+    }
+#pragma unroll
+    for (int jj = E / 2; jj > 0; jj >>= 1) {
+      if ((uint32_t)jj < k) {
+#pragma unroll
+        for (int r = 0; r < E; ++r) {
+          if (r & jj) continue;
+          const bool up = ((tid * E + r) & k) == 0u;
+          const uint64_t a = v[r], b = v[r | jj];
+          const bool swap = (a > b) == up;
+          v[r] = swap ? b : a;
+          v[r | jj] = swap ? a : b;
+        }
+      }
+    }
+  }
+}
+
+template <int E>
+__device__ __forceinline__ void sort_tile_wave(uint32_t lo, uint32_t n, uint32_t lane,
+                                               const uint32_t* __restrict__ depth_keys, const uint32_t* __restrict__ inst_in,
+                                               const uint32_t* __restrict__ splat_in, uint32_t* __restrict__ inst_out,
+                                               uint32_t* __restrict__ splat_out) {
+  uint64_t v[E];
+#pragma unroll
+  for (int r = 0; r < E; ++r) {
+    const uint32_t i = lane * E + r;
+    v[r] = i < n ? ((uint64_t)depth_keys[splat_in[lo + i] & 0x3FFFFFFFu] << 32) | i : ~0ull;
+  }
+  bitonic_sort_regs<GSR_WAVE, E>(v, lane, nullptr);
+#pragma unroll
+  for (int r = 0; r < E; ++r) {
+    const uint32_t i = lane * E + r;
+    if (i < n) {
+      const uint32_t j = lo + (uint32_t)v[r];
+      inst_out[lo + i] = inst_in[j];
+      splat_out[lo + i] = splat_in[j];
+    }
+  }
+}
+
+#define GSR_RUN_PER_THREAD (GSR_TILE_SORT_CAP / 256)
+
+__device__ __forceinline__ void sort_run(uint64_t* xch, uint32_t a, uint32_t b, const uint32_t* __restrict__ depth_keys,
+                                         const uint32_t* __restrict__ splat_in, uint64_t* __restrict__ runs) {
+  constexpr int E = GSR_RUN_PER_THREAD;
+  uint64_t v[E];
+#pragma unroll
+  for (int r = 0; r < E; ++r) {
+    const uint32_t p = a + threadIdx.x * E + r;
+    v[r] = p < b ? ((uint64_t)depth_keys[splat_in[p] & 0x3FFFFFFFu] << 32) | p : ~0ull;
+  }
+  bitonic_sort_regs<256, E>(v, threadIdx.x, xch);
+#pragma unroll
+  for (int r = 0; r < E; ++r) {
+    const uint32_t p = a + threadIdx.x * E + r;
+    if (p < b) runs[p] = v[r];
+  }
+}
+
+__global__ __launch_bounds__(256) void tile_depth_sort_kernel(const uint32_t* __restrict__ range, uint32_t num_tiles,
+                                                              const uint32_t* __restrict__ tile_keys,
+                                                              const uint32_t* __restrict__ depth_keys,
+                                                              const uint32_t* __restrict__ inst_in,
+                                                              const uint32_t* __restrict__ splat_in,
+                                                              uint32_t* __restrict__ inst_out,
+                                                              uint32_t* __restrict__ splat_out, uint32_t capacity,
+                                                              const uint32_t* __restrict__ O_dev,
+                                                              uint64_t* __restrict__ runs, uint32_t chunk_blocks) {
+  if (blockIdx.x < chunk_blocks) {
+    __shared__ uint64_t xch[GSR_TILE_SORT_CAP];
+    const uint32_t O = O_dev ? min(capacity, *O_dev) : capacity;
+    const uint32_t c0 = blockIdx.x * GSR_TILE_SORT_CAP;
+    if (c0 >= O) return;
+    const uint32_t c1 = min(c0 + GSR_TILE_SORT_CAP, O);
+    const uint32_t ta = tile_keys[c0], tb = tile_keys[c1 - 1u];
+    const uint32_t alo = range[2 * ta], ahi = range[2 * ta + 1];
+    if (ahi - alo > GSR_TILE_SORT_CAP) sort_run(xch, c0, min(ahi, c1), depth_keys, splat_in, runs);
+    if (tb != ta) {
+      const uint32_t blo = range[2 * tb], bhi = range[2 * tb + 1];
+      if (bhi - blo > GSR_TILE_SORT_CAP) sort_run(xch, blo, c1, depth_keys, splat_in, runs);
+    }
+    return;
+  }
+  const uint32_t t = (blockIdx.x - chunk_blocks) * 4u + (threadIdx.x >> 6);
+  if (t >= num_tiles) return;
+  const uint32_t lo = range[2 * t], n = range[2 * t + 1] - lo;
+  const uint32_t lane = (uint32_t)gsr_lane();
+  if (n == 0u || n > GSR_TILE_SORT_CAP) return;
+  if (n <= 64u) sort_tile_wave<1>(lo, n, lane, depth_keys, inst_in, splat_in, inst_out, splat_out);
+  else if (n <= 128u) sort_tile_wave<2>(lo, n, lane, depth_keys, inst_in, splat_in, inst_out, splat_out);
+  else if (n <= 256u) sort_tile_wave<4>(lo, n, lane, depth_keys, inst_in, splat_in, inst_out, splat_out);
+  else if (n <= 512u) sort_tile_wave<8>(lo, n, lane, depth_keys, inst_in, splat_in, inst_out, splat_out);
+  else sort_tile_wave<16>(lo, n, lane, depth_keys, inst_in, splat_in, inst_out, splat_out);
+}
+
+__device__ __forceinline__ uint32_t gallop_lds(const uint64_t* s, uint32_t j, uint32_t m, uint64_t x) {
+  if (j >= m || s[j] >= x) return j;
+  uint32_t lo = j, step = 1u;
+  while (lo + step < m && s[lo + step] < x) {
+    lo += step;
+    step <<= 1;
+  }
+  uint32_t hi = min(lo + step, m);
+  while (hi - lo > 1u) {
+    const uint32_t mid = (lo + hi) >> 1;
+    if (s[mid] < x) lo = mid;
+    else hi = mid;
+  }
+  return hi;
+}
+
+#define GSR_MERGE_PER_THREAD GSR_RUN_PER_THREAD
+__global__ __launch_bounds__(256) void tile_depth_merge_kernel(const uint32_t* __restrict__ range,
+                                                               const uint32_t* __restrict__ tile_keys,
+                                                               const uint32_t* __restrict__ inst_in,
+                                                               const uint32_t* __restrict__ splat_in,
+                                                               uint32_t* __restrict__ inst_out,
+                                                               uint32_t* __restrict__ splat_out, uint32_t capacity,
+                                                               const uint32_t* __restrict__ O_dev,
+                                                               const uint64_t* __restrict__ runs) {
+  static_assert(GSR_MERGE_PER_THREAD * 256 == GSR_TILE_SORT_CAP, "one element slot per thread and chunk position");
+  __shared__ uint64_t s[GSR_TILE_SORT_CAP];
+  const uint32_t O = O_dev ? min(capacity, *O_dev) : capacity;
+  const uint32_t c = blockIdx.x, c0 = c * GSR_TILE_SORT_CAP;
+  if (c0 >= O) return;
+  const uint32_t c1 = min(c0 + GSR_TILE_SORT_CAP, O);
+  const uint32_t ta = tile_keys[c0], tb = tile_keys[c1 - 1u];
+  for (int side = 0; side < 2; ++side) {
+    const uint32_t t = side == 0 ? ta : tb;
+    if (side == 1 && tb == ta) break;
+    const uint32_t lo = range[2 * t], hi = range[2 * t + 1];
+    if (hi - lo <= GSR_TILE_SORT_CAP) continue;
+    const uint32_t rlo = max(lo, c0), rhi = min(hi, c1);
+    uint64_t v[GSR_MERGE_PER_THREAD];
+    uint32_t rank[GSR_MERGE_PER_THREAD];
+    const uint32_t e0 = rlo + GSR_MERGE_PER_THREAD * threadIdx.x;
+#pragma unroll
+    for (int e = 0; e < GSR_MERGE_PER_THREAD; ++e) {
+      const uint32_t p = e0 + (uint32_t)e;
+      v[e] = p < rhi ? runs[p] : ~0ull;
+      rank[e] = p - rlo;
+    }
+    const uint32_t cfirst = lo / GSR_TILE_SORT_CAP, clast = (hi - 1u) / GSR_TILE_SORT_CAP;
+    for (uint32_t o = cfirst; o <= clast; ++o) {
+      if (o == c) continue;
+      const uint32_t olo = max(lo, o * GSR_TILE_SORT_CAP), ohi = min(hi, (o + 1u) * GSR_TILE_SORT_CAP);
+      const uint32_t m = ohi - olo;
+      __syncthreads();
+      for (uint32_t i = threadIdx.x; i < m; i += 256u) s[i] = runs[olo + i];
+      __syncthreads();
+      if (e0 < rhi) {
+        uint32_t j = 0u;
+#pragma unroll
+        for (int e = 0; e < GSR_MERGE_PER_THREAD; ++e) {
+          j = gallop_lds(s, j, m, v[e]);
+          rank[e] += j;
+        }
+      }
+    }
+#pragma unroll
+    for (int e = 0; e < GSR_MERGE_PER_THREAD; ++e) {
+      if (e0 + (uint32_t)e < rhi) {
+        const uint32_t src = (uint32_t)v[e];
+        inst_out[lo + rank[e]] = inst_in[src];
+        splat_out[lo + rank[e]] = splat_in[src];
+      }
+    }
+    __syncthreads();
+  }
 }
 
 #define GSR_REDUCE_SERIAL 64u
@@ -491,7 +693,7 @@
   if (M < 0 || M >= (1ll << 30) || !params_host || W <= 0 || H <= 0) return GSR_ERR_INVALID_ARGUMENT;
   if (params_host->tile_size != 16) return GSR_ERR_UNSUPPORTED;
   if (M == 0) return GSR_OK;
-  if (!rows || !order || !count_out || !tile_hits_out) return GSR_ERR_INVALID_ARGUMENT;
+  if (!rows || !count_out || !tile_hits_out) return GSR_ERR_INVALID_ARGUMENT;
   const int tx = (W + 15) / 16, ty = (H + 15) / 16;
   if (tx > 0xFFFF || ty > 0xFFFF) return GSR_ERR_UNSUPPORTED;
   tile_count_kernel<<<grid_for(M, 256), 256, 0, stream>>>(rows, order, M, tx, ty, to_params(params_host), count_out,
@@ -513,7 +715,7 @@
   if (params_host->tile_size != 16) return GSR_ERR_UNSUPPORTED;
   if (!total_dev || !overflow_flag) return GSR_ERR_INVALID_ARGUMENT;
   if (M == 0) { hipMemsetAsync(total_dev, 0, sizeof(uint32_t), stream); return GSR_OK; }
-  if (!rows || !order || !count_out || !tile_hits_out || !offsets_out) return GSR_ERR_INVALID_ARGUMENT;
+  if (!rows || !count_out || !tile_hits_out || !offsets_out) return GSR_ERR_INVALID_ARGUMENT;
   if (!workspace || workspace_bytes < gsr_tile_count_offsets_workspace_bytes(M)) return GSR_ERR_WORKSPACE_TOO_SMALL;
   const int tx = (W + 15) / 16, ty = (H + 15) / 16;
   if (tx > 0xFFFF || ty > 0xFFFF) return GSR_ERR_UNSUPPORTED;
@@ -535,7 +737,7 @@
   if (capacity < 0 || capacity > 0x7FFFFFFFll) return GSR_ERR_INVALID_ARGUMENT;
   if (params_host->tile_size != 16) return GSR_ERR_UNSUPPORTED;
   if (M == 0) return GSR_OK;
-  if (!rows || !order || !offsets || !tile_hits || !keys_out || !inst2splat_out) return GSR_ERR_INVALID_ARGUMENT;
+  if (!rows || !offsets || !tile_hits || !keys_out || !inst2splat_out) return GSR_ERR_INVALID_ARGUMENT;
   const int tx = (W + 15) / 16, ty = (H + 15) / 16;
   tile_emit_kernel<<<grid_for(M, 256), 256, 0, stream>>>(rows, order, offsets, reinterpret_cast<const TileHits*>(tile_hits),
                                                         M, tx, ty, to_params(params_host), keys_out, inst2splat_out,
@@ -544,13 +746,44 @@
   return GSR_OK;
 }
 
-int gsr_tile_ranges(const uint32_t* sorted_keys, int64_t O, int32_t num_tiles, uint32_t* tile_range,
-                    const uint32_t* O_dev, void* stream_) {
+int gsr_tile_ranges_flag_long(const uint32_t* sorted_keys, int64_t O, int32_t num_tiles, uint32_t* tile_range,
+                              const uint32_t* O_dev, uint32_t long_bound, uint32_t* long_flag, void* stream_) {
   hipStream_t stream = reinterpret_cast<hipStream_t>(stream_);
   if (O < 0 || num_tiles <= 0) return GSR_ERR_INVALID_ARGUMENT;
   if (O == 0) return GSR_OK;
   if (!sorted_keys || !tile_range) return GSR_ERR_INVALID_ARGUMENT;
-  tile_ranges_kernel<<<grid_for(O, 256), 256, 0, stream>>>(sorted_keys, O, tile_range, O_dev);
+  tile_ranges_kernel<<<grid_for(O, 256), 256, 0, stream>>>(sorted_keys, O, tile_range, O_dev, long_bound, long_flag);
+  GSR_CHECK_LAUNCH();
+  return GSR_OK;
+}
+
+int gsr_tile_ranges(const uint32_t* sorted_keys, int64_t O, int32_t num_tiles, uint32_t* tile_range,
+                    const uint32_t* O_dev, void* stream_) {
+  return gsr_tile_ranges_flag_long(sorted_keys, O, num_tiles, tile_range, O_dev, 0u, nullptr, stream_);
+}
+
+size_t gsr_tile_depth_sort_workspace_bytes(int64_t capacity) {
+  return (size_t)(capacity > 0 ? capacity : 0) * sizeof(uint64_t) + 256;
+}
+
+int gsr_tile_depth_sort(const uint32_t* tile_range, int32_t num_tiles, const uint32_t* tile_keys, const uint32_t* depth_keys,
+                        const uint32_t* inst_in, const uint32_t* splat_in, uint32_t* inst_out, uint32_t* splat_out,
+                        int64_t capacity, const uint32_t* O_dev, void* workspace, size_t workspace_bytes, void* stream_) {
+  hipStream_t stream = reinterpret_cast<hipStream_t>(stream_);
+  if (num_tiles <= 0 || capacity < 0 || capacity > 0x7FFFFFFFll) return GSR_ERR_INVALID_ARGUMENT;
+  if (capacity == 0) return GSR_OK;
+  if (!tile_range || !tile_keys || !depth_keys || !inst_in || !splat_in || !inst_out || !splat_out)
+    return GSR_ERR_INVALID_ARGUMENT;
+  if (inst_out == inst_in || splat_out == splat_in) return GSR_ERR_INVALID_ARGUMENT;
+  if (!workspace || workspace_bytes < gsr_tile_depth_sort_workspace_bytes(capacity)) return GSR_ERR_WORKSPACE_TOO_SMALL;
+  uint64_t* runs = reinterpret_cast<uint64_t*>(workspace);
+  const unsigned chunks = grid_for(capacity, (int)GSR_TILE_SORT_CAP);
+  tile_depth_sort_kernel<<<chunks + grid_for(num_tiles, 4), 256, 0, stream>>>(
+      tile_range, (uint32_t)num_tiles, tile_keys, depth_keys, inst_in, splat_in, inst_out, splat_out, (uint32_t)capacity,
+      O_dev, runs, chunks);
+  GSR_CHECK_LAUNCH();
+  tile_depth_merge_kernel<<<chunks, 256, 0, stream>>>(tile_range, tile_keys, inst_in, splat_in, inst_out, splat_out,
+                                                      (uint32_t)capacity, O_dev, runs);
   GSR_CHECK_LAUNCH();
   return GSR_OK;
 }
diff --git a/splat-trainer_amd/csrc/frame.hip b/splat-trainer_amd/csrc/frame.hip
--- a/splat-trainer_amd/csrc/frame.hip
+++ b/splat-trainer_amd/csrc/frame.hip
@@ -17,16 +17,20 @@
   }
 };
 
+inline int bit_length(uint32_t v) {
+  int b = 0;
+  while (v) { ++b; v >>= 1; }
+  return b < 1 ? 1 : b;
+}
+
+inline bool per_tile_depth_order(const GsrFrameC* f, int64_t cap, int64_t T) {
+  return !f->depth_order && f->per_tile_sort && cap <= (int64_t)GSR_TILE_SORT_MEAN_MAX * T;
+}
+
 inline int tile_bits_of(int num_tiles) {
   int b = 1;
   while ((1 << b) < num_tiles) ++b;
   return b;
-}
-
-inline int bit_length(uint32_t v) {
-  int b = 0;
-  while (v) { ++b; v >>= 1; }
-  return b < 1 ? 1 : b;
 }
 
 template <class T>
@@ -57,7 +61,7 @@
   p->zero_begin = 0;
   p->prune_cost = out.take(4 * N);
   p->split_score = out.take(4 * N);
-  p->counts = out.take(4 * (3 + GSR_SEG_TOTAL_WORDS));
+  p->counts = out.take(4 * (GSR_COUNTS_LONG_LIST + 1));
   p->tile_range = out.take(4 * 2 * T);
   p->vis_partial = vis_partial ? out.take(4 * cap) : -1;
   p->zero_bytes = out.at;
@@ -72,8 +76,10 @@
   p->median = f->want_median ? out.take(4 * P) : -1;
   p->count = out.take(4 * N);
   p->offsets = out.take(4 * N);
-  p->vals_a = out.take(4 * N);
-  p->vals_b = out.take(4 * N);
+  const bool per_tile = per_tile_depth_order(f, cap, T);
+  const bool global_sort = !f->depth_order && !per_tile;
+  p->vals_a = global_sort ? out.take(4 * N) : -1;
+  p->vals_b = global_sort ? out.take(4 * N) : -1;
   p->tvals_a = out.take(4 * cap);
   p->tvals_b = out.take(4 * cap);
   p->trank_a = out.take(4 * cap + 16);
@@ -100,17 +106,18 @@
 
   Cursor work;
   p->cull_ws_bytes = projected ? 0 : (int64_t)gsr_cull_workspace_bytes(N);
-  p->sort_ws_bytes = (int64_t)gsr_sort_workspace_bytes(N);
+  p->sort_ws_bytes = per_tile      ? (int64_t)gsr_tile_depth_sort_workspace_bytes(cap)
+                     : global_sort ? (int64_t)gsr_sort_workspace_bytes(N) : 0;
   p->scan_ws_bytes = (int64_t)gsr_scan_workspace_bytes(N);
   if (N <= GSR_TILE_COUNT_OFFSETS_MAX && (int64_t)gsr_tile_count_offsets_workspace_bytes(N) > p->scan_ws_bytes)
     p->scan_ws_bytes = (int64_t)gsr_tile_count_offsets_workspace_bytes(N);
   p->tsort_ws_bytes = (int64_t)gsr_sort_workspace_bytes(cap);
   p->cull_ws = projected ? -1 : work.take(p->cull_ws_bytes);
-  p->sort_ws = work.take(p->sort_ws_bytes);
+  p->sort_ws = f->depth_order ? -1 : work.take(p->sort_ws_bytes);
   p->scan_ws = work.take(p->scan_ws_bytes);
   p->tsort_ws = work.take(p->tsort_ws_bytes);
   p->keys_a = work.take(4 * N);
-  p->keys_b = work.take(4 * N);
+  p->keys_b = global_sort ? work.take(4 * N) : -1;
   p->tile_hits = work.take(16 * N);
   p->tkeys_a = work.take(4 * cap);
   p->tkeys_b = work.take(4 * cap);
@@ -168,11 +175,12 @@
                                    at<float>(out, p->screen_scale), at<float>(out, p->jacobian), M_dev,
                                    keys_a, key_bias, key_max, stream_));
   }
-  uint32_t* vals_a = at<uint32_t>(out, p->vals_a);
-  uint32_t* vals_b = at<uint32_t>(out, p->vals_b);
+  const bool per_tile = per_tile_depth_order(f, cap, T);
   const uint32_t* order = f->depth_order;
-  res->order = -1;
-  if (!order) {
+  res->order = order ? GSR_ORDER_CALLER : GSR_ORDER_IDENTITY;
+  if (!order && !per_tile) {
+    uint32_t* vals_a = at<uint32_t>(out, p->vals_a);
+    uint32_t* vals_b = at<uint32_t>(out, p->vals_b);
     GSR_TRY(gsr_sort_pairs_u32(keys_a, vals_a, at<uint32_t>(work, p->keys_b), vals_b, N, 1, 0, bit_length(key_max),
                                at<uint8_t>(work, p->sort_ws), (size_t)p->sort_ws_bytes, M_dev, stream_));
     res->order = rc == 1 ? p->vals_b : p->vals_a;
@@ -207,14 +215,21 @@
     GSR_TRY(gsr_tile_emit(rows, order, offsets, hits, N, f->W, f->H, &f->params, tkeys_a, trank_a, cap, M_dev, stream_));
     GSR_TRY(gsr_sort_pairs2_u32(tkeys_a, tvals_a, trank_a, tkeys_b, tvals_b, trank_b, cap, 1, 0, tile_bits_of(T),
                                 at<uint8_t>(work, p->tsort_ws), (size_t)p->tsort_ws_bytes, O_dev, stream_));
-    const bool in_b = rc == 1;
+    bool in_b = rc == 1;
+    const uint32_t* sorted_keys = in_b ? tkeys_b : tkeys_a;
+    uint32_t* tile_range = at<uint32_t>(out, p->tile_range);
+    GSR_TRY(gsr_tile_ranges_flag_long(sorted_keys, cap, T, tile_range, O_dev, GSR_TILE_SORT_CAP,
+                                      counts + GSR_COUNTS_LONG_LIST, stream_));
+    if (per_tile) {
+      GSR_TRY(gsr_tile_depth_sort(tile_range, T, sorted_keys, keys_a, in_b ? tvals_b : tvals_a, in_b ? trank_b : trank_a,
+                                  in_b ? tvals_a : tvals_b, in_b ? trank_a : trank_b, cap, O_dev,
+                                  at<uint8_t>(work, p->sort_ws), (size_t)p->sort_ws_bytes, stream_));
+      in_b = !in_b;
+    }
     res->sorted_inst = in_b ? p->tvals_b : p->tvals_a;
     res->sorted_splat = in_b ? p->trank_b : p->trank_a;
-    const uint32_t* sorted_keys = in_b ? tkeys_b : tkeys_a;
     const uint32_t* sorted_inst = in_b ? tvals_b : tvals_a;
     const uint32_t* sorted_splat = in_b ? trank_b : trank_a;
-    uint32_t* tile_range = at<uint32_t>(out, p->tile_range);
-    GSR_TRY(gsr_tile_ranges(sorted_keys, cap, T, tile_range, O_dev, stream_));
     const GsrSegmentsC* seg = nullptr;
     if (p->seg_capacity > 0) {
       uint32_t* tables = at<uint32_t>(out, p->seg_tables);
diff --git a/splat-trainer_amd/csrc/geometry.hip b/splat-trainer_amd/csrc/geometry.hip
--- a/splat-trainer_amd/csrc/geometry.hip
+++ b/splat-trainer_amd/csrc/geometry.hip
@@ -816,7 +816,7 @@
 
 extern "C" {
 
-int gsr_abi_version(void) { return 36; }
+int gsr_abi_version(void) { return 37; }
 
 const char* gsr_error_string(int code) {
   switch (code) {
diff --git a/splat-trainer_amd/renderer.py b/splat-trainer_amd/renderer.py
--- a/splat-trainer_amd/renderer.py
+++ b/splat-trainer_amd/renderer.py
@@ -539,12 +539,28 @@
   return guesses, raw, min((raw + step - 1) // step * step, 0x7fffffff)
 
 
+LIST_CHECK_FRAMES = 8
+
+
+def _list_state(dev_index):
+  pool = _TLS.__dict__.setdefault("long_lists", {})
+  state = pool.get(dev_index)
+  if state is None:
+    state = pool[dev_index] = {"host": torch.zeros(1, dtype=torch.int32).pin_memory(), "event": torch.cuda.Event(),
+                               "pending": False, "long": True, "per_tile": False, "countdown": 0}
+  return state
+
+
 def _run_frame(frame: "_lib.GsrFrameC", st: _RasterState, dev, rows_bound: int, projected: bool):
   lib = _lib.load()
   guesses, raw_guess, capacity = _pair_capacity(dev.index, rows_bound)
   plan, res = _lib.GsrFramePlanC(), _lib.GsrFrameResultC()
   timer = KERNEL_TIMER
   N, W, H, C_ = rows_bound, st.W, st.H, st.C
+  lists = _list_state(dev.index)
+  if lists["pending"] and lists["event"].query():
+    lists["long"], lists["pending"] = bool(int(lists["host"][0])), False
+  frame.per_tile_sort = 0 if lists["long"] else 1
   while True:
     frame.pair_capacity = capacity
     _lib.check(lib.gsr_frame_plan(C.byref(frame), C.byref(plan)), "gsr_frame_plan")
@@ -568,6 +584,13 @@
   guesses[dev.index] = min(max(O + O // 4 + 4096, raw_guess - raw_guess // 64), 0x7fffffff)
   if projected:
     M = N
+  lists["per_tile"] = res.order == _lib.ORDER_IDENTITY
+  lists["countdown"] -= 1
+  if not lists["pending"] and lists["countdown"] <= 0 and O > 0:
+    word = (plan.counts >> 2) + _lib.COUNTS_LONG_LIST
+    lists["host"].copy_(out.view(torch.int32)[word:word + 1], non_blocking=True)
+    lists["event"].record(_lib.current_stream())
+    lists["pending"], lists["countdown"] = True, LIST_CHECK_FRAMES
   base = out.data_ptr()
   out_f = out.view(torch.float32)
   V = lambda off, shape, strides: torch.as_strided(out_f, shape, strides, off >> 2)
@@ -576,6 +599,8 @@
   st.screen_scale = V(plan.screen_scale, (M, 2), (2, 1))
   if res.order >= 0:
     st.order = base + res.order
+  elif res.order == _lib.ORDER_IDENTITY:
+    st.order = None
   st.count, st.offsets = base + plan.count, base + plan.offsets
   st.sorted_splat, st.sorted_inst = base + res.sorted_splat, base + res.sorted_inst
   st.tile_range = base + plan.tile_range
```

After: 559.3 million, median of 6. 2.9% higher.
